# yaramohamadi/Pairwise_Sample_Optimization

Measured on AMD Instinct MI355X. Metric: PSO train-step imgs/sec (paired 1024² SDXL) at 1/2/4/8 MI355X, higher is better.
Workload: dtype bf16; 1 GPU; C2: SDXL-Turbo PSO train step, LoRA r=32 grads, 2 pairs/GPU/micro-step, gas 2, 2-step sampler (T=1); global_batch=4, seq_len=4096, resolution=1024, parallelism=dp1, launch=eager

## Files before the change

include/pso_amd.h:

```cpp
#ifndef PSO_AMD_H
#define PSO_AMD_H

#include <stddef.h>
#include <stdint.h>

#ifdef __cplusplus
extern "C" {
#endif

#define PSO_ABI_VERSION 1

#define PSO_OK 0
#define PSO_ERR_ARG 1
#define PSO_ERR_HIP 2
#define PSO_ERR_UNSUPPORTED 3

#define PSO_F32 0
#define PSO_BF16 1
#define PSO_F16 2
#define PSO_U8 2

#define PSO_MODE_TURBO 0
#define PSO_MODE_DMD 1
#define PSO_MODE_DMD_F16 2
// ... 18 lines not shown
                      const void* eps_ref, int eps_dtype, const float* coef, const float* pref, float beta,
                      float clip_eps, float* lp_out, float* loss_out, void* ws, size_t ws_bytes, void* stream);
int pso_pair_loss_bwd(int mode, int P, int n, const float* x, const float* x_prev, const void* eps_pol,
                      int eps_dtype, const float* coef, const float* pref, float beta, float clip_eps,
                      const float* grad_out, float grad_scale, void* deps_pol, int deps_dtype, const void* ws,
                      size_t ws_bytes, void* stream);

int pso_pair_loss_from_lp(int mode, int P, const float* lp_pol, const float* lp_ref, const float* pref, float beta,
                          float clip_eps, float* loss_out, float* dlp_out, void* stream);

int pso_gemm(int M, int N, const void* a1, long lda1, int K1, const void* b1, long ldb1, const void* a2, long lda2,
             int K2, const void* b2, long ldb2, float alpha, const void* bias, const void* rowbias, long ld_rowbias,
             int rows_per_group, const void* resid, long ldr, void* out, long ldo, int out_dtype, int accumulate,
             int tail_group_n, int tail_rows, void* stream);
size_t pso_gemm_ws_bytes(int M, int N, int K1, int K2);
int pso_gemm_ws(int M, int N, const void* a1, long lda1, int K1, const void* b1, long ldb1, const void* a2, long lda2,
                int K2, const void* b2, long ldb2, float alpha, const void* bias, const void* rowbias, long ld_rowbias,
                int rows_per_group, const void* resid, long ldr, void* out, long ldo, int out_dtype, int accumulate,
                int tail_group_n, int tail_rows, void* ws, size_t ws_bytes, void* stream);

int pso_gemm_batched(int batch, int M, int N, int K, const void* a, long lda, long stride_a, const void* b, long ldb,
                     long stride_b, float alpha, void* out, long ldo, long stride_o, int out_dtype, void* stream);

const char* pso_last_kernel(void);


int pso_gemm_tn(int M, int I, int J, const void* A, long lda, const void* B, long ldb, float alpha, float* out,
                long ldo, void* stream);
size_t pso_gemm_tn_ws_bytes(int M, int I, int J);
int pso_gemm_tn_ws(int M, int I, int J, const void* A, long lda, const void* B, long ldb, float alpha, float* out,
                   long ldo, void* ws, size_t ws_bytes, void* stream);
int pso_gemm_tn_grouped(int M, int I, int J, const void* A, long lda, const void* B, long ldb, float alpha, float* out,
                        long ldo, int group, void* stream);
int pso_gemm_tn_geglu(int M, int F2, int J, const void* A, long lda, const void* B, long ldb, float alpha, float* out,
                      long ldo, void* stream);
typedef struct {
  const void* x; long ldx;
  const void* u; long ldu;
  float* out; long ldo;
  int M, C, group_c;
  float alpha;
} PsoTnRankProblem;
int pso_gemm_tn_rank_batch(int R, int out_jc, int count, const PsoTnRankProblem* probs, void* stream);
size_t pso_gemm_tn_rank_batch_ws_bytes(int R, int out_jc, int count, const PsoTnRankProblem* probs);
int pso_gemm_tn_rank_batch_ws(int R, int out_jc, int count, const PsoTnRankProblem* probs, void* ws, size_t ws_bytes,
                              void* stream);
int pso_gemm_skinny_grouped(int M, int N, int K, const void* A, long lda, const void* W, long ldw, float alpha,
                            void* out, long ldo, int groups, void* stream);

int pso_gemm_geglu(int M, int N, const void* a, long lda, int K, const void* w, long ldw, const void* bias, void* out,
                   long ldo, void* out_pre, long ld_pre, int pre_rows, void* stream);
int pso_gemm_geglu_bwd(int M, int N, const void* a, long lda, int K, const void* w, long ldw, const void* pre,
                       long ld_pre, void* out, long ldo, void* stream);

int pso_quant_rows_fp8(int M, int K, const void* x, long ldx, void* q, long ldq, void* e8m0, void* stream);
int pso_gemm_fp8(int epi, int M, int N, int K, const void* a, long lda, const void* sa, const void* w, long ldw,
                 const void* sw, const void* a2, long lda2, int K2, const void* sa2, const void* w2, long ldw2,
                 const void* sw2, int tail_m, int tail_group_n, float alpha, const void* bias, const void* resid,
                 long ldr, void* out, long ldo, void* out_pre, long ld_pre, int pre_rows, void* stream);

size_t pso_db_loss_ws_bytes(int B, int n);
int pso_db_loss_fwd(int loss_type, int B, int n, const void* eps, const void* eps_ref, int eps_dtype,
                    const float* noisy, const float* x0, const float* sigma, float beta, float neg_defactor,
                    float prior_w, float* losses_out, float* logits_out, float* loss_out, void* ws, size_t ws_bytes,
                    void* stream);
int pso_db_loss_bwd(int loss_type, int B, int n, const void* eps, int eps_dtype, const float* noisy, const float* x0,
                    const float* sigma, float beta, float neg_defactor, float prior_w, const float* grad_out,
                    float grad_scale, void* deps, int deps_dtype, const void* ws, size_t ws_bytes, void* stream);

#define PSO_CONV_NORMAL 1
#define PSO_CONV_UP2 2
#define PSO_CONV_T2 3
int pso_conv2d(int mode, int B, const void* src1, int C1, const void* src2, int C2, int H, int W, int Ho, int Wo,
               int ks, int stride, int pad, const void* weight, int Cout, const void* a2, long lda2, int K2,
               const void* b2, long ldb2, float alpha, const void* bias, const void* rowbias, long ld_rowbias,
               const void* resid, long ldr, void* out, long ldo, int out_dtype, int accumulate, void* stream);
size_t pso_conv2d_ws_bytes(int B, int Ho, int Wo, int Cout, int K1, int K2);
int pso_conv2d_ws(int mode, int B, const void* src1, int C1, const void* src2, int C2, int H, int W, int Ho, int Wo,
                  int ks, int stride, int pad, const void* weight, int Cout, const void* a2, long lda2, int K2,
                  const void* b2, long ldb2, float alpha, const void* bias, const void* rowbias, long ld_rowbias,
                  const void* resid, long ldr, void* out, long ldo, int out_dtype, int accumulate, void* ws,
                  size_t ws_bytes, void* stream);

size_t pso_group_norm_ws_bytes(int B, int HW, int C);
int pso_group_norm_fwd(int B, int HW, int C, int G, float eps, const void* x, const void* gamma, const void* beta,
                       int silu, void* y, float* stats, void* ws, size_t ws_bytes, void* stream);
int pso_group_norm_bwd(int B, int HW, int C, int G, const void* x, const void* dy, const float* stats,
                       const void* gamma, const void* beta, int silu, const void* dadd, void* dx, float* dgamma,
                       float* dbeta, int accumulate_dparams, void* ws, size_t ws_bytes, void* stream);

int pso_layer_norm_fwd(int M, int C, float eps, const void* x, long ldx, const void* gamma, const void* beta, void* y,
                       long ldy, float* stats, void* stream);
int pso_layer_norm_bwd(int M, int C, const void* x, long ldx, const void* dy, long lddy, const float* stats,
                       const void* gamma, const void* dadd, long ldadd, void* dx, long lddx, void* stream);

int pso_attention_fwd(int B, int H, int Sq, int Sk, const void* q, long ldq, long sq_b, const void* k, long ldk,
                      long sk_b, const void* v, long ldv, long sv_b, float scale, void* o, long ldo, long so_b,
                      float* lse, void* stream);
size_t pso_attention_bwd_ws_bytes(int B, int H, int Sq, int Sk);
int pso_attention_bwd(int B, int H, int Sq, int Sk, const void* q, long ldq, long sq_b, const void* k, long ldk,
                      long sk_b, const void* v, long ldv, long sv_b, const void* o, long ldo, long so_b,
                      const float* lse, const void* dO, long lddo, long sdo_b, float scale, void* dq, long lddq,
                      long sdq_b, void* dk, long lddk, long sdk_b, void* dv, long lddv, long sdv_b, void* ws,
                      size_t ws_bytes, void* stream);

int pso_geglu_fwd(long M, int F, const void* in, long ldi, void* out, long ldo, void* stream);
int pso_geglu_bwd(long M, int F, const void* in, long ldi, const void* dout, long lddo, void* din, long lddi,
                  void* stream);
int pso_silu(long n, const void* x, void* y, void* stream);
int pso_timestep_embedding(int n, int dim, const float* t, void* out, long ldo, int out_col, void* stream);
int pso_transpose(int R, int Rp, int C, const void* in, long ldi, void* out, long ldo, void* stream);
int pso_im2col3(int B, int H, int W, int C, const void* in, void* out, int Kp, void* stream);

int pso_colsum_acc(long M, int N, const void* x, long ldx, long rows_per_group, float* out, long ldo, void* stream);
int pso_layer_norm_dparam(int M, int C, const void* x, long ldx, const void* dy, long lddy, const float* stats,
                          float* dgamma, float* dbeta, void* stream);
size_t pso_colsum_acc_ws_bytes(long M, int N, long rows_per_group);
int pso_colsum_acc_ws(long M, int N, const void* x, long ldx, long rows_per_group, float* out, long ldo, void* ws,
                      size_t ws_bytes, void* stream);
size_t pso_layer_norm_dparam_ws_bytes(int M, int C);
int pso_layer_norm_dparam_ws(int M, int C, const void* x, long ldx, const void* dy, long lddy, const float* stats,
                             float* dgamma, float* dbeta, void* ws, size_t ws_bytes, void* stream);
int pso_im2col_conv(int mode, int B, const void* src1, int C1, const void* src2, int C2, int H, int W, int Ho, int Wo,
                    int stride, int pad, void* out, long ldo, void* stream);
int pso_sumpool2(int B, int H, int W, int C, const void* in, const void* dadd, void* out, void* stream);
int pso_axpby(long n, float a, const void* x, float b, const void* z, void* y, void* stream);
int pso_cast_f32_bf16(long n, const float* x, float scale, void* y, void* stream);
int pso_cast_bf16_f32(long n, const void* x, float* y, void* stream);
int pso_conv_weight_t(int Co, int ks, int Ci, int flip, const void* w, void* wt, void* stream);
int pso_transpose_batched(int n, const void* descs, int max_r, int max_c, void* stream);
int pso_lora_pack(int n, const void* descs, long max_items, float scale, void* stream);
int pso_lora_grad_fold(int n, const void* descs, long max_items, void* stream);
int pso_dora_weight_norm(int n, const void* descs, int max_out, int init, void* stream);
int pso_dora_scale_fwd(int M, int N, int rows_policy, const void* z, long ldz, const float* g, const void* bias,
                       const void* resid, long ldr, void* y, long ldy, void* stream);
size_t pso_dora_bwd_ws_bytes(int M, int N);
int pso_dora_bwd(int M, int N, const void* dy, long lddy, const void* z, long ldz, const float* g, const float* n,
                 void* dyg, long lddyg, float* dm, void* ws, size_t ws_bytes, void* stream);
int pso_lora_merge(int n, const void* descs, const void* host_descs, void* stream);
int pso_transpose_multi(int n, const void* descs, int total_tiles, void* stream);
int pso_gather_rows(long n, long row_bytes, const void* src, const int64_t* idx, void* dst, void* stream);
int pso_nchw_to_nhwc(int B, int C, int Cp, long HW, const void* src, int src_dtype, float scale, void* dst,
                     void* stream);
int pso_softmax_rows(int M, int N, void* x, long ld, void* stream);
int pso_nhwc_to_nchw(int B, int C, long HW, const void* src, void* dst, int dst_dtype, void* stream);
int pso_concat_channels(long npix, int C1, const void* x1, int C2, const void* x2, void* out, void* stream);
int pso_split_channels(long npix, int C1, int C2, const void* in, void* y1, void* y2, const void* add2,
                       void* stream);

size_t pso_grad_clip_ws_bytes(long n);
int pso_grad_clip_coef(long n, const float* grad, float grad_scale, float max_norm, float* out_norm_coef, void* ws,
                       size_t ws_bytes, void* stream);
int pso_adamw_step(long n, float* param, const float* grad, float* exp_avg, float* exp_avg_sq, float lr, float beta1,
                   float beta2, float eps, float weight_decay, int step, float grad_scale, const float* clip_coef,
                   void* stream);
size_t pso_adamw8bit_blocks(long n);
void pso_adamw8bit_maps(float* signed_map, float* unsigned_map);
int pso_adamw8bit_step(long n, float* param, const float* grad, uint8_t* exp_avg_q, uint8_t* exp_avg_sq_q,
                       float* absmax_m, float* absmax_v, float lr, float beta1, float beta2, float eps,
                       float weight_decay, int step, float grad_scale, const float* clip_coef, void* stream);
int pso_adamw8bit_step_bf16(long n, float* param, void* param_bf16, const float* grad, uint8_t* exp_avg_q,
                            uint8_t* exp_avg_sq_q, float* absmax_m, float* absmax_v, float lr, float beta1, float beta2,
                            float eps, float weight_decay, int step, float grad_scale, const float* clip_coef,
                            void* stream);
int pso_adamw8bit_step_blocks(long n, int nblk, const long* desc, float* param, void* param_bf16, const float* grad,
                              uint8_t* exp_avg_q, uint8_t* exp_avg_sq_q, float* absmax_m, float* absmax_v,
                              float* exp_avg_32, float* exp_avg_sq_32, float lr, float beta1, float beta2, float eps,
                              float weight_decay, int step, float grad_scale, const float* clip_coef, void* stream);
int pso_adamw8bit_step_blocks_zero_grad(long n, int nblk, const long* desc, float* param, void* param_bf16,
                                        float* grad, uint8_t* exp_avg_q, uint8_t* exp_avg_sq_q, float* absmax_m,
                                        float* absmax_v, float* exp_avg_32, float* exp_avg_sq_32, float lr,
                                        float beta1, float beta2, float eps, float weight_decay, int step,
                                        float grad_scale, const float* clip_coef, void* stream);
int pso_zero_f32(long n, float* x, void* stream);
#define PSO_AMP_WORDS 16
#define PSO_AMP_SCALE 0
#define PSO_AMP_INV_SCALE 1
#define PSO_AMP_FOUND_INF 2
#define PSO_AMP_GROWTH_TRACKER 3
#define PSO_AMP_STEP 4
#define PSO_AMP_SKIPPED 5
#define PSO_AMP_NORM 6
#define PSO_AMP_CLIP_COEF 7
#define PSO_AMP_GRAD_MUL 8
#define PSO_AMP_BC1 9
#define PSO_AMP_BC2_SQRT 10
#define PSO_AMP_C1 11
#define PSO_AMP_C2 12
int pso_amp_unscale_clip(long n, const float* grad, float grad_scale, float max_norm, float beta1, float beta2,
                         void* amp_state, void* ws, size_t ws_bytes, void* stream);
int pso_amp_update(void* amp_state, float growth_factor, float backoff_factor, int growth_interval, void* stream);
int pso_adamw_step_amp(long n, float* param, const float* grad, float* exp_avg, float* exp_avg_sq, float lr,
                       float beta1, float beta2, float eps, float weight_decay, const void* amp_state, void* stream);
int pso_adamw8bit_step_blocks_amp(long n, int nblk, const long* desc, float* param, void* param_bf16,
                                  const float* grad, uint8_t* exp_avg_q, uint8_t* exp_avg_sq_q, float* absmax_m,
                                  float* absmax_v, float* exp_avg_32, float* exp_avg_sq_32, float lr, float beta1,
                                  float beta2, float eps, float weight_decay, const void* amp_state, void* stream);
int pso_adamw8bit_step_blocks_zero_grad_amp(long n, int nblk, const long* desc, float* param, void* param_bf16,
                                            float* grad, uint8_t* exp_avg_q, uint8_t* exp_avg_sq_q, float* absmax_m,
                                            float* absmax_v, float* exp_avg_32, float* exp_avg_sq_32, float lr,
                                            float beta1, float beta2, float eps, float weight_decay,
                                            const void* amp_state, void* stream);
#define PSO_LR_CONSTANT 0
#define PSO_LR_CONSTANT_WITH_WARMUP 1
#define PSO_LR_LINEAR 2
#define PSO_LR_COSINE 3
#define PSO_LR_COSINE_WITH_RESTARTS 4
#define PSO_LR_POLYNOMIAL 5
int pso_lr_schedule(int kind, double base_lr, int warmup, int total, int num_cycles, double power,
                    const void* amp_state, int step, float* lr_out, void* stream);
int pso_adamw_step_amp_lr(long n, float* param, const float* grad, float* exp_avg, float* exp_avg_sq,
                          const float* lr_dev, float beta1, float beta2, float eps, float weight_decay,
                          const void* amp_state, void* stream);
int pso_adamw8bit_step_blocks_amp_lr(long n, int nblk, const long* desc, float* param, void* param_bf16,
                                     const float* grad, uint8_t* exp_avg_q, uint8_t* exp_avg_sq_q, float* absmax_m,
                                     float* absmax_v, float* exp_avg_32, float* exp_avg_sq_32, const float* lr_dev,
                                     float beta1, float beta2, float eps, float weight_decay, const void* amp_state,
                                     void* stream);
int pso_adamw8bit_step_blocks_zero_grad_amp_lr(long n, int nblk, const long* desc, float* param, void* param_bf16,
                                               float* grad, uint8_t* exp_avg_q, uint8_t* exp_avg_sq_q,
                                               float* absmax_m, float* absmax_v, float* exp_avg_32,
                                               float* exp_avg_sq_32, const float* lr_dev, float beta1, float beta2,
                                               float eps, float weight_decay, const void* amp_state, void* stream);
#define PSO_PRODIGY_WORDS 24
#define PSO_PRODIGY_D 0
#define PSO_PRODIGY_D0 2
#define PSO_PRODIGY_D_MAX 4
#define PSO_PRODIGY_D_NUMERATOR 6
#define PSO_PRODIGY_D_DENOM 8
#define PSO_PRODIGY_D_HAT 10
#define PSO_PRODIGY_DLR 12
// ... 43 lines not shown
```

pairwise_sample_optimization_amd/_lib.py:

```python
import ctypes
import os

import torch

_HERE = os.path.dirname(os.path.abspath(__file__))
KNOBS = os.environ.get("PSO_LIB", "") == "knobs"
F16 = os.environ.get("PSO_LIB", "") == "f16"
LIB_PATH = os.environ.get("PSO_LIB_PATH") or os.path.join(
    _HERE, "libpso_amd_knobs.so" if KNOBS else "libpso_amd_f16.so" if F16 else "libpso_amd.so")

PSO_F32 = 0
PSO_BF16 = 1
PSO_F16 = 2
ELEM_DTYPE = torch.float16 if F16 else torch.bfloat16
ELEM_CODE = PSO_F16 if F16 else PSO_BF16
MODE_TURBO = 0
MODE_DMD = 1
MODE_DMD_F16 = 2
MODE_DMD_BF16 = 3
COEF_STRIDE = 8
AMP_WORDS = 16
(AMP_SCALE, AMP_INV_SCALE, AMP_FOUND_INF, AMP_GROWTH_TRACKER, AMP_STEP, AMP_SKIPPED, AMP_NORM, AMP_CLIP_COEF,
 AMP_GRAD_MUL, AMP_BC1, AMP_BC2_SQRT, AMP_C1, AMP_C2) = range(13)
AMP_INT_WORDS = (AMP_FOUND_INF, AMP_GROWTH_TRACKER, AMP_STEP, AMP_SKIPPED)
PRODIGY_WORDS = 24
PRODIGY_F64 = {"d": 0, "d0": 2, "d_max": 4, "d_numerator": 6, "d_denom": 8, "d_hat": 10, "dlr": 12}
PRODIGY_I32 = {"k": 14, "updated": 15, "skipped": 16}
PRODIGY_DECOUPLE, PRODIGY_BIAS_CORRECTION, PRODIGY_SAFEGUARD_WARMUP = 1, 2, 4
LR_KINDS = {"constant": 0, "constant_with_warmup": 1, "linear": 2, "cosine": 3, "cosine_with_restarts": 4,
            "polynomial": 5}

_lib = None


class PsoTnRankProblem(ctypes.Structure):
    _fields_ = [("x", ctypes.c_void_p), ("ldx", ctypes.c_long), ("u", ctypes.c_void_p), ("ldu", ctypes.c_long),
                ("out", ctypes.c_void_p), ("ldo", ctypes.c_long), ("M", ctypes.c_int), ("C", ctypes.c_int),
                ("group_c", ctypes.c_int), ("alpha", ctypes.c_float)]

vp = ctypes.c_void_p
ci = ctypes.c_int
cf = ctypes.c_float
cd = ctypes.c_double
csz = ctypes.c_size_t
ci64 = ctypes.c_int64
cl = ctypes.c_long

SIGNATURES = {
    "pso_last_error": (ctypes.c_char_p, []),
    "pso_abi_version": (ci, []),
    "pso_elem_dtype": (ci, []),
    "pso_step_logprob_ws_bytes": (csz, [ci, ci]),
    "pso_step_logprob": (ci, [ci, ci, ci, vp, vp, ci, vp, vp, ci, vp, vp, vp, vp, csz, vp]),
    "pso_pair_loss_ws_bytes": (csz, [ci, ci]),
    "pso_pair_loss_fwd": (ci, [ci, ci, ci, vp, vp, vp, vp, ci, vp, vp, cf, cf, vp, vp, vp, csz, vp]),
    "pso_pair_loss_bwd": (ci, [ci, ci, ci, vp, vp, vp, ci, vp, vp, cf, cf, vp, cf, vp, ci, vp, csz, vp]),
    "pso_pair_loss_from_lp": (ci, [ci, ci, vp, vp, vp, cf, cf, vp, vp, vp]),
    "pso_db_loss_ws_bytes": (csz, [ci, ci]),
    "pso_db_loss_fwd": (ci, [ci, ci, ci, vp, vp, ci, vp, vp, vp, cf, cf, cf, vp, vp, vp, vp, csz, vp]),
    "pso_db_loss_bwd": (ci, [ci, ci, ci, vp, ci, vp, vp, vp, cf, cf, cf, vp, cf, vp, ci, vp, csz, vp]),
    "pso_gemm": (ci, [ci, ci, vp, cl, ci, vp, cl, vp, cl, ci, vp, cl, cf, vp, vp, cl, ci, vp, cl, vp, cl, ci, ci,
                      ci, ci, vp]),
    "pso_gemm_ws_bytes": (csz, [ci, ci, ci, ci]),
    "pso_gemm_ws": (ci, [ci, ci, vp, cl, ci, vp, cl, vp, cl, ci, vp, cl, cf, vp, vp, cl, ci, vp, cl, vp, cl, ci, ci,
                         ci, ci, vp, csz, vp]),
    "pso_gemm_batched": (ci, [ci, ci, ci, ci, vp, cl, cl, vp, cl, cl, cf, vp, cl, cl, ci, vp]),
    "pso_last_kernel": (ctypes.c_char_p, []),
    "pso_attention_small": (ci, [ci, ci, ci, ci, vp, cl, cl, vp, cl, cl, vp, cl, cl, ci, cf, vp, cl, cl, vp]),
    "pso_activation": (ci, [cl, vp, ci, vp]),
    "pso_embed_tokens": (ci, [ci, ci, ci, vp, vp, vp, vp, vp]),
    "pso_embed_vision": (ci, [ci, ci, ci, vp, vp, vp, vp, vp]),
    "pso_cosine_rows": (ci, [ci, ci, vp, cl, vp, cl, vp, vp]),
    "pso_row_mean": (ci, [ci, cl, vp, vp, vp]),
    "pso_patchify": (ci, [ci, ci, ci, ci, ci, vp, vp, vp]),
    "pso_clip_preprocess_ws_bytes": (csz, [ci, ci, ci, ci]),
    "pso_clip_preprocess": (ci, [ci, ci, ci, vp, ci, ci, ci, ci, vp, vp, vp, vp, csz, vp]),
    "pso_gemm_tn": (ci, [ci, ci, ci, vp, cl, vp, cl, cf, vp, cl, vp]),
    "pso_gemm_tn_grouped": (ci, [ci, ci, ci, vp, cl, vp, cl, cf, vp, cl, ci, vp]),
    "pso_gemm_tn_geglu": (ci, [ci, ci, ci, vp, cl, vp, cl, cf, vp, cl, vp]),
    "pso_gemm_tn_ws_bytes": (csz, [ci, ci, ci]),
    "pso_gemm_tn_ws": (ci, [ci, ci, ci, vp, cl, vp, cl, cf, vp, cl, vp, csz, vp]),
    "pso_gemm_tn_rank_batch": (ci, [ci, ci, ci, vp, vp]),
    "pso_gemm_tn_rank_batch_ws_bytes": (csz, [ci, ci, ci, vp]),
    "pso_gemm_tn_rank_batch_ws": (ci, [ci, ci, ci, vp, vp, csz, vp]),
    "pso_gemm_skinny_grouped": (ci, [ci, ci, ci, vp, cl, vp, cl, cf, vp, cl, ci, vp]),
    "pso_gemm_geglu": (ci, [ci, ci, vp, cl, ci, vp, cl, vp, vp, cl, vp, cl, ci, vp]),
    "pso_gemm_geglu_bwd": (ci, [ci, ci, vp, cl, ci, vp, cl, vp, cl, vp, cl, vp]),
    "pso_quant_rows_fp8": (ci, [ci, ci, vp, cl, vp, cl, vp, vp]),
    "pso_gemm_fp8": (ci, [ci, ci, ci, ci, vp, cl, vp, vp, cl, vp, vp, cl, ci, vp, vp, cl, vp, ci, ci, cf, vp, vp, cl,
                          vp, cl, vp, cl, ci, vp]),
    "pso_conv2d": (ci, [ci, ci, vp, ci, vp, ci, ci, ci, ci, ci, ci, ci, ci, vp, ci, vp, cl, ci, vp, cl, cf, vp, vp,
                        cl, vp, cl, vp, cl, ci, ci, vp]),
    "pso_conv2d_ws_bytes": (csz, [ci, ci, ci, ci, ci, ci]),
    "pso_conv2d_ws": (ci, [ci, ci, vp, ci, vp, ci, ci, ci, ci, ci, ci, ci, ci, vp, ci, vp, cl, ci, vp, cl, cf, vp, vp,
                           cl, vp, cl, vp, cl, ci, ci, vp, csz, vp]),
    "pso_group_norm_ws_bytes": (csz, [ci, ci, ci]),
    "pso_group_norm_fwd": (ci, [ci, ci, ci, ci, cf, vp, vp, vp, ci, vp, vp, vp, csz, vp]),
    "pso_group_norm_bwd": (ci, [ci, ci, ci, ci, vp, vp, vp, vp, vp, ci, vp, vp, vp, vp, ci, vp, csz, vp]),
    "pso_layer_norm_fwd": (ci, [ci, ci, cf, vp, cl, vp, vp, vp, cl, vp, vp]),
    "pso_layer_norm_bwd": (ci, [ci, ci, vp, cl, vp, cl, vp, vp, vp, cl, vp, cl, vp]),
    "pso_attention_fwd": (ci, [ci, ci, ci, ci, vp, cl, cl, vp, cl, cl, vp, cl, cl, cf, vp, cl, cl, vp, vp]),
    "pso_attention_bwd_ws_bytes": (csz, [ci, ci, ci, ci]),
    "pso_attention_bwd": (ci, [ci, ci, ci, ci, vp, cl, cl, vp, cl, cl, vp, cl, cl, vp, cl, cl, vp, vp, cl, cl, cf,
                               vp, cl, cl, vp, cl, cl, vp, cl, cl, vp, csz, vp]),
    "pso_geglu_fwd": (ci, [cl, ci, vp, cl, vp, cl, vp]),
    "pso_geglu_bwd": (ci, [cl, ci, vp, cl, vp, cl, vp, cl, vp]),
    "pso_silu": (ci, [cl, vp, vp, vp]),
    "pso_timestep_embedding": (ci, [ci, ci, vp, vp, cl, ci, vp]),
    "pso_transpose": (ci, [ci, ci, ci, vp, cl, vp, cl, vp]),
    "pso_im2col3": (ci, [ci, ci, ci, ci, vp, vp, ci, vp]),
    "pso_colsum_acc": (ci, [cl, ci, vp, cl, cl, vp, cl, vp]),
    "pso_layer_norm_dparam": (ci, [ci, ci, vp, cl, vp, cl, vp, vp, vp, vp]),
    "pso_colsum_acc_ws_bytes": (csz, [cl, ci, cl]),
    "pso_colsum_acc_ws": (ci, [cl, ci, vp, cl, cl, vp, cl, vp, csz, vp]),
    "pso_layer_norm_dparam_ws_bytes": (csz, [ci, ci]),
    "pso_layer_norm_dparam_ws": (ci, [ci, ci, vp, cl, vp, cl, vp, vp, vp, vp, csz, vp]),
    "pso_im2col_conv": (ci, [ci, ci, vp, ci, vp, ci, ci, ci, ci, ci, ci, ci, vp, cl, vp]),
    "pso_sumpool2": (ci, [ci, ci, ci, ci, vp, vp, vp, vp]),
    "pso_axpby": (ci, [cl, cf, vp, cf, vp, vp, vp]),
    "pso_cast_f32_bf16": (ci, [cl, vp, cf, vp, vp]),
    "pso_cast_bf16_f32": (ci, [cl, vp, vp, vp]),
    "pso_conv_weight_t": (ci, [ci, ci, ci, ci, vp, vp, vp]),
    "pso_concat_channels": (ci, [cl, ci, vp, ci, vp, vp, vp]),
    "pso_nchw_to_nhwc": (ci, [ci, ci, ci, cl, vp, ci, cf, vp, vp]),
    "pso_softmax_rows": (ci, [ci, ci, vp, cl, vp]),
    "pso_grad_clip_ws_bytes": (csz, [cl]),
    "pso_transpose_batched": (ci, [ci, vp, ci, ci, vp]),
    "pso_transpose_multi": (ci, [ci, vp, ci, vp]),
    "pso_lora_pack": (ci, [ci, vp, cl, cf, vp]),
    "pso_lora_grad_fold": (ci, [ci, vp, cl, vp]),
    "pso_dora_weight_norm": (ci, [ci, vp, ci, ci, vp]),
    "pso_dora_scale_fwd": (ci, [ci, ci, ci, vp, cl, vp, vp, vp, cl, vp, cl, vp]),
    "pso_dora_bwd_ws_bytes": (csz, [ci, ci]),
    "pso_dora_bwd": (ci, [ci, ci, vp, cl, vp, cl, vp, vp, vp, cl, vp, vp, csz, vp]),
    "pso_lora_merge": (ci, [ci, vp, vp, vp]),
    "pso_gather_rows": (ci, [cl, cl, vp, vp, vp, vp]),
    "pso_grad_clip_coef": (ci, [cl, vp, cf, cf, vp, vp, csz, vp]),
    "pso_adamw_step": (ci, [cl, vp, vp, vp, vp, cf, cf, cf, cf, cf, ci, cf, vp, vp]),
    "pso_adamw8bit_blocks": (csz, [cl]),
    "pso_adamw8bit_maps": (None, [vp, vp]),
    "pso_adamw8bit_step": (ci, [cl, vp, vp, vp, vp, vp, vp, cf, cf, cf, cf, cf, ci, cf, vp, vp]),
    "pso_adamw8bit_step_bf16": (ci, [cl, vp, vp, vp, vp, vp, vp, vp, cf, cf, cf, cf, cf, ci, cf, vp, vp]),
    "pso_adamw8bit_step_blocks": (ci, [cl, ci, vp, vp, vp, vp, vp, vp, vp, vp, vp, vp, cf, cf, cf, cf, cf, ci, cf,
                                       vp, vp]),
    "pso_adamw8bit_step_blocks_zero_grad": (ci, [cl, ci, vp, vp, vp, vp, vp, vp, vp, vp, vp, vp, cf, cf, cf, cf, cf,
                                                 ci, cf, vp, vp]),
    "pso_amp_unscale_clip": (ci, [cl, vp, cf, cf, cf, cf, vp, vp, csz, vp]),
    "pso_amp_update": (ci, [vp, cf, cf, ci, vp]),
    "pso_adamw_step_amp": (ci, [cl, vp, vp, vp, vp, cf, cf, cf, cf, cf, vp, vp]),
    "pso_adamw8bit_step_blocks_amp": (ci, [cl, ci, vp, vp, vp, vp, vp, vp, vp, vp, vp, vp, cf, cf, cf, cf, cf, vp,
                                           vp]),
    "pso_adamw8bit_step_blocks_zero_grad_amp": (ci, [cl, ci, vp, vp, vp, vp, vp, vp, vp, vp, vp, vp, cf, cf, cf, cf,
                                                     cf, vp, vp]),
    "pso_lr_schedule": (ci, [ci, cd, ci, ci, ci, cd, vp, ci, vp, vp]),
    "pso_adamw_step_amp_lr": (ci, [cl, vp, vp, vp, vp, vp, cf, cf, cf, cf, vp, vp]),
    "pso_adamw8bit_step_blocks_amp_lr": (ci, [cl, ci, vp, vp, vp, vp, vp, vp, vp, vp, vp, vp, vp, cf, cf, cf, cf, vp,
                                              vp]),
    "pso_adamw8bit_step_blocks_zero_grad_amp_lr": (ci, [cl, ci, vp, vp, vp, vp, vp, vp, vp, vp, vp, vp, vp, cf, cf, cf,
                                                        cf, vp, vp]),
    "pso_prodigy_step_lr": (ci, [cl, vp, vp, vp, vp, vp, vp, vp, vp, cf, cf, cf, cf, cf, ci, cf, cf, cf, vp, vp, vp,
                                 csz, vp]),
    "pso_prodigy_ws_bytes": (csz, [cl]),
    "pso_prodigy_step": (ci, [cl, vp, vp, vp, vp, vp, vp, vp, cf, cf, cf, cf, cf, cf, ci, cf, cf, cf, vp, vp, vp, csz,
                              vp]),
    "pso_ema_step": (ci, [cl, vp, vp, cf, vp]),
    "pso_ema_swap": (ci, [cl, vp, vp, vp]),
    "pso_zero_f32": (ci, [cl, vp, vp]),
    "pso_preference": (ci, [ci, ci, vp, vp, ci, vp, vp]),
    "pso_nhwc_to_nchw": (ci, [ci, ci, cl, vp, vp, ci, vp]),
    "pso_split_channels": (ci, [cl, ci, ci, vp, vp, vp, vp, vp]),
}


class PsoGemmPlanQuery(ctypes.Structure):
    _fields_ = ([(n, ci) for n in ("variant", "group", "tn_split", "have_ws", "M", "N", "K1", "K2")] +
                [(n, cl) for n in ("lda1", "ldb1", "lda2", "ldb2")] +
                [(n, ci) for n in ("tail_group_n", "tail_rows", "batch", "out_dtype", "accumulate", "bias_align",
                                   "rowbias_align", "resid_align", "out_align")] +
                [(n, cl) for n in ("ld_rowbias", "ldr", "ldo")] + [("rows_per_group", ci), ("alpha", cf)] +
                [(n, ci) for n in ("conv_mode", "B", "C1", "C2", "H", "W", "Ho", "Wo", "ks", "stride", "pad",
                                   "tn_group")])


class PsoGemmPlanInfo(ctypes.Structure):
    _fields_ = [(n, ci) for n in ("form", "bm", "bn", "wm", "wn", "stages", "pipe", "epi", "conv_mode", "atomic_ks",
                                  "ws_ks", "stage_epi", "vec_ok", "group_m")]


PLAN_GEMM, PLAN_CONV, PLAN_BATCHED, PLAN_GEGLU, PLAN_GEGLU_BWD, PLAN_TN, PLAN_TN_GEGLU = range(7)

KNOB_SIGNATURES = {
    "pso_gemm_set_variant": (None, [ci]),
    "pso_gemm_plan_query": (ci, [ci, ctypes.POINTER(PsoGemmPlanQuery), ctypes.POINTER(PsoGemmPlanInfo)]),
    "pso_gemm8p_skip_epilogue": (None, [ci]),
    "pso_gemm_tn_set_split": (None, [ci]),
    "pso_attention_set_variant": (None, [ci]),
    "pso_attn_pp_trace": (ci, [vp]),
}


class PsoLibError(RuntimeError):
    pass


def _bind(lib):
    for name, (res, args) in SIGNATURES.items():
        fn = getattr(lib, name)
        fn.restype = res
        fn.argtypes = args
    if KNOBS:
        for name, (res, args) in KNOB_SIGNATURES.items():
            fn = getattr(lib, name)
            fn.restype = res
            fn.argtypes = args


def require_knobs(what):
    if not KNOBS:
        raise PsoLibError(f"{what} is a benchmark knob: run with PSO_LIB=knobs (libpso_amd_knobs.so); the product "
                          "library libpso_amd.so has none")


def require_bf16(what):
    if F16:
        raise PsoLibError(f"{what} is not supported by the f16 library (PSO_LIB=f16, libpso_amd_f16.so): unset "
                          "PSO_LIB and run it on the bf16 library")


def lib():
    global _lib
    if _lib is None:
        if not os.path.exists(LIB_PATH):
            raise PsoLibError(f"{LIB_PATH} not built: run `python -c 'import __graft_entry__ as g; g.build()'` "
                              "(no CPU fallback exists)")
        l = ctypes.CDLL(LIB_PATH, mode=ctypes.RTLD_GLOBAL)
        _bind(l)
        if l.pso_elem_dtype() != ELEM_CODE:
            raise PsoLibError(f"{LIB_PATH} has 16-bit element code {l.pso_elem_dtype()}, but PSO_LIB="
                              f"{os.environ.get('PSO_LIB', '')!r} expects {ELEM_CODE} ({ELEM_DTYPE}): PSO_LIB=f16 goes "
                              "with libpso_amd_f16.so, everything else with a bf16 library")
        _lib = l
    return _lib


def check(rc, what=""):
    if rc != 0:
        msg = lib().pso_last_error().decode(errors="replace")
        raise PsoLibError(f"{what} failed (rc={rc}): {msg}")


def stream_ptr(device=None):
    return torch.cuda.current_stream(device).cuda_stream

# ... 22 lines not shown
```

pairwise_sample_optimization_amd/csrc/elementwise.hip:

```cpp
#include "common.h"

__device__ __forceinline__ void unpack8e(uint4 v, float* f) {
  const uint32_t w[4] = {v.x, v.y, v.z, v.w};
#pragma unroll
  for (int i = 0; i < 4; ++i) {
    f[2 * i] = bf2f(w[i] & 0xffff);
    f[2 * i + 1] = bf2f(w[i] >> 16);
  }
}
__device__ __forceinline__ uint4 pack8e(const float* f) {
  return make_uint4(pack2bf(f[0], f[1]), pack2bf(f[2], f[3]), pack2bf(f[4], f[5]), pack2bf(f[6], f[7]));
}

static int grid_for(long n, int per_thread = 1) {
  long g = (n / per_thread + 255) / 256;
  if (g > 8192) g = 8192;
  return (int)(g < 1 ? 1 : g);
}

#define GRID_STRIDE(i, n) for (long i = blockIdx.x * (long)blockDim.x + threadIdx.x; i < (n); i += (long)gridDim.x * blockDim.x)


__global__ void geglu_fwd_kernel(long M, int F, const bf16_t* __restrict__ in, long ldi, bf16_t* __restrict__ out,
                                 long ldo) {
// ... 141 lines not shown
        unpack8e(*reinterpret_cast<const uint4*>(in + (((long)b * 2 * H + 2 * y + dy) * 2 * W + 2 * x + dx) * C + c), a);
#pragma unroll
        for (int j = 0; j < 8; ++j) acc[j] += a[j];
      }
    if (dadd) {
      float a[8];
      unpack8e(*reinterpret_cast<const uint4*>(dadd + pix * C + c), a);
#pragma unroll
      for (int j = 0; j < 8; ++j) acc[j] += a[j];
    }
    *reinterpret_cast<uint4*>(out + pix * C + c) = pack8e(acc);
  }
}

__global__ void axpby_kernel(long n8, float a, const bf16_t* __restrict__ x, float b, const bf16_t* __restrict__ z,
                             bf16_t* __restrict__ y) {
  GRID_STRIDE(v, n8) {
    float p[8], q[8];
    unpack8e(*reinterpret_cast<const uint4*>(x + v * 8), p);
    if (z) unpack8e(*reinterpret_cast<const uint4*>(z + v * 8), q);
#pragma unroll
    for (int j = 0; j < 8; ++j) p[j] = a * p[j] + (z ? b * q[j] : 0.f);
    *reinterpret_cast<uint4*>(y + v * 8) = pack8e(p);
  }
}

__global__ void cast_f32_bf16_kernel(long n, const float* __restrict__ x, float scale, bf16_t* __restrict__ y) {
  long done = 0;
  if (((reinterpret_cast<uintptr_t>(x) | reinterpret_cast<uintptr_t>(y)) & 15) == 0) {
    done = n & ~7L;
    GRID_STRIDE(v, n >> 3) {
      const float4 a = reinterpret_cast<const float4*>(x)[2 * v], b = reinterpret_cast<const float4*>(x)[2 * v + 1];
      reinterpret_cast<uint4*>(y)[v] = make_uint4(pack2bf(a.x * scale, a.y * scale), pack2bf(a.z * scale, a.w * scale),
                                                  pack2bf(b.x * scale, b.y * scale), pack2bf(b.z * scale, b.w * scale));
    }
  }
  GRID_STRIDE(i, n - done) y[done + i] = f2bf(x[done + i] * scale);
}
__global__ void cast_bf16_f32_kernel(long n, const bf16_t* __restrict__ x, float* __restrict__ y) {
  long done = 0;
  if (((reinterpret_cast<uintptr_t>(x) | reinterpret_cast<uintptr_t>(y)) & 15) == 0) {
    done = n & ~7L;
    GRID_STRIDE(v, n >> 3) {
      const uint4 u = reinterpret_cast<const uint4*>(x)[v];
#ifdef PSO_ELEM_F16
      reinterpret_cast<float4*>(y)[2 * v] = make_float4(bf2f(u.x & 0xffff), bf2f(u.x >> 16), bf2f(u.y & 0xffff), bf2f(u.y >> 16));
      reinterpret_cast<float4*>(y)[2 * v + 1] = make_float4(bf2f(u.z & 0xffff), bf2f(u.z >> 16), bf2f(u.w & 0xffff), bf2f(u.w >> 16));
#else
      reinterpret_cast<float4*>(y)[2 * v] = make_float4(__uint_as_float(u.x << 16), __uint_as_float(u.x & 0xffff0000u),
                                                        __uint_as_float(u.y << 16), __uint_as_float(u.y & 0xffff0000u));
      reinterpret_cast<float4*>(y)[2 * v + 1] = make_float4(__uint_as_float(u.z << 16), __uint_as_float(u.z & 0xffff0000u),
                                                            __uint_as_float(u.w << 16), __uint_as_float(u.w & 0xffff0000u));
#endif
    }
  }
  GRID_STRIDE(i, n - done) y[done + i] = bf2f(x[done + i]);
}

__global__ __launch_bounds__(256) void conv_weight_t_kernel(int Co, int ks, int Ci, int flip,
                                                            const bf16_t* __restrict__ w, bf16_t* __restrict__ wt) {
  __shared__ bf16_t tile[64][72];
  const int tap = blockIdx.z, kh = tap / ks, kw = tap - kh * ks;
  const int tap2 = flip ? (ks - 1 - kh) * ks + (ks - 1 - kw) : tap;
  const int ci0 = blockIdx.x * 64, co0 = blockIdx.y * 64, t = threadIdx.x;
  const long ldw = (long)ks * ks * Ci;
  const bool vec = (Ci % 8) == 0 && (reinterpret_cast<uintptr_t>(w) & 15) == 0;
  for (int q = t; q < 64 * 8; q += 256) {
    const int r = q >> 3, c = (q & 7) * 8, co = co0 + r, ci = ci0 + c;
    const bf16_t* src = w + co * ldw + (long)tap * Ci + ci;
    if (vec && co < Co && ci + 8 <= Ci) {
      *reinterpret_cast<uint4*>(&tile[r][c]) = *reinterpret_cast<const uint4*>(src);
    } else {
      for (int e = 0; e < 8; ++e) tile[r][c + e] = (co < Co && ci + e < Ci) ? src[e] : (bf16_t)0;
    }
  }
  __syncthreads();
  const int lx = t & 63, ly = t >> 6;
  for (int i = ly; i < 64; i += 4) {
    const int ci = ci0 + i, co = co0 + lx;
    if (ci < Ci && co < Co) wt[((long)ci * ks * ks + tap2) * Co + co] = tile[lx][i];
  }
}

__global__ void concat_kernel(long npix, int C1, const bf16_t* __restrict__ x1, int C2, const bf16_t* __restrict__ x2,
                              bf16_t* __restrict__ out) {
  const int C8 = (C1 + C2) / 8, c18 = C1 / 8;
  GRID_STRIDE(v, npix * C8) {
    const long p = v / C8;
    const int ch = (int)(v - p * C8);
    const uint4 val = ch < c18 ? *reinterpret_cast<const uint4*>(x1 + p * C1 + ch * 8)
                               : *reinterpret_cast<const uint4*>(x2 + p * C2 + (ch - c18) * 8);
    *reinterpret_cast<uint4*>(out + v * 8) = val;
  }
}

__global__ void split_kernel(long npix, int C1, int C2, const bf16_t* __restrict__ in, bf16_t* __restrict__ y1,
                             bf16_t* __restrict__ y2, const bf16_t* __restrict__ add2) {
  const int C8 = (C1 + C2) / 8, c18 = C1 / 8;
  GRID_STRIDE(v, npix * C8) {
    const long p = v / C8;
    const int ch = (int)(v - p * C8);
    const uint4 val = *reinterpret_cast<const uint4*>(in + v * 8);
    if (ch < c18) {
      *reinterpret_cast<uint4*>(y1 + p * C1 + ch * 8) = val;
    } else {
      bf16_t* o = y2 + p * C2 + (ch - c18) * 8;
      if (add2) {
        float a[8], b[8];
        unpack8e(val, a);
        unpack8e(*reinterpret_cast<const uint4*>(add2 + p * C2 + (ch - c18) * 8), b);
#pragma unroll
        for (int j = 0; j < 8; ++j) a[j] += b[j];
        *reinterpret_cast<uint4*>(o) = pack8e(a);
      } else {
        *reinterpret_cast<uint4*>(o) = val;
      }
    }
  }
}

__global__ void nchw_to_nhwc_kernel(int B, int C, int Cp, long HW, const void* __restrict__ src, int src_f32,
                                    float scale, bf16_t* __restrict__ dst) {
  GRID_STRIDE(i, (long)B * Cp * HW) {
    const int c = (int)(i % Cp);
    const long p = (i / Cp) % HW;
    const int b = (int)(i / (Cp * HW));
    const long s = ((long)b * C + c) * HW + p;
    float v = 0.f;
    if (c < C) v = src_f32 ? reinterpret_cast<const float*>(src)[s] : bf2f(reinterpret_cast<const bf16_t*>(src)[s]);
    dst[i] = f2bf(v * scale);
  }
}
__global__ void nhwc_to_nchw_kernel(int B, int C, long HW, const bf16_t* __restrict__ src, void* __restrict__ dst,
                                    int dst_f32) {
  GRID_STRIDE(i, (long)B * C * HW) {
    const long p = i % HW;
    const int c = (int)((i / HW) % C);
    const int b = (int)(i / (C * HW));
    const bf16_t v = src[((long)b * HW + p) * C + c];
    if (dst_f32) reinterpret_cast<float*>(dst)[i] = bf2f(v);
    else reinterpret_cast<bf16_t*>(dst)[i] = v;
  }
}

struct TransposeDesc {
  const bf16_t* src;
  bf16_t* dst;
  int R, C;
  long ldi, ldo;
};
__global__ void transpose_batched_kernel(const TransposeDesc* __restrict__ d) {
  __shared__ bf16_t tile[64][66];
  const TransposeDesc t = d[blockIdx.z];
  const int r0 = blockIdx.y * 64, c0 = blockIdx.x * 64;
  if (r0 >= t.R || c0 >= t.C) return;
  const int tx = threadIdx.x & 63, ty = threadIdx.x >> 6;
  for (int i = ty; i < 64; i += 4) {
    const int r = r0 + i, c = c0 + tx;
    tile[i][tx] = (r < t.R && c < t.C) ? t.src[(long)r * t.ldi + c] : (bf16_t)0;
  }
  __syncthreads();
  for (int i = ty; i < 64; i += 4) {
    const int c = c0 + i, r = r0 + tx;
    if (c < t.C && r < t.R) t.dst[(long)c * t.ldo + r] = tile[tx][i];
  }
}

template <typename U>
__global__ void gather_rows_kernel(long n, long units, const U* __restrict__ src, const int64_t* __restrict__ idx,
                                   U* __restrict__ dst) {
  GRID_STRIDE(i, n * units) {
    const long r = i / units, c = i - r * units;
    dst[i] = src[idx[r] * units + c];
  }
}

__global__ __launch_bounds__(256) void softmax_rows_kernel(int N, bf16_t* __restrict__ x, long ld) {
  __shared__ float red[4];
  bf16_t* row = x + blockIdx.x * ld;
  float mx = -INFINITY;
  for (int c = threadIdx.x * 8; c < N; c += 256 * 8) {
    float a[8];
    unpack8e(*reinterpret_cast<const uint4*>(row + c), a);
#pragma unroll
    for (int j = 0; j < 8; ++j) mx = fmaxf(mx, a[j]);
  }
  mx = warp_max(mx);
  if ((threadIdx.x & 63) == 0) red[threadIdx.x >> 6] = mx;
  __syncthreads();
  mx = fmaxf(fmaxf(red[0], red[1]), fmaxf(red[2], red[3]));
  __syncthreads();
  float s = 0.f;
  for (int c = threadIdx.x * 8; c < N; c += 256 * 8) {
    float a[8];
    unpack8e(*reinterpret_cast<const uint4*>(row + c), a);
#pragma unroll
    for (int j = 0; j < 8; ++j) s += __expf(a[j] - mx);
  }
  s = warp_sum(s);
  if ((threadIdx.x & 63) == 0) red[threadIdx.x >> 6] = s;
  __syncthreads();
  const float inv = 1.f / (red[0] + red[1] + red[2] + red[3]);
  for (int c = threadIdx.x * 8; c < N; c += 256 * 8) {
    float a[8];
    unpack8e(*reinterpret_cast<const uint4*>(row + c), a);
#pragma unroll
    for (int j = 0; j < 8; ++j) a[j] = __expf(a[j] - mx) * inv;
    *reinterpret_cast<uint4*>(row + c) = pack8e(a);
  }
}

extern "C" {

int pso_softmax_rows(int M, int N, void* x, long ld, void* stream) {
  PSO_ARG_CHECK(N % 8 == 0 && ld % 8 == 0 && x, "pso_softmax_rows: N, ld multiples of 8");
  softmax_rows_kernel<<<M, 256, 0, (hipStream_t)stream>>>(N, (bf16_t*)x, ld);
  return pso_check_launch("pso_softmax_rows");
}

int pso_transpose_batched(int n, const void* descs, int max_r, int max_c, void* stream) {
  PSO_ARG_CHECK(n > 0 && descs, "pso_transpose_batched: bad args");
  dim3 grid(cdiv(max_c, 64), cdiv(max_r, 64), n);
  transpose_batched_kernel<<<grid, 256, 0, (hipStream_t)stream>>>((const TransposeDesc*)descs);
  return pso_check_launch("pso_transpose_batched");
}

int pso_gather_rows(long n, long row_bytes, const void* src, const int64_t* idx, void* dst, void* stream) {
  PSO_ARG_CHECK(row_bytes % 4 == 0 && src && idx && dst, "pso_gather_rows: row_bytes %% 4");
  if (row_bytes % 16 == 0 && ((uintptr_t)src & 15) == 0 && ((uintptr_t)dst & 15) == 0)
    gather_rows_kernel<uint4><<<grid_for(n * (row_bytes / 16)), 256, 0, (hipStream_t)stream>>>(
        n, row_bytes / 16, (const uint4*)src, idx, (uint4*)dst);
  else
    gather_rows_kernel<uint32_t><<<grid_for(n * (row_bytes / 4)), 256, 0, (hipStream_t)stream>>>(
        n, row_bytes / 4, (const uint32_t*)src, idx, (uint32_t*)dst);
  return pso_check_launch("pso_gather_rows");
}

int pso_nchw_to_nhwc(int B, int C, int Cp, long HW, const void* src, int src_dtype, float scale, void* dst,
                     void* stream) {
  PSO_DTYPE_CHECK(src_dtype, "pso_nchw_to_nhwc");
  PSO_ARG_CHECK(src && dst && Cp >= C, "pso_nchw_to_nhwc: bad args");
  nchw_to_nhwc_kernel<<<grid_for((long)B * Cp * HW), 256, 0, (hipStream_t)stream>>>(
      B, C, Cp, HW, src, src_dtype == PSO_F32, scale, (bf16_t*)dst);
  return pso_check_launch("pso_nchw_to_nhwc");
}

int pso_nhwc_to_nchw(int B, int C, long HW, const void* src, void* dst, int dst_dtype, void* stream) {
  PSO_DTYPE_CHECK(dst_dtype, "pso_nhwc_to_nchw");
  PSO_ARG_CHECK(src && dst, "pso_nhwc_to_nchw: bad args");
  nhwc_to_nchw_kernel<<<grid_for((long)B * C * HW), 256, 0, (hipStream_t)stream>>>(B, C, HW, (const bf16_t*)src,
                                                                                  dst, dst_dtype == PSO_F32);
  return pso_check_launch("pso_nhwc_to_nchw");
}

int pso_concat_channels(long npix, int C1, const void* x1, int C2, const void* x2, void* out, void* stream) {
  PSO_ARG_CHECK(C1 % 8 == 0 && C2 % 8 == 0 && x1 && x2 && out, "pso_concat_channels: C %% 8");
  concat_kernel<<<grid_for(npix * (C1 + C2) / 8), 256, 0, (hipStream_t)stream>>>(
      npix, C1, (const bf16_t*)x1, C2, (const bf16_t*)x2, (bf16_t*)out);
  return pso_check_launch("pso_concat_channels");
}

int pso_split_channels(long npix, int C1, int C2, const void* in, void* y1, void* y2, const void* add2,
                       void* stream) {
  PSO_ARG_CHECK(C1 % 8 == 0 && C2 % 8 == 0 && in && y1 && y2, "pso_split_channels: C %% 8");
  split_kernel<<<grid_for(npix * (C1 + C2) / 8), 256, 0, (hipStream_t)stream>>>(
      npix, C1, C2, (const bf16_t*)in, (bf16_t*)y1, (bf16_t*)y2, (const bf16_t*)add2);
  return pso_check_launch("pso_split_channels");
}

int pso_geglu_fwd(long M, int F, const void* in, long ldi, void* out, long ldo, void* stream) {
  PSO_ARG_CHECK(F % 8 == 0 && ldi % 8 == 0 && ldo % 8 == 0 && in && out, "pso_geglu_fwd: bad args");
  geglu_fwd_kernel<<<grid_for(M * (F / 8)), 256, 0, (hipStream_t)stream>>>(M, F, (const bf16_t*)in, ldi,
                                                                          (bf16_t*)out, ldo);
  return pso_check_launch("pso_geglu_fwd");
}

int pso_geglu_bwd(long M, int F, const void* in, long ldi, const void* dout, long lddo, void* din, long lddi,
                  void* stream) {
  PSO_ARG_CHECK(F % 8 == 0 && ldi % 8 == 0 && lddo % 8 == 0 && lddi % 8 == 0 && in && dout && din,
                "pso_geglu_bwd: bad args");
  geglu_bwd_kernel<<<grid_for(M * (F / 8)), 256, 0, (hipStream_t)stream>>>(M, F, (const bf16_t*)in, ldi,
                                                                          (const bf16_t*)dout, lddo, (bf16_t*)din,
                                                                          lddi);
  return pso_check_launch("pso_geglu_bwd");
}

int pso_silu(long n, const void* x, void* y, void* stream) {
  PSO_ARG_CHECK(n % 8 == 0 && x && y, "pso_silu: n must be a multiple of 8");
  silu_kernel<<<grid_for(n / 8), 256, 0, (hipStream_t)stream>>>(n / 8, (const bf16_t*)x, (bf16_t*)y);
  return pso_check_launch("pso_silu");
}

int pso_timestep_embedding(int n, int dim, const float* t, void* out, long ldo, int out_col, void* stream) {
  PSO_ARG_CHECK(dim % 2 == 0 && t && out, "pso_timestep_embedding: bad args");
  timestep_embed_kernel<<<grid_for((long)n * dim / 2), 256, 0, (hipStream_t)stream>>>(n, dim, t, (bf16_t*)out, ldo,
                                                                                      out_col);
  return pso_check_launch("pso_timestep_embedding");
}

int pso_transpose_multi(int n, const void* descs, int total_tiles, void* stream) {
  PSO_ARG_CHECK(n > 0 && descs && total_tiles > 0, "pso_transpose_multi: bad args");
  transpose_multi_kernel<<<total_tiles, 256, 0, (hipStream_t)stream>>>(n, (const TransposeMultiDesc*)descs);
  return pso_check_launch("pso_transpose_multi");
}

int pso_transpose(int R, int Rp, int C, const void* in, long ldi, void* out, long ldo, void* stream) {
  PSO_ARG_CHECK(in && out && Rp >= R, "pso_transpose: bad args");
  dim3 grid(cdiv(C, 64), cdiv(Rp, 64));
  transpose_kernel<<<grid, 256, 0, (hipStream_t)stream>>>(R, Rp, C, (const bf16_t*)in, ldi, (bf16_t*)out, ldo);
  return pso_check_launch("pso_transpose");
}

int pso_im2col3(int B, int H, int W, int C, const void* in, void* out, int Kp, void* stream) {
  PSO_ARG_CHECK(Kp >= 9 * C && in && out, "pso_im2col3: Kp < 9C");
  im2col3_kernel<<<grid_for((long)B * H * W * Kp), 256, 0, (hipStream_t)stream>>>(B, H, W, C, (const bf16_t*)in, 0,
                                                                                  (bf16_t*)out, Kp);
  return pso_check_launch("pso_im2col3");
}

int pso_sumpool2(int B, int H, int W, int C, const void* in, const void* dadd, void* out, void* stream) {
  PSO_ARG_CHECK(C % 8 == 0 && in && out, "pso_sumpool2: C %% 8");
  sumpool2_kernel<<<grid_for((long)B * H * W * C / 8), 256, 0, (hipStream_t)stream>>>(
      B, H, W, C, (const bf16_t*)in, (const bf16_t*)dadd, (bf16_t*)out);
  return pso_check_launch("pso_sumpool2");
}

int pso_axpby(long n, float a, const void* x, float b, const void* z, void* y, void* stream) {
  PSO_ARG_CHECK(n % 8 == 0 && x && y, "pso_axpby: n %% 8");
  axpby_kernel<<<grid_for(n / 8), 256, 0, (hipStream_t)stream>>>(n / 8, a, (const bf16_t*)x, b, (const bf16_t*)z,
                                                                 (bf16_t*)y);
  return pso_check_launch("pso_axpby");
}

int pso_cast_f32_bf16(long n, const float* x, float scale, void* y, void* stream) {
  cast_f32_bf16_kernel<<<grid_for(n, 8), 256, 0, (hipStream_t)stream>>>(n, x, scale, (bf16_t*)y);
  return pso_check_launch("pso_cast_f32_bf16");
}

int pso_cast_bf16_f32(long n, const void* x, float* y, void* stream) {
  cast_bf16_f32_kernel<<<grid_for(n, 8), 256, 0, (hipStream_t)stream>>>(n, (const bf16_t*)x, y);
  return pso_check_launch("pso_cast_bf16_f32");
}
// ... 9 lines not shown
```

pairwise_sample_optimization_amd/csrc/gemm.hip:

```cpp
#include "gemm_args.h"
#include "gemm_plan.h"

#include <cstdlib>

#define GEMM_THREADS 256
#define BK 64

#define EPI_NONE 0
#define EPI_GEGLU 1
#define EPI_GEGLU_BWD 2

__device__ __forceinline__ int swz(int r, int c) { return r * BK + ((c ^ (r & 7)) << 3); }

template <int BM, int BN, int WAVES>
struct Tile {
  static constexpr int A_P = BM / 8, B_P = BN / 8;
  static constexpr int A_CH = (A_P + WAVES - 1) / WAVES;
  static constexpr int B_CH = (B_P + WAVES - 1) / WAVES;
  static constexpr bool A_EVEN = A_P % WAVES == 0, B_EVEN = B_P % WAVES == 0;
};

struct RowCoord {
  int b, oy, ox;
  bool valid;
// ... 718 lines not shown
  GemmFacts f{};
  f.M = g.M; f.N = g.N; f.K1 = g.K1; f.K2 = g.a2 ? g.K2 : 0; f.has_tail = g.a2 != nullptr;
  f.tail_group_n = g.tail_group_n; f.tail_m = g.tail_m; f.batch = g.batch;
  f.out_dtype = g.out_dtype; f.accumulate = g.accumulate;
  f.has_bias = g.bias != nullptr; f.has_rowbias = g.rowbias != nullptr; f.has_resid = g.resid != nullptr;
  f.conv_mode = cv.mode; f.B = hw > 0 ? (int)(g.M / hw) : 0; f.C1 = cv.C1; f.C2 = cv.C2; f.H = cv.H; f.W = cv.W;
  f.Ho = cv.Ho; f.Wo = cv.Wo; f.ks = cv.ks; f.stride = cv.stride; f.pad = cv.pad;
  f.ab16 = al16(g.a1) && al16(g.b1);
  f.ld_ab8 = (g.lda1 % 8) == 0 && (g.ldb1 % 8) == 0;
  f.ld_ab_eq = g.lda1 == g.ldb1;
  f.out16 = al16(g.out); f.out_vec = g.out_dtype == PSO_F32 ? al16(g.out) : al8(g.out);
  f.ldo8 = (g.ldo % 8) == 0; f.ldo4 = (g.ldo % 4) == 0;
  f.resid16 = !g.resid || (al16(g.resid) && (g.ldr % 8) == 0);
  f.resid8 = !g.resid || (al8(g.resid) && (g.ldr % 4) == 0);
  f.bias8 = !g.bias || al8(g.bias);
  f.rowbias8 = !g.rowbias || al8(g.rowbias);
  f.ld_rowbias4 = !g.rowbias || (g.ld_rowbias % 4) == 0;
  f.rowgroup_hw = g.rows_per_group == hw;
  f.fits_a = fits30(g.M, g.lda1); f.fits_b = fits30(g.N, g.ldb1);
  f.fits_tail = fits30(g.tail_m, g.lda2) && fits30(g.N, g.ldb2);
  f.fits_conv = fits30((long)g.M + 2L * (cv.W + 1), cv.C1);
  f.have_ws = g.ws && al16(g.ws); f.ws_bytes = ws_bytes;
  f.small_conv_entry = small_conv_entry;
  return f;
}

#define PSO_TILE(BM, BN, WM, WN, ST, PIPE, EPI) \
  if (p.epi == EPI && p.tile_is(BM, BN, WM, WN, ST, PIPE)) return launch<BM, BN, WM, WN, ST, PIPE, EPI>(g, st, ks)
static int launch_tile(const GemmPlan& p, const GemmArgs& g, hipStream_t st, int ks) {
  PSO_TILE(64, 64, 2, 2, 2, false, EPI_NONE);
  PSO_TILE(64, 128, 2, 2, 2, false, EPI_NONE);
  PSO_TILE(128, 64, 2, 2, 2, false, EPI_NONE);
  PSO_TILE(64, 160, 2, 2, 2, false, EPI_NONE);
  PSO_TILE(128, 128, 2, 4, 2, false, EPI_NONE);
  PSO_TILE(128, 160, 2, 2, 2, false, EPI_NONE);
  PSO_TILE(256, 256, 2, 4, 2, false, EPI_NONE);
  PSO_TILE(256, 256, 2, 4, 2, false, EPI_GEGLU);
  PSO_TILE(128, 160, 2, 2, 2, false, EPI_GEGLU_BWD);
  PSO_TILE(64, 64, 2, 2, 2, false, EPI_GEGLU_BWD);
#ifdef PSO_BENCH_KNOBS
#define PSO_FORCED(V, OK, BM, BN, WM, WN, ST, PIPE) PSO_TILE(BM, BN, WM, WN, ST, PIPE, EPI_NONE);
  PSO_FORCED_TILES(PSO_FORCED)
#undef PSO_FORCED
  PSO_TILE(128, 128, 2, 2, 2, false, EPI_GEGLU);
  PSO_TILE(128, 256, 2, 4, 2, false, EPI_GEGLU);
  PSO_TILE(256, 128, 4, 2, 2, false, EPI_GEGLU);
  PSO_TILE(128, 128, 2, 2, 3, false, EPI_GEGLU);
#endif
  pso_set_error("pso_gemm: tile %d x %d (%d x %d waves, %d stages%s, epilogue %d) is not compiled into this library",
                p.BM, p.BN, p.WM, p.WN, p.STAGES, p.PIPE ? ", pipelined" : "", p.epi);
  return PSO_ERR_UNSUPPORTED;
}
#undef PSO_TILE

static int run_plan(const GemmPlan& p, GemmArgs& g, hipStream_t st) {
  g.stage_epi = p.stage_epi; g.vec_ok = p.vec_ok; g.group_m = p.group_m;
  if (p.ws_ks < 2) g.ws = nullptr;
  switch (p.form) {
    case GF_NONE: return PSO_OK;
    case GF_SKINNY:
      return pso_gemm_skinny_nt(g.M, g.N, g.K1, g.a1, g.lda1, g.b1, g.ldb1, g.alpha, g.out, g.ldo,
                                g.out_dtype == PSO_F32, g.accumulate, 1, st);
    case GF_SMALL_CONV:
      return pso_conv3x3_smallc_run(g.M / (g.conv.H * g.conv.W), g.conv.H, g.conv.W, g.conv.C1, g.N, g.a1, g.b1, g.bias,
                                    g.out, st);
    case GF_8P256: return pso_gemm8p_launch(256, p.epi, false, gemm8_args(g), st);
    case GF_8P160: return pso_gemm8p_launch(160, p.epi, false, gemm8_args(g), st);
    case GF_8P320: return pso_gemm8p_launch(320, p.epi, false, gemm8_args(g), st);
    case GF_8P320_CONV: return pso_gemm8p_launch(320, p.epi, true, gemm8_args(g), st);
    case GF_TILE: break;
    default: pso_set_error("pso_gemm: bad plan form %d", p.form); return PSO_ERR_UNSUPPORTED;
  }
  if (p.ws_ks >= 2) {
    launch_tile(p, g, st, p.ws_ks);
    const long n4 = (long)g.M * (g.N / 4);
    gemm_splitk_reduce_kernel<<<(unsigned)((n4 + 255) / 256), 256, 0, st>>>(g, p.ws_ks);
    return pso_check_launch("pso_gemm_ws");
  }
  return launch_tile(p, g, st, p.atomic_ks);
}

static int run_gemm(GemmArgs& g, hipStream_t st, size_t ws_bytes = 0, bool small_conv_entry = false) {
  GemmFacts f = gemm_facts(g, ws_bytes, small_conv_entry);
  GemmPlan p = gemm_plan(f, g_gemm_knobs);
  if (p.form == GF_SMALL_CONV) {
    if (run_plan(p, g, st) == PSO_OK) return PSO_OK;
    f.small_conv_entry = false;
    p = gemm_plan(f, g_gemm_knobs);
  }
  if (p.form != GF_NONE && g.tail_group_n > 0 && (g.tail_group_n % 64) != 0) {
    pso_set_error("pso_gemm: tail_group_n must be a multiple of 64");
    return PSO_ERR_ARG;
  }
  return run_plan(p, g, st);
}

typedef __attribute__((address_space(3))) s16x4 lds_s16x4_g;
typedef __attribute__((address_space(3))) void tnr_lds_void_g;
__device__ __forceinline__ int swz_tr64(int r, int c) { return r * 64 + ((c ^ (((r >> 1) & 3) << 1)) << 3); }

__device__ __forceinline__ s16x4 tr_read64(const bf16_t* img, int r0, int col0, int lane) {
  const int li = lane & 15;
  const int q = li >> 2, p = li & 3;
  const int col = col0 + 4 * p;
  return __builtin_amdgcn_ds_read_tr16_b64_v4i16((lds_s16x4_g*)(img + swz_tr64(r0 + q, col >> 3) + (col & 7)));
}

__global__ __launch_bounds__(256, 2) void gemm_tn_kernel(int M, int I, int J, const bf16_t* __restrict__ A, long lda,
                                                         const bf16_t* __restrict__ B, long ldb, float alpha,
                                                         float* __restrict__ out, long ldo,
                                                         float* __restrict__ part) {
  __shared__ __attribute__((aligned(16))) bf16_t sA[2][64 * 64];
  __shared__ __attribute__((aligned(16))) bf16_t sB[2][64 * 64];
  const int tid = threadIdx.x, lane = tid & 63, wave = tid >> 6;
  const int wi = wave >> 1, wj = wave & 1;
  const int nbj = (J + 63) / 64;
  const int bi = blockIdx.x / nbj, bj = blockIdx.x - bi * nbj;
  const int i0 = bi * 64, j0 = bj * 64;
  const int nkt = (M + 63) / 64;
  const int per = (nkt + gridDim.y - 1) / gridDim.y;
  const int t_beg = blockIdx.y * per, t_end = min(nkt, t_beg + per);
  uint4 ra[2], rb[2];
  auto load = [&](int t) {
#pragma unroll
    for (int h = 0; h < 2; ++h) {
      const int q = tid + 256 * h;
      const int row = q >> 3, ch = q & 7;
      const int m = t * 64 + row;
      const int ci = i0 + ch * 8, cj = j0 + ch * 8;
      ra[h] = (m < M && ci < I) ? *reinterpret_cast<const uint4*>(A + (long)m * lda + ci) : make_uint4(0, 0, 0, 0);
      rb[h] = (m < M && cj < J) ? *reinterpret_cast<const uint4*>(B + (long)m * ldb + cj) : make_uint4(0, 0, 0, 0);
    }
  };
  auto store = [&](int buf) {
#pragma unroll
    for (int h = 0; h < 2; ++h) {
      const int q = tid + 256 * h;
      const int row = q >> 3, ch = q & 7;
      *reinterpret_cast<uint4*>(sA[buf] + swz_tr64(row, ch)) = ra[h];
      *reinterpret_cast<uint4*>(sB[buf] + swz_tr64(row, ch)) = rb[h];
    }
  };
  f32x4 acc[2][2];
#pragma unroll
  for (int a = 0; a < 2; ++a)
#pragma unroll
    for (int b = 0; b < 2; ++b) acc[a][b] = f32x4{0.f, 0.f, 0.f, 0.f};
  const int g = lane >> 4, c = lane & 15;
  if (t_beg < t_end) {
    load(t_beg);
    store(0);
  }
  __syncthreads();
  for (int t = t_beg; t < t_end; ++t) {
    const int cur = (t - t_beg) & 1;
    if (t + 1 < t_end) load(t + 1);
#pragma unroll
    for (int ks = 0; ks < 2; ++ks) {
      bf16x8 af[2], bfr[2];
#pragma unroll
      for (int a = 0; a < 2; ++a) {
        const int col = wi * 32 + a * 16;
        typedef __attribute__((ext_vector_type(8))) short s16x8;
        const s16x4 x0 = tr_read64(sA[cur], ks * 32 + 8 * g, col, lane);
        const s16x4 x1 = tr_read64(sA[cur], ks * 32 + 8 * g + 4, col, lane);
        s16x8 v = {x0[0], x0[1], x0[2], x0[3], x1[0], x1[1], x1[2], x1[3]};
// ... 353 lines not shown
}

static int conv_entry_args(const char* who, GemmArgs& g, int mode, int B, const void* src1, int C1, const void* src2,
                           int C2, int H, int W, int Ho, int Wo, int ks, int stride, int pad, const void* weight,
                           int Cout, const void* a2, long lda2, int K2, const void* b2, long ldb2, float alpha,
                           const void* bias, const void* rowbias, long ld_rowbias, const void* resid, long ldr,
                           void* out, long ldo, int out_dtype, int accumulate) {
  PSO_ARG_CHECK(mode == PSO_CONV_NORMAL || mode == PSO_CONV_UP2 || mode == PSO_CONV_T2, "%s: bad mode", who);
  PSO_ARG_CHECK(src1 && weight && out, "%s: null operand", who);
  PSO_ARG_CHECK((C1 % 64) == 0 && (C2 % 64) == 0 && (C2 == 0 || src2),
                "%s: channel sources must be multiples of 64 (C1=%d C2=%d); use im2col for small C", who, C1, C2);
  PSO_ARG_CHECK(al16(src1) && (!src2 || al16(src2)) && al16(weight), "%s: alignment", who);
  PSO_ARG_CHECK(ks == 1 || ks == 3, "%s: ks must be 1 or 3", who);
  PSO_ARG_CHECK(mode != PSO_CONV_UP2 || (Ho == 2 * H && Wo == 2 * W && stride == 1), "%s: UP2 geometry", who);
  PSO_ARG_CHECK(!a2 || ((K2 % 8) == 0 && b2 && al16(a2) && al16(b2)), "%s: bad second operand", who);
  PSO_DTYPE_CHECK(out_dtype, who);
  PSO_ARG_CHECK(!accumulate || out_dtype == PSO_F32, "%s: accumulate needs f32 output", who);
  const int Ct = C1 + C2;
  g.a1 = (const bf16_t*)src1; g.lda1 = 0; g.K1 = ks * ks * Ct;
  g.b1 = (const bf16_t*)weight; g.ldb1 = g.K1;
  g.a2 = (const bf16_t*)a2; g.lda2 = lda2; g.K2 = a2 ? K2 : 0;
  g.b2 = (const bf16_t*)b2; g.ldb2 = ldb2;
  g.M = B * Ho * Wo; g.N = Cout;
  g.tail_m = g.M;
  g.conv.mode = mode; g.conv.src2 = (const bf16_t*)src2; g.conv.C1 = C1; g.conv.C2 = C2;
  g.conv.H = H; g.conv.W = W; g.conv.Ho = Ho; g.conv.Wo = Wo; g.conv.ks = ks; g.conv.stride = stride; g.conv.pad = pad;
  g.alpha = alpha;
  g.bias = (const bf16_t*)bias;
  g.rowbias = (const bf16_t*)rowbias; g.ld_rowbias = ld_rowbias; g.rows_per_group = Ho * Wo;
  g.resid = (const bf16_t*)resid; g.ldr = ldr;
  g.out = out; g.ldo = ldo; g.out_dtype = out_dtype; g.accumulate = accumulate;
  return PSO_OK;
}

static GemmArgs batched_args(int batch, int M, int N, int K, const void* a, long lda, long stride_a, const void* b,
                             long ldb, long stride_b, float alpha, void* out, long ldo, long stride_o, int out_dtype) {
  GemmArgs g{};
  g.a1 = (const bf16_t*)a; g.lda1 = lda; g.K1 = K;
  g.b1 = (const bf16_t*)b; g.ldb1 = ldb;
  g.M = M; g.N = N; g.tail_m = M;
  g.alpha = alpha; g.rows_per_group = 1;
  g.out = out; g.ldo = ldo; g.out_dtype = out_dtype;
  g.bat_a = stride_a; g.bat_b = stride_b; g.bat_o = stride_o; g.batch = batch;
  return g;
}

extern "C" {

int pso_gemm_tn_ws(int M, int I, int J, const void* A, long lda, const void* B, long ldb, float alpha, float* out,
                   long ldo, void* ws, size_t ws_bytes, void* stream) {
  PSO_ARG_CHECK(M >= 0 && I > 0 && J > 0 && A && B && out, "pso_gemm_tn_ws: bad args");
  PSO_ARG_CHECK(((uintptr_t)A & 15) == 0 && ((uintptr_t)B & 15) == 0 && (lda % 8) == 0 && (ldb % 8) == 0 &&
                    (I % 8) == 0 && (J % 8) == 0,
                "pso_gemm_tn_ws: operands need 16-B aligned rows and I, J multiples of 8");
  if (M == 0) return PSO_OK;
  const hipStream_t st = (hipStream_t)stream;
  const TnPlan p = tn_plan(M, I, J, lda, ldb, 0, ws && al16(ws), g_gemm_knobs);
  const size_t need = tn_plan_ws_bytes(p, M, I, J);
  if (!need || ws_bytes < need) return pso_gemm_tn_grouped(M, I, J, A, lda, B, ldb, alpha, out, ldo, 0, stream);
  if (p.kind == TNP_RANK) {
    PsoTnRankProblem q{};
    q.x = p.swap ? B : A; q.ldx = p.swap ? ldb : lda;
    q.u = p.swap ? A : B; q.ldu = p.swap ? lda : ldb;
    q.out = out; q.ldo = ldo; q.M = M; q.C = p.swap ? J : I; q.group_c = 0; q.alpha = alpha;
    return pso_gemm_tn_rank_batch_ws(p.rank, p.swap ? 1 : 0, 1, &q, ws, ws_bytes, stream);
  }
  tn_launch_tiles(p, M, I, J, A, lda, B, ldb, alpha, out, ldo, (float*)ws, st);
  const long n4 = (long)I * J / 4;
  tn_reduce_slices_kernel<<<(unsigned)((n4 + 255) / 256), 256, 0, st>>>(I, J, p.ks, (const float*)ws, out, ldo);
  return pso_check_launch("pso_gemm_tn_ws");
}

int pso_gemm(int M, int N, const void* a1, long lda1, int K1, const void* b1, long ldb1, const void* a2, long lda2,
             int K2, const void* b2, long ldb2, float alpha, const void* bias, const void* rowbias, long ld_rowbias,
             int rows_per_group, const void* resid, long ldr, void* out, long ldo, int out_dtype, int accumulate,
             int tail_group_n, int tail_rows, void* stream) {
  GemmArgs g{};
  const int rc = gemm_entry_args("pso_gemm", g, M, N, a1, lda1, K1, b1, ldb1, a2, lda2, K2, b2, ldb2, alpha, bias,
                                 rowbias, ld_rowbias, rows_per_group, resid, ldr, out, ldo, out_dtype, accumulate,
                                 tail_group_n, tail_rows);
  return rc != PSO_OK ? rc : run_gemm(g, (hipStream_t)stream);
}

size_t pso_gemm_ws_bytes(int M, int N, int K1, int K2) {
  const SplitPlan sp = gemm_split_plan(M, N, K1, K2, K2 > 0, g_gemm_knobs);
  return sp.ks >= 2 ? (size_t)sp.ks * M * N * sizeof(float) : 0;
}

int pso_gemm_ws(int M, int N, const void* a1, long lda1, int K1, const void* b1, long ldb1, const void* a2, long lda2,
                int K2, const void* b2, long ldb2, float alpha, const void* bias, const void* rowbias, long ld_rowbias,
                int rows_per_group, const void* resid, long ldr, void* out, long ldo, int out_dtype, int accumulate,
                int tail_group_n, int tail_rows, void* ws, size_t ws_bytes, void* stream) {
  GemmArgs g{};
  const int rc = gemm_entry_args("pso_gemm_ws", g, M, N, a1, lda1, K1, b1, ldb1, a2, lda2, K2, b2, ldb2, alpha, bias,
                                 rowbias, ld_rowbias, rows_per_group, resid, ldr, out, ldo, out_dtype, accumulate,
                                 tail_group_n, tail_rows);
  g.ws = (float*)ws;
  return rc != PSO_OK ? rc : run_gemm(g, (hipStream_t)stream, ws_bytes);
}

int pso_gemm_batched(int batch, int M, int N, int K, const void* a, long lda, long stride_a, const void* b, long ldb,
                     long stride_b, float alpha, void* out, long ldo, long stride_o, int out_dtype, void* stream) {
  PSO_ARG_CHECK(batch >= 1 && M >= 0 && N >= 0 && K >= 0 && (K % 8) == 0, "pso_gemm_batched: bad shape (K %% 8 == 0)");
  PSO_ARG_CHECK(a && b && out, "pso_gemm_batched: null operand");
  PSO_ARG_CHECK(al16(a) && al16(b) && (lda % 8) == 0 && (ldb % 8) == 0 && (stride_a % 8) == 0 && (stride_b % 8) == 0,
                "pso_gemm_batched: A/B need 16-B aligned rows and batch strides");
  PSO_DTYPE_CHECK(out_dtype, "pso_gemm_batched");
  PSO_ARG_CHECK((long)M * lda < 0x7fffffffL && (long)N * ldb < 0x7fffffffL,
                "pso_gemm_batched: one operand spans more than 2^31 elements");
  GemmArgs g = batched_args(batch, M, N, K, a, lda, stride_a, b, ldb, stride_b, alpha, out, ldo, stride_o, out_dtype);
  return run_gemm(g, (hipStream_t)stream);
}

int pso_conv2d(int mode, int B, const void* src1, int C1, const void* src2, int C2, int H, int W, int Ho, int Wo,
               int ks, int stride, int pad, const void* weight, int Cout, const void* a2, long lda2, int K2,
               const void* b2, long ldb2, float alpha, const void* bias, const void* rowbias, long ld_rowbias,
               const void* resid, long ldr, void* out, long ldo, int out_dtype, int accumulate, void* stream) {
  GemmArgs g{};
  const int rc = conv_entry_args("pso_conv2d", g, mode, B, src1, C1, src2, C2, H, W, Ho, Wo, ks, stride, pad, weight,
                                 Cout, a2, lda2, K2, b2, ldb2, alpha, bias, rowbias, ld_rowbias, resid, ldr, out, ldo,
                                 out_dtype, accumulate);
  return rc != PSO_OK ? rc : run_gemm(g, (hipStream_t)stream, 0, alpha == 1.f && ldo == Cout);
}

size_t pso_conv2d_ws_bytes(int B, int Ho, int Wo, int Cout, int K1, int K2) {
  const long M = (long)B * Ho * Wo;
  if (M <= 0 || M > 0x7fffffffL) return 0;
  return pso_gemm_ws_bytes((int)M, Cout, K1, K2);
}

int pso_conv2d_ws(int mode, int B, const void* src1, int C1, const void* src2, int C2, int H, int W, int Ho, int Wo,
                  int ks, int stride, int pad, const void* weight, int Cout, const void* a2, long lda2, int K2,
                  const void* b2, long ldb2, float alpha, const void* bias, const void* rowbias, long ld_rowbias,
                  const void* resid, long ldr, void* out, long ldo, int out_dtype, int accumulate, void* ws,
                  size_t ws_bytes, void* stream) {
  GemmArgs g{};
  const int rc = conv_entry_args("pso_conv2d_ws", g, mode, B, src1, C1, src2, C2, H, W, Ho, Wo, ks, stride, pad, weight,
                                 Cout, a2, lda2, K2, b2, ldb2, alpha, bias, rowbias, ld_rowbias, resid, ldr, out, ldo,
                                 out_dtype, accumulate);
  g.ws = (float*)ws;
  return rc != PSO_OK ? rc : run_gemm(g, (hipStream_t)stream, ws_bytes);
}

int pso_gemm_geglu(int M, int N, const void* a, long lda, int K, const void* w, long ldw, const void* bias, void* out,
                   long ldo, void* out_pre, long ld_pre, int pre_rows, void* stream) {
  PSO_ARG_CHECK(M > 0 && N > 0 && (N % 256) == 0 && K > 0 && (K % 8) == 0 && a && w && bias && out,
                "pso_gemm_geglu: need N %% 256 == 0, K %% 8 == 0, bias");
  PSO_ARG_CHECK(al16(a) && al16(w) && (lda % 8) == 0 && (ldw % 8) == 0 && al16(out) && (ldo % 8) == 0 && al8(bias) &&
                    (!out_pre || (al16(out_pre) && (ld_pre % 8) == 0)),
                "pso_gemm_geglu: alignment (16-B rows)");
  PSO_ARG_CHECK((long)M * lda < 0x7fffffffL && (long)N * ldw < 0x7fffffffL, "pso_gemm_geglu: operand too large");
  GemmArgs g{};
  g.a1 = (const bf16_t*)a; g.lda1 = lda; g.K1 = K;
  g.b1 = (const bf16_t*)w; g.ldb1 = ldw;
  g.M = M; g.N = N; g.alpha = 1.f;
  g.bias = (const bf16_t*)bias;
  g.out = out; g.ldo = ldo; g.out_dtype = PSO_ELEM;
  g.out2 = out_pre; g.ldo2 = ld_pre;
  g.tail_m = (pre_rows > 0 && pre_rows < M) ? pre_rows : M;
  g.rows_per_group = 1;
  return run_plan(geglu_plan(M, N, K, lda == ldw, fits30(M, lda) && fits30(N, ldw), g_gemm_knobs), g,
                  (hipStream_t)stream);
}

int pso_gemm_geglu_bwd(int M, int N, const void* a, long lda, int K, const void* w, long ldw, const void* pre,
                       long ld_pre, void* out, long ldo, void* stream) {
// ... 141 lines not shown
```

pairwise_sample_optimization_amd/csrc/gemm_args.h:

```cpp
#ifndef PSO_GEMM_ARGS_H
#define PSO_GEMM_ARGS_H

#include "common.h"

struct ConvGeom {
  int mode;
  const bf16_t* src2;
  int C1, C2;
  int H, W;
  int Ho, Wo;
  int ks, stride, pad;
};

struct GemmArgs {
  const bf16_t* a1; long lda1; int K1;
  const bf16_t* b1; long ldb1;
  const bf16_t* a2; long lda2; int K2;
  const bf16_t* b2; long ldb2;
  int tail_group_n;
  int tail_m;
  int M, N;
  ConvGeom conv;
  float alpha;
  const bf16_t* bias;
  const bf16_t* rowbias; long ld_rowbias; int rows_per_group;
  const bf16_t* resid; long ldr;
  void* out; long ldo; int out_dtype; int accumulate;
  int vec_ok;
  int stage_epi;
  int group_m;
  void* out2; long ldo2;
  const bf16_t* aux; long ldaux;
  long bat_a, bat_b, bat_o;
  int batch;
  float* ws;
};

struct Gemm8Args {
  const bf16_t* a; long lda;
  const bf16_t* w; long ldw;
  int M, N, K;
  const bf16_t* a2; long lda2; int K2;
  const bf16_t* w2; long ldw2;
  int tail_m, tail_group_n;
  float alpha;
  const bf16_t* bias;
  const bf16_t* resid; long ldr;
  void* out; long ldo;
  void* out2; long ldo2; int pre_rows;
  const bf16_t* aux; long ldaux;
  int group_m;
  int skip_epi;
  const uint8_t* sa; const uint8_t* sw; const uint8_t* sa2; const uint8_t* sw2;
  int cv_H, cv_W, cv_lh, cv_lw, cv_ct, cv_recip;
  const bf16_t* rowbias; long ld_rowbias;
};

inline Gemm8Args gemm8_args(const GemmArgs& g) {
  Gemm8Args r{};
  r.a = g.a1; r.lda = g.conv.mode ? g.conv.C1 : g.lda1; r.w = g.b1; r.ldw = g.ldb1;
  r.M = g.M; r.N = g.N; r.K = g.K1;
  r.a2 = g.a2; r.lda2 = g.lda2; r.K2 = g.a2 ? g.K2 : 0; r.w2 = g.b2; r.ldw2 = g.ldb2;
  r.tail_m = g.tail_m; r.tail_group_n = g.a2 ? g.tail_group_n : 0;
  r.alpha = g.alpha; r.bias = g.bias; r.resid = g.resid; r.ldr = g.ldr;
  r.out = g.out; r.ldo = g.ldo; r.out2 = g.out2; r.ldo2 = g.ldo2; r.pre_rows = g.tail_m;
  r.aux = g.aux; r.ldaux = g.ldaux;
  r.group_m = g.group_m;
  r.cv_H = g.conv.H; r.cv_W = g.conv.W;
  r.rowbias = g.rowbias; r.ld_rowbias = g.ld_rowbias;
  return r;
}

int pso_gemm8p_launch(int bn, int epi, bool conv, Gemm8Args g, hipStream_t st);

#endif
```

pairwise_sample_optimization_amd/csrc/norm.hip:

```cpp
#include "common.h"

#define GN_ROWS 64
#define GN_ROWS_BIG 512
static int gn_rows_fwd(int HW) { return (HW + GN_ROWS - 1) / GN_ROWS > 256 ? GN_ROWS_BIG : GN_ROWS; }

__device__ __forceinline__ void unpack8(uint4 v, float* f) {
  const uint32_t w[4] = {v.x, v.y, v.z, v.w};
#pragma unroll
  for (int i = 0; i < 4; ++i) {
    f[2 * i] = bf2f(w[i] & 0xffff);
    f[2 * i + 1] = bf2f(w[i] >> 16);
  }
}
__device__ __forceinline__ uint4 pack8(const float* f) {
  return make_uint4(pack2bf(f[0], f[1]), pack2bf(f[2], f[3]), pack2bf(f[4], f[5]), pack2bf(f[6], f[7]));
}
__device__ __forceinline__ float sigmoidf_(float x) { return 1.0f / (1.0f + __expf(-x)); }

template <bool BWD, bool SILU>
__global__ void gn_partial_kernel(int HW, int rows, int C, int G, const bf16_t* __restrict__ x, const bf16_t* __restrict__ dy,
                                  const float* __restrict__ stats, const bf16_t* __restrict__ gamma,
                                  const bf16_t* __restrict__ beta, float* __restrict__ ws, float* __restrict__ ws_ch) {
  extern __shared__ float red[];
  const int TPR = C / 8;
  const int RS = blockDim.x / TPR;
  const int slot = threadIdx.x / TPR, cc = threadIdx.x - slot * TPR;
  const int b = blockIdx.y, chunk = blockIdx.x, nchunks = gridDim.x;
  const int r0 = chunk * rows, r1 = min(HW, r0 + rows);
  const int Cg = C / G;
  float s1[8], s2[8];
#pragma unroll
  for (int j = 0; j < 8; ++j) s1[j] = s2[j] = 0.f;
  float mean[8], rstd[8], gm[8], bt[8];
  if (BWD && slot < RS) {
#pragma unroll
    for (int j = 0; j < 8; ++j) {
      const int c = cc * 8 + j, g = c / Cg;
      mean[j] = stats[(b * G + g) * 2];
      rstd[j] = stats[(b * G + g) * 2 + 1];
      gm[j] = gamma ? bf2f(gamma[c]) : 1.f;
      bt[j] = beta ? bf2f(beta[c]) : 0.f;
    }
  }
  if (slot < RS) {
    for (int r = r0 + slot; r < r1; r += RS) {
      const size_t off = ((size_t)b * HW + r) * C + cc * 8;
      float xv[8];
      unpack8(*reinterpret_cast<const uint4*>(x + off), xv);
      if (!BWD) {
#pragma unroll
        for (int j = 0; j < 8; ++j) {
          s1[j] += xv[j];
          s2[j] += xv[j] * xv[j];
        }
      } else {
        float dv[8];
        unpack8(*reinterpret_cast<const uint4*>(dy + off), dv);
#pragma unroll
        for (int j = 0; j < 8; ++j) {
          const float xh = (xv[j] - mean[j]) * rstd[j];
          float dz = dv[j];
          if (SILU) {
            const float z = xh * gm[j] + bt[j];
            const float sg = sigmoidf_(z);
            dz *= sg * (1.f + z * (1.f - sg));
          }
          s1[j] += dz;
          s2[j] += dz * xh;
        }
      }
    }
  }
  if (slot < RS) {
#pragma unroll
    for (int j = 0; j < 8; ++j) {
      red[(slot * C + cc * 8 + j) * 2] = s1[j];
      red[(slot * C + cc * 8 + j) * 2 + 1] = s2[j];
    }
  }
  __syncthreads();
  for (int c = threadIdx.x; c < C; c += blockDim.x) {
    float a = 0.f, q = 0.f;
    for (int s = 0; s < RS; ++s) {
      a += red[(s * C + c) * 2];
      q += red[(s * C + c) * 2 + 1];
    }
    if (ws_ch) {
      float* o = ws_ch + (((size_t)b * nchunks + chunk) * C + c) * 2;
      o[0] = a;
      o[1] = q;
    }
    if (BWD && gamma) {
      const float gmc = bf2f(gamma[c]);
      a *= gmc;
      q *= gmc;
    }
    red[c * 2] = a;
    red[c * 2 + 1] = q;
  }
  __syncthreads();
  for (int g = threadIdx.x; g < G; g += blockDim.x) {
    float a = 0.f, q = 0.f;
    for (int c = g * Cg; c < (g + 1) * Cg; ++c) {
      a += red[c * 2];
      q += red[c * 2 + 1];
    }
    float* o = ws + (((size_t)b * nchunks + chunk) * G + g) * 2;
    o[0] = a;
    o[1] = q;
  }
}

template <bool BWD>
__global__ void gn_finalize_kernel(int B, int HW, int C, int G, int nchunks, float eps, const float* __restrict__ ws,
                                   float* __restrict__ out) {
  const int id = blockIdx.x * (blockDim.x / 64) + (threadIdx.x >> 6);
  const int lane = threadIdx.x & 63;
  if (id >= B * G) return;
  const int b = id / G, g = id - b * G;
  const int Cg = C / G;
  double a = 0.0, q = 0.0;
  for (int k = lane; k < nchunks; k += 64) {
    const float* p = ws + (((size_t)b * nchunks + k) * G + g) * 2;
    a += p[0];
    q += p[1];
  }
  a = warp_sum_d(a);
  q = warp_sum_d(q);
  if (lane != 0) return;
  const double n = (double)HW * Cg;
  if (!BWD) {
// ... 10 lines not shown

__global__ void gn_dparam_kernel(int B, int C, int nchunks, const float* __restrict__ ws, float* __restrict__ dgamma,
                                 float* __restrict__ dbeta, int accumulate) {
  const int c = blockIdx.x * blockDim.x + threadIdx.x;
  if (c >= C) return;
  double a = 0.0, q = 0.0;
  for (int b = 0; b < B; ++b)
    for (int k = 0; k < nchunks; ++k) {
      const float* p = ws + (((size_t)b * nchunks + k) * C + c) * 2;
      a += p[0];
      q += p[1];
    }
  if (dbeta) dbeta[c] = (accumulate ? dbeta[c] : 0.f) + (float)a;
  if (dgamma) dgamma[c] = (accumulate ? dgamma[c] : 0.f) + (float)q;
}

__global__ __launch_bounds__(256) void gn_dparam_split_kernel(int BK, int C, int S, const float* __restrict__ ws,
                                                              double* __restrict__ part2) {
  __shared__ double red[4][64][2];
  const int t = threadIdx.x, tx = t & 63, ty = t >> 6;
  const int c = blockIdx.x * 64 + tx, sp = blockIdx.y;
  double a = 0.0, q = 0.0;
  if (c < C)
    for (int e = sp + S * ty; e < BK; e += 4 * S) {
      const float2 v = *reinterpret_cast<const float2*>(ws + ((size_t)e * C + c) * 2);
      a += v.x;
      q += v.y;
    }
  red[ty][tx][0] = a;
  red[ty][tx][1] = q;
  __syncthreads();
  if (ty == 0 && c < C) {
    part2[((size_t)sp * C + c) * 2] = red[0][tx][0] + red[1][tx][0] + red[2][tx][0] + red[3][tx][0];
    part2[((size_t)sp * C + c) * 2 + 1] = red[0][tx][1] + red[1][tx][1] + red[2][tx][1] + red[3][tx][1];
  }
}

__global__ void gn_dparam_final_kernel(int C, int S, const double* __restrict__ part2, float* __restrict__ dgamma,
                                       float* __restrict__ dbeta, int accumulate) {
  const int c = blockIdx.x * blockDim.x + threadIdx.x;
  if (c >= C) return;
  double a = 0.0, q = 0.0;
  for (int sp = 0; sp < S; ++sp) {
    a += part2[((size_t)sp * C + c) * 2];
    q += part2[((size_t)sp * C + c) * 2 + 1];
  }
  if (dbeta) dbeta[c] = (accumulate ? dbeta[c] : 0.f) + (float)a;
  if (dgamma) dgamma[c] = (accumulate ? dgamma[c] : 0.f) + (float)q;
}

template <bool SILU>
__global__ void gn_apply_fwd_kernel(int HW, int rows, int C, int G, const bf16_t* __restrict__ x, const float* __restrict__ stats,
                                    const bf16_t* __restrict__ gamma, const bf16_t* __restrict__ beta,
                                    bf16_t* __restrict__ y) {
  const int TPR = C / 8;
  const int RS = blockDim.x / TPR;
  const int slot = threadIdx.x / TPR, cc = threadIdx.x - slot * TPR;
  if (slot >= RS) return;
  const int b = blockIdx.y;
  const int r0 = blockIdx.x * rows, r1 = min(HW, r0 + rows);
  const int Cg = C / G;
  float sc[8], sh[8];
#pragma unroll
  for (int j = 0; j < 8; ++j) {
    const int c = cc * 8 + j, g = c / Cg;
    const float mean = stats[(b * G + g) * 2], rstd = stats[(b * G + g) * 2 + 1];
    const float gm = gamma ? bf2f(gamma[c]) : 1.f, bt = beta ? bf2f(beta[c]) : 0.f;
    sc[j] = rstd * gm;
    sh[j] = bt - mean * rstd * gm;
  }
  for (int r = r0 + slot; r < r1; r += RS) {
    const size_t off = ((size_t)b * HW + r) * C + cc * 8;
    float xv[8], o[8];
    unpack8(*reinterpret_cast<const uint4*>(x + off), xv);
#pragma unroll
    for (int j = 0; j < 8; ++j) {
      const float z = fmaf(xv[j], sc[j], sh[j]);
      o[j] = SILU ? z * sigmoidf_(z) : z;
    }
    *reinterpret_cast<uint4*>(y + off) = pack8(o);
  }
}

template <bool SILU>
__global__ void gn_apply_bwd_kernel(int HW, int C, int G, const bf16_t* __restrict__ x, const bf16_t* __restrict__ dy,
                                    const float* __restrict__ stats, const float* __restrict__ coef,
                                    const bf16_t* __restrict__ gamma, const bf16_t* __restrict__ beta,
                                    const bf16_t* __restrict__ dadd, bf16_t* __restrict__ dx) {
  const int TPR = C / 8;
  const int RS = blockDim.x / TPR;
  const int slot = threadIdx.x / TPR, cc = threadIdx.x - slot * TPR;
  if (slot >= RS) return;
  const int b = blockIdx.y;
  const int r0 = blockIdx.x * GN_ROWS, r1 = min(HW, r0 + GN_ROWS);
  const int Cg = C / G;
  float xs[8], xo[8], zs[8], zo[8], P[8], Q[8], R[8];
#pragma unroll
  for (int j = 0; j < 8; ++j) {
    const int c = cc * 8 + j, g = c / Cg;
    const float mean = stats[(b * G + g) * 2], rstd = stats[(b * G + g) * 2 + 1];
    const float ca = coef[(b * G + g) * 2], cb = coef[(b * G + g) * 2 + 1];
    const float gm = gamma ? bf2f(gamma[c]) : 1.f, bt = beta ? bf2f(beta[c]) : 0.f;
    xs[j] = rstd;
    xo[j] = -mean * rstd;
    zs[j] = rstd * gm;
    zo[j] = bt - mean * rstd * gm;
    P[j] = rstd * gm;
    Q[j] = -rstd * ca;
    R[j] = -rstd * cb;
  }
  for (int r = r0 + slot; r < r1; r += RS) {
    const size_t off = ((size_t)b * HW + r) * C + cc * 8;
    float xv[8], dv[8], o[8], av[8];
    unpack8(*reinterpret_cast<const uint4*>(x + off), xv);
    unpack8(*reinterpret_cast<const uint4*>(dy + off), dv);
    if (dadd) unpack8(*reinterpret_cast<const uint4*>(dadd + off), av);
#pragma unroll
    for (int j = 0; j < 8; ++j) {
      const float xh = fmaf(xv[j], xs[j], xo[j]);
      float dz = dv[j];
      if (SILU) {
        const float z = fmaf(xv[j], zs[j], zo[j]);
        const float sg = sigmoidf_(z);
        dz *= sg * (1.f + z * (1.f - sg));
      }
      o[j] = fmaf(P[j], dz, fmaf(R[j], xh, Q[j])) + (dadd ? av[j] : 0.f);
    }
    *reinterpret_cast<uint4*>(dx + off) = pack8(o);
  }
}

static int gn_block(int C) {
  const int TPR = C / 8;
  int rs = 1;
  while (TPR * rs * 2 <= 512) rs *= 2;
  return TPR * rs;
}


template <int MAXV>
__global__ __launch_bounds__(256) void ln_fwd_kernel(int M, int C, float eps, const bf16_t* __restrict__ x, long ldx,
                                                     const bf16_t* __restrict__ gamma, const bf16_t* __restrict__ beta,
                                                     bf16_t* __restrict__ y, long ldy, float* __restrict__ stats) {
  const int row = blockIdx.x * 4 + (threadIdx.x >> 6);
  const int lane = threadIdx.x & 63;
  if (row >= M) return;
  const int C8 = C / 8;
  float v[MAXV][8];
  float s = 0.f;
#pragma unroll
  for (int i = 0; i < MAXV; ++i) {
    const int ch = lane + 64 * i;
    if (ch < C8) {
      unpack8(*reinterpret_cast<const uint4*>(x + row * ldx + ch * 8), v[i]);
#pragma unroll
      for (int j = 0; j < 8; ++j) s += v[i][j];
    }
  }
  const float mean = warp_sum(s) / C;
  float q = 0.f;
#pragma unroll
  for (int i = 0; i < MAXV; ++i) {
    const int ch = lane + 64 * i;
    if (ch < C8) {
#pragma unroll
      for (int j = 0; j < 8; ++j) {
        const float d = v[i][j] - mean;
        q += d * d;
      }
    }
  }
  const float rstd = rsqrtf(warp_sum(q) / C + eps);
#pragma unroll
  for (int i = 0; i < MAXV; ++i) {
    const int ch = lane + 64 * i;
    if (ch < C8) {
      const uint4 gv = *reinterpret_cast<const uint4*>(gamma + ch * 8);
      const uint4 bv = *reinterpret_cast<const uint4*>(beta + ch * 8);
      float gf[8], bf[8], o[8];
      unpack8(gv, gf);
      unpack8(bv, bf);
#pragma unroll
      for (int j = 0; j < 8; ++j) o[j] = (v[i][j] - mean) * rstd * gf[j] + bf[j];
      *reinterpret_cast<uint4*>(y + row * ldy + ch * 8) = pack8(o);
    }
  }
  if (stats && lane == 0) {
    stats[row * 2] = mean;
    stats[row * 2 + 1] = rstd;
  }
}

template <int MAXV>
__global__ __launch_bounds__(256) void ln_bwd_kernel(int M, int C, const bf16_t* __restrict__ x, long ldx,
                                                     const bf16_t* __restrict__ dy, long lddy,
                                                     const float* __restrict__ stats, const bf16_t* __restrict__ gamma,
                                                     const bf16_t* __restrict__ dadd, long ldadd,
                                                     bf16_t* __restrict__ dx, long lddx) {
  const int row = blockIdx.x * 4 + (threadIdx.x >> 6);
  const int lane = threadIdx.x & 63;
  if (row >= M) return;
  const int C8 = C / 8;
  const float mean = stats[row * 2], rstd = stats[row * 2 + 1];
  float xh[MAXV][8], g[MAXV][8];
  float s1 = 0.f, s2 = 0.f;
#pragma unroll
  for (int i = 0; i < MAXV; ++i) {
    const int ch = lane + 64 * i;
    if (ch < C8) {
      float xv[8], dv[8], gf[8];
      unpack8(*reinterpret_cast<const uint4*>(x + row * ldx + ch * 8), xv);
// ... 19 lines not shown
      for (int j = 0; j < 8; ++j) o[j] = rstd * (g[i][j] - a - xh[i][j] * b) + (dadd ? av[j] : 0.f);
      *reinterpret_cast<uint4*>(dx + row * lddx + ch * 8) = pack8(o);
    }
  }
}

static bool ln_aligned16(const void* p, long ld) { return (((uintptr_t)p) & 15) == 0 && (ld % 8) == 0; }

extern "C" {

size_t pso_group_norm_ws_bytes(int B, int HW, int C) {
  return (size_t)B * cdiv(HW, GN_ROWS) * C * 2 * sizeof(float) * 2 + (size_t)B * C * 2 * sizeof(float);
}

int pso_group_norm_fwd(int B, int HW, int C, int G, float eps, const void* x, const void* gamma, const void* beta,
                       int silu, void* y, float* stats, void* ws, size_t ws_bytes, void* stream) {
  PSO_ARG_CHECK(B > 0 && HW > 0 && C > 0 && G > 0 && C % G == 0 && C % 8 == 0 && C <= 4096,
                "pso_group_norm_fwd: bad shape B=%d HW=%d C=%d G=%d", B, HW, C, G);
  PSO_ARG_CHECK(x && y && stats && ws, "pso_group_norm_fwd: null pointer");
  PSO_ARG_CHECK(ws_bytes >= pso_group_norm_ws_bytes(B, HW, C), "pso_group_norm_fwd: workspace too small");
  hipStream_t st = (hipStream_t)stream;
  const int rows = gn_rows_fwd(HW);
  const int nchunks = cdiv(HW, rows);
  const int threads = gn_block(C);
  const size_t shm = (size_t)(threads / (C / 8)) * C * 2 * sizeof(float);
  gn_partial_kernel<false, false><<<dim3(nchunks, B), threads, shm, st>>>(HW, rows, C, G, (const bf16_t*)x, nullptr,
                                                                          nullptr, nullptr, nullptr, (float*)ws,
                                                                          nullptr);
  gn_finalize_kernel<false><<<cdiv(B * G, 4), 256, 0, st>>>(B, HW, C, G, nchunks, eps, (const float*)ws, stats);
  if (silu)
    gn_apply_fwd_kernel<true><<<dim3(nchunks, B), threads, 0, st>>>(HW, rows, C, G, (const bf16_t*)x, stats,
                                                                    (const bf16_t*)gamma, (const bf16_t*)beta,
                                                                    (bf16_t*)y);
  else
    gn_apply_fwd_kernel<false><<<dim3(nchunks, B), threads, 0, st>>>(HW, rows, C, G, (const bf16_t*)x, stats,
                                                                     (const bf16_t*)gamma, (const bf16_t*)beta,
                                                                     (bf16_t*)y);
  return pso_check_launch("pso_group_norm_fwd");
}

int pso_group_norm_bwd(int B, int HW, int C, int G, const void* x, const void* dy, const float* stats,
                       const void* gamma, const void* beta, int silu, const void* dadd, void* dx, float* dgamma,
                       float* dbeta, int accumulate_dparams, void* ws, size_t ws_bytes, void* stream) {
  PSO_ARG_CHECK(B > 0 && HW > 0 && C > 0 && G > 0 && C % G == 0 && C % 8 == 0 && C <= 4096,
                "pso_group_norm_bwd: bad shape");
  PSO_ARG_CHECK(x && dy && stats && dx && ws, "pso_group_norm_bwd: null pointer");
  PSO_ARG_CHECK(ws_bytes >= pso_group_norm_ws_bytes(B, HW, C), "pso_group_norm_bwd: workspace too small");
  hipStream_t st = (hipStream_t)stream;
  const int nchunks = cdiv(HW, GN_ROWS);
  const int threads = gn_block(C);
  const size_t shm = (size_t)(threads / (C / 8)) * C * 2 * sizeof(float);
  const size_t half = (size_t)B * nchunks * C * 2;
  float* part = (float*)ws;
  float* part_ch = (dgamma || dbeta) ? part + half : nullptr;
  float* coef = part + 2 * half;
  const bf16_t *xp = (const bf16_t*)x, *dyp = (const bf16_t*)dy, *gp = (const bf16_t*)gamma,
               *bp = (const bf16_t*)beta;
  if (silu)
    gn_partial_kernel<true, true><<<dim3(nchunks, B), threads, shm, st>>>(HW, GN_ROWS, C, G, xp, dyp, stats, gp, bp,
                                                                          part, part_ch);
  else
    gn_partial_kernel<true, false><<<dim3(nchunks, B), threads, shm, st>>>(HW, GN_ROWS, C, G, xp, dyp, stats, gp, bp,
                                                                           part, part_ch);
  gn_finalize_kernel<true><<<cdiv(B * G, 4), 256, 0, st>>>(B, HW, C, G, nchunks, 0.f, part, coef);
  if (dgamma || dbeta) {
    const int BK = B * nchunks, S = BK >= 64 ? 32 : BK / 2;
    if (S >= 2) {
      gn_dparam_split_kernel<<<dim3(cdiv(C, 64), S), 256, 0, st>>>(BK, C, S, part_ch, (double*)part);
      gn_dparam_final_kernel<<<cdiv(C, 128), 128, 0, st>>>(C, S, (const double*)part, dgamma, dbeta,
                                                           accumulate_dparams);
    } else {
      gn_dparam_kernel<<<cdiv(C, 128), 128, 0, st>>>(B, C, nchunks, part_ch, dgamma, dbeta, accumulate_dparams);
    }
  }
  if (silu)
    gn_apply_bwd_kernel<true><<<dim3(nchunks, B), threads, 0, st>>>(HW, C, G, xp, dyp, stats, coef, gp, bp,
                                                                    (const bf16_t*)dadd, (bf16_t*)dx);
  else
    gn_apply_bwd_kernel<false><<<dim3(nchunks, B), threads, 0, st>>>(HW, C, G, xp, dyp, stats, coef, gp, bp,
                                                                     (const bf16_t*)dadd, (bf16_t*)dx);
  return pso_check_launch("pso_group_norm_bwd");
}

int pso_layer_norm_fwd(int M, int C, float eps, const void* x, long ldx, const void* gamma, const void* beta, void* y,
                       long ldy, float* stats, void* stream) {
  PSO_ARG_CHECK(M >= 0 && C > 0 && C % 8 == 0 && C <= 64 * 8 * 4, "pso_layer_norm_fwd: C=%d unsupported", C);
  PSO_ARG_CHECK(x && y && gamma && beta, "pso_layer_norm_fwd: null pointer");
  PSO_ARG_CHECK(ln_aligned16(x, ldx) && ln_aligned16(y, ldy) && ln_aligned16(gamma, 0) && ln_aligned16(beta, 0),
                "pso_layer_norm_fwd: x, y, gamma, beta need 16-B aligned rows (pointers, and ld % 8 == 0)");
  if (M == 0) return PSO_OK;
  hipStream_t st = (hipStream_t)stream;
  const int C8 = C / 8;
  const int grid = cdiv(M, 4);
  if (C8 <= 64)
    ln_fwd_kernel<1><<<grid, 256, 0, st>>>(M, C, eps, (const bf16_t*)x, ldx, (const bf16_t*)gamma,
                                          (const bf16_t*)beta, (bf16_t*)y, ldy, stats);
  else if (C8 <= 128)
    ln_fwd_kernel<2><<<grid, 256, 0, st>>>(M, C, eps, (const bf16_t*)x, ldx, (const bf16_t*)gamma,
                                          (const bf16_t*)beta, (bf16_t*)y, ldy, stats);
  else
    ln_fwd_kernel<4><<<grid, 256, 0, st>>>(M, C, eps, (const bf16_t*)x, ldx, (const bf16_t*)gamma,
                                          (const bf16_t*)beta, (bf16_t*)y, ldy, stats);
  return pso_check_launch("pso_layer_norm_fwd");
}

int pso_layer_norm_bwd(int M, int C, const void* x, long ldx, const void* dy, long lddy, const float* stats,
                       const void* gamma, const void* dadd, long ldadd, void* dx, long lddx, void* stream) {
  PSO_ARG_CHECK(M >= 0 && C > 0 && C % 8 == 0 && C <= 64 * 8 * 4, "pso_layer_norm_bwd: C=%d unsupported", C);
  PSO_ARG_CHECK(x && dy && stats && gamma && dx, "pso_layer_norm_bwd: null pointer");
  PSO_ARG_CHECK(ln_aligned16(x, ldx) && ln_aligned16(dy, lddy) && ln_aligned16(gamma, 0) && ln_aligned16(dx, lddx) &&
                    (!dadd || ln_aligned16(dadd, ldadd)),
                "pso_layer_norm_bwd: x, dy, gamma, dadd, dx need 16-B aligned rows (pointers, and ld % 8 == 0)");
  if (M == 0) return PSO_OK;
  hipStream_t st = (hipStream_t)stream;
  const int C8 = C / 8;
  const int grid = cdiv(M, 4);
  if (C8 <= 64)
    ln_bwd_kernel<1><<<grid, 256, 0, st>>>(M, C, (const bf16_t*)x, ldx, (const bf16_t*)dy, lddy, stats,
                                          (const bf16_t*)gamma, (const bf16_t*)dadd, ldadd, (bf16_t*)dx, lddx);
  else if (C8 <= 128)
    ln_bwd_kernel<2><<<grid, 256, 0, st>>>(M, C, (const bf16_t*)x, ldx, (const bf16_t*)dy, lddy, stats,
                                          (const bf16_t*)gamma, (const bf16_t*)dadd, ldadd, (bf16_t*)dx, lddx);
  else
    ln_bwd_kernel<4><<<grid, 256, 0, st>>>(M, C, (const bf16_t*)x, ldx, (const bf16_t*)dy, lddy, stats,
                                          (const bf16_t*)gamma, (const bf16_t*)dadd, ldadd, (bf16_t*)dx, lddx);
  return pso_check_launch("pso_layer_norm_bwd");
}

}
```

pairwise_sample_optimization_amd/kernels.py:

```python
import ctypes
import math
import os

import torch

from . import _lib
from ._lib import check, lib, ptr, require_cuda, stream_ptr, dtype_code, PSO_BF16, PSO_F32

CONV_NORMAL, CONV_UP2, CONV_T2 = 1, 2, 3
ELEM = _lib.ELEM_DTYPE

PROFILE = None


def _prof_begin():
    if PROFILE is None:
        return None
    e0 = torch.cuda.Event(enable_timing=True)
    e0.record()
    return e0


def _prof_end(e0, flops, nbytes=0.0, tag=None):
    if e0 is not None:
# ... 256 lines not shown
    return None


class TnRankQueue:

    deterministic = os.environ.get("PSO_TN_DETERMINISTIC", "1") != "0"

    def __init__(self):
        self.pending = {}

    def add(self, a, b, out, alpha=1.0, group=0):
        M, I = a.shape
        J = b.shape[1]
        r = J * group // I if group else J
        assert b.shape[0] == M and out.shape == (I, r) and out.dtype == torch.float32
        form = _tn_rank_form(a, b, group)
        if form is None:
            return gemm_tn(a, b, out, alpha, group)
        key, x, u, R, gc = form
        require_cuda(x, u, out)
        prob = _lib.PsoTnRankProblem(ptr(x), _row_stride(x), ptr(u), _row_stride(u), ptr(out), _row_stride(out),
                                     M, x.shape[1], gc, float(alpha))
        self.pending.setdefault(key, []).append((prob, (x, u, out), 2.0 * M * I * r, 2.0 * M * (I + J) + 8.0 * I * r))
        return out

    def flush(self):
        for (R, ojc), items in self.pending.items():
            arr = (_lib.PsoTnRankProblem * len(items))(*[it[0] for it in items])
            e0 = _prof_begin()
            if TnRankQueue.deterministic:
                wsb = lib().pso_gemm_tn_rank_batch_ws_bytes(R, ojc, len(items), arr)
                ws = torch.empty(max(int(wsb), 16), device=items[0][1][2].device, dtype=torch.uint8)
                check(lib().pso_gemm_tn_rank_batch_ws(R, ojc, len(items), arr, ptr(ws), ws.numel(), stream_ptr()),
                      "pso_gemm_tn_rank_batch_ws")
            else:
                check(lib().pso_gemm_tn_rank_batch(R, ojc, len(items), arr, stream_ptr()), "pso_gemm_tn_rank_batch")
            _prof_end(e0, sum(it[2] for it in items), sum(it[3] for it in items), ("gemm_tn_batch", R, ojc, len(items)))
        self.pending = {}


def conv2d(x, weight, *, x2=None, mode=CONV_NORMAL, stride=1, pad=None, out_hw=None, bias=None, rowbias=None,
           resid=None, a2=None, w2=None, alpha=1.0, out=None, out_dtype=ELEM, accumulate=False):
    require_cuda(x, weight)
    B, H, W, C1 = x.shape
    C2 = x2.shape[3] if x2 is not None else 0
    Cout, ks, ks2, Ct = weight.shape
    assert ks == ks2 and Ct == C1 + C2 and x.is_contiguous() and weight.is_contiguous()
    if pad is None:
        pad = ks // 2
    if out_hw is None:
        if mode == CONV_UP2:
            out_hw = (2 * H, 2 * W)
        elif mode == CONV_T2:
            out_hw = (2 * H, 2 * W)
        else:
            out_hw = ((H + 2 * pad - ks) // stride + 1, (W + 2 * pad - ks) // stride + 1)
    Ho, Wo = out_hw
    if out is None:
        out = torch.empty((B, Ho, Wo, Cout), device=x.device, dtype=out_dtype)
    K2 = a2.shape[1] if a2 is not None else 0
    o2 = out.view(B * Ho * Wo, -1) if out.is_contiguous() else None
    ldo = Cout if o2 is None else o2.stride(0)
    key = ("conv", B, Ho, Wo, Cout, ks * ks * Ct, K2)
    wsb = _GEMM_WS.get(key)
    if wsb is None:
        wsb = _GEMM_WS[key] = int(lib().pso_conv2d_ws_bytes(B, Ho, Wo, Cout, ks * ks * Ct, K2))
    args = (mode, B, ptr(x), C1, ptr(x2), C2, H, W, Ho, Wo, ks, stride, pad, ptr(weight), Cout,
            ptr(a2), _row_stride(a2) if a2 is not None else 0, K2,
            ptr(w2), _row_stride(w2) if w2 is not None else 0, float(alpha), ptr(bias),
            ptr(rowbias), rowbias.stride(0) if rowbias is not None else 0,
            ptr(resid), Cout if resid is not None else 0, ptr(out), ldo, dtype_code(out), int(accumulate))
    e0 = _prof_begin()
    if wsb:
        ws = torch.empty(wsb, device=x.device, dtype=torch.uint8)
        check(lib().pso_conv2d_ws(*args, ptr(ws), wsb, stream_ptr()), "pso_conv2d_ws")
    else:
        check(lib().pso_conv2d(*args, stream_ptr()), "pso_conv2d")
    _prof_end(e0, 2.0 * B * Ho * Wo * Cout * (ks * ks * (C1 + C2) + K2),
              2.0 * (B * H * W * (C1 + C2) + Cout * ks * ks * (C1 + C2) + B * Ho * Wo * K2 + Cout * K2)
              + out.element_size() * B * Ho * Wo * Cout, ("conv", mode, B, H, W, C1, C2, Cout, ks, stride, K2))
    return out


def step_logprob(mode, sample, eps, coef, prev=None, noise=None, noise_shared=False):
    require_cuda(sample, eps, coef, prev, noise)
    B = sample.shape[0]
    n = sample[0].numel()
    sample = sample.contiguous()
    eps = eps.contiguous()
    lp = torch.empty(B, device=sample.device, dtype=torch.float32)
    prev_out = None if prev is not None else torch.empty_like(sample, dtype=torch.float32)
    ws_bytes = lib().pso_step_logprob_ws_bytes(B, n)
    ws = torch.empty(ws_bytes, device=sample.device, dtype=torch.uint8)
    check(lib().pso_step_logprob(mode, B, n, ptr(sample), ptr(eps), dtype_code(eps),
                                 ptr(prev.contiguous()) if prev is not None else None,
                                 ptr(noise.contiguous()) if noise is not None else None, int(noise_shared),
                                 ptr(coef.contiguous()), ptr(prev_out), ptr(lp), ptr(ws), ws_bytes, stream_ptr()),
          "pso_step_logprob")
    return (prev if prev is not None else prev_out), lp


def pair_loss_ws(P, n, device):
    return torch.empty(lib().pso_pair_loss_ws_bytes(P, n), device=device, dtype=torch.uint8)


def _check_pair_operands(x, x_prev, eps_pol, coef, pref, eps_ref=None):
    require_cuda(x, x_prev, eps_pol, eps_ref, coef, pref)
    if x.dtype != torch.float32 or x_prev.dtype != torch.float32:
        raise _lib.PsoLibError("pair loss: x / x_prev must be float32")
    if x.shape != x_prev.shape or x.shape != eps_pol.shape or (eps_ref is not None and eps_ref.shape != x.shape):
        raise _lib.PsoLibError(f"pair loss: shape mismatch x {tuple(x.shape)} x_prev {tuple(x_prev.shape)} "
                               f"eps_pol {tuple(eps_pol.shape)}" +
                               (f" eps_ref {tuple(eps_ref.shape)}" if eps_ref is not None else ""))
    if eps_ref is not None and eps_ref.dtype != eps_pol.dtype:
        raise _lib.PsoLibError(f"pair loss: eps_pol {eps_pol.dtype} and eps_ref {eps_ref.dtype} differ")
    dtype_code(eps_pol)
    if x.shape[0] % 2:
        raise _lib.PsoLibError("pair loss: batch must be 2P images (pair p, member k at row 2p + k)")
    P = x.shape[0] // 2
    if coef.dtype != torch.float32 or tuple(coef.shape) != (2 * P, _lib.COEF_STRIDE):
        raise _lib.PsoLibError(f"pair loss: coef must be float32 [{2 * P}, {_lib.COEF_STRIDE}]")
    if pref.dtype != torch.float32 or tuple(pref.shape) != (P, 2):
        raise _lib.PsoLibError(f"pair loss: pref must be float32 [{P}, 2]")
    for t in (x, x_prev, eps_pol, eps_ref, coef, pref):
        if t is not None and not t.is_contiguous():
            raise _lib.PsoLibError("pair loss: operands must be contiguous")


def pair_loss_fwd(mode, x, x_prev, eps_pol, eps_ref, coef, pref, beta, clip_eps, ws):
    _check_pair_operands(x, x_prev, eps_pol, coef, pref, eps_ref)
    P = x.shape[0] // 2
    n = x[0].numel()
    lp = torch.empty((2 * P, 2), device=x.device, dtype=torch.float32)
    loss = torch.empty((), device=x.device, dtype=torch.float32)
    check(lib().pso_pair_loss_fwd(mode, P, n, ptr(x), ptr(x_prev), ptr(eps_pol), ptr(eps_ref), dtype_code(eps_pol),
                                  ptr(coef), ptr(pref), float(beta), float(clip_eps), ptr(lp), ptr(loss), ptr(ws),
                                  ws.numel(), stream_ptr()), "pso_pair_loss_fwd")
    return loss, lp


def pair_loss_bwd(mode, x, x_prev, eps_pol, coef, pref, beta, clip_eps, ws, grad_out=None, grad_scale=1.0,
                  out_dtype=ELEM):
    _check_pair_operands(x, x_prev, eps_pol, coef, pref)
    P = x.shape[0] // 2
    n = x[0].numel()
    deps = torch.empty(eps_pol.shape, device=x.device, dtype=out_dtype)
    check(lib().pso_pair_loss_bwd(mode, P, n, ptr(x), ptr(x_prev), ptr(eps_pol), dtype_code(eps_pol), ptr(coef),
                                  ptr(pref), float(beta), float(clip_eps), ptr(grad_out), float(grad_scale),
                                  ptr(deps), dtype_code(deps), ptr(ws), ws.numel(), stream_ptr()),
          "pso_pair_loss_bwd")
    return deps


def pair_loss_from_lp(mode, lp_pol, lp_ref, pref, beta, clip_eps):
    require_cuda(lp_pol, lp_ref, pref)
    P = lp_pol.shape[0]
    for t in (lp_pol, lp_ref, pref):
        assert t.dtype == torch.float32 and tuple(t.shape) == (P, 2)
    loss = torch.empty((), device=lp_pol.device, dtype=torch.float32)
    dlp = torch.empty((P, 2), device=lp_pol.device, dtype=torch.float32)
    check(lib().pso_pair_loss_from_lp(mode, P, ptr(lp_pol.contiguous()), ptr(lp_ref.contiguous()),
                                      ptr(pref.contiguous()), float(beta), float(clip_eps), ptr(loss), ptr(dlp),
                                      stream_ptr()), "pso_pair_loss_from_lp")
    return loss, dlp


DB_SIGMOID, DB_HINGE = 0, 1


def db_loss_ws(B, n, device):
    return torch.empty(lib().pso_db_loss_ws_bytes(B, n), device=device, dtype=torch.uint8)


def db_loss_fwd(loss_type, eps, noisy, x0, sigma, beta, neg_defactor, prior_w, ws, eps_ref=None):
    B2 = eps.shape[0]
    n = eps[0].numel()
    B = B2 // 2
    losses = torch.empty((2 * B2 if eps_ref is not None else B2,), device=eps.device, dtype=torch.float32)
    logits = torch.empty((B,), device=eps.device, dtype=torch.float32)
    loss = torch.empty((), device=eps.device, dtype=torch.float32)
    check(lib().pso_db_loss_fwd(loss_type, B, n, ptr(eps), ptr(eps_ref), dtype_code(eps), ptr(noisy), ptr(x0),
                                ptr(sigma), float(beta), float(neg_defactor), float(prior_w), ptr(losses), ptr(logits),
                                ptr(loss), ptr(ws), ws.numel(), stream_ptr()), "pso_db_loss_fwd")
    return loss, losses, logits


def db_loss_bwd(loss_type, eps, noisy, x0, sigma, beta, neg_defactor, prior_w, ws, grad_out=None, grad_scale=1.0,
                out_dtype=ELEM):
    B = eps.shape[0] // 2
    n = eps[0].numel()
    deps = torch.empty(eps.shape, device=eps.device, dtype=out_dtype)
    check(lib().pso_db_loss_bwd(loss_type, B, n, ptr(eps), dtype_code(eps), ptr(noisy), ptr(x0), ptr(sigma),
                                float(beta), float(neg_defactor), float(prior_w), ptr(grad_out), float(grad_scale),
                                ptr(deps), dtype_code(deps), ptr(ws), ws.numel(), stream_ptr()), "pso_db_loss_bwd")
    return deps


def _norm_out(out, like, rows_contiguous):
    if out is None:
        if rows_contiguous:
            return torch.empty_like(like)
        return torch.empty(like.shape, device=like.device, dtype=like.dtype)
    require_cuda(out)
    assert out.shape == like.shape and out.dtype == like.dtype, (out.shape, out.dtype, like.shape, like.dtype)
    assert not rows_contiguous or out.is_contiguous(), "GroupNorm writes contiguous NHWC rows"
    return out


def group_norm_fwd(x, gamma, beta, groups, eps, silu, out=None):
    B, C = x.shape[0], x.shape[-1]
    HW = x.numel() // (B * C)
    y = _norm_out(out, x, True)
    stats = torch.empty((B, groups, 2), device=x.device, dtype=torch.float32)
    wsb = lib().pso_group_norm_ws_bytes(B, HW, C)
    ws = torch.empty(wsb, device=x.device, dtype=torch.uint8)
    check(lib().pso_group_norm_fwd(B, HW, C, groups, float(eps), ptr(x), ptr(gamma), ptr(beta), int(silu), ptr(y),
                                   ptr(stats), ptr(ws), wsb, stream_ptr()), "pso_group_norm_fwd")
    return y, stats


def group_norm_bwd(x, dy, stats, gamma, beta, silu, dadd=None, dgamma=None, dbeta=None, accumulate=False, out=None):
    B, C = x.shape[0], x.shape[-1]
    G = stats.shape[1]
    HW = x.numel() // (B * C)
    dx = _norm_out(out, x, True)
    wsb = lib().pso_group_norm_ws_bytes(B, HW, C)
    ws = torch.empty(wsb, device=x.device, dtype=torch.uint8)
    check(lib().pso_group_norm_bwd(B, HW, C, G, ptr(x), ptr(dy.contiguous()), ptr(stats), ptr(gamma), ptr(beta),
                                   int(silu), ptr(dadd), ptr(dx), ptr(dgamma), ptr(dbeta), int(accumulate), ptr(ws),
                                   wsb, stream_ptr()), "pso_group_norm_bwd")
    return dx


def layer_norm_fwd(x, gamma, beta, eps, out=None):
    M, C = x.shape
    y = _norm_out(out, x, False)
    stats = torch.empty((M, 2), device=x.device, dtype=torch.float32)
    check(lib().pso_layer_norm_fwd(M, C, float(eps), ptr(x), _row_stride(x), ptr(gamma), ptr(beta), ptr(y),
                                   _row_stride(y), ptr(stats), stream_ptr()), "pso_layer_norm_fwd")
    return y, stats


def layer_norm_bwd(x, dy, stats, gamma, dadd=None, out=None):
    M, C = x.shape
    dx = _norm_out(out, x, False)
    check(lib().pso_layer_norm_bwd(M, C, ptr(x), _row_stride(x), ptr(dy), _row_stride(dy), ptr(stats), ptr(gamma),
                                   ptr(dadd), _row_stride(dadd) if dadd is not None else 0, ptr(dx), _row_stride(dx),
                                   stream_ptr()), "pso_layer_norm_bwd")
    return dx


def _bsd(t):
    assert t.dim() == 3 and t.stride(2) == 1
    return t.stride(1), t.stride(0)


def attention_fwd(q, k, v, heads, scale=None, out=None):
    B, Sq, C = q.shape
    Sk = k.shape[1]
    assert C == heads * 64
    if scale is None:
        scale = 64 ** -0.5
    if out is None:
        out = torch.empty((B, Sq, C), device=q.device, dtype=q.dtype)
    lse = torch.empty((B, heads, Sq), device=q.device, dtype=torch.float32)
    (ldq, sqb), (ldk, skb), (ldv, svb), (ldo, sob) = _bsd(q), _bsd(k), _bsd(v), _bsd(out)
    check(lib().pso_attention_fwd(B, heads, Sq, Sk, ptr(q), ldq, sqb, ptr(k), ldk, skb, ptr(v), ldv, svb,
                                  float(scale), ptr(out), ldo, sob, ptr(lse), stream_ptr()), "pso_attention_fwd")
    return out, lse


def attention_bwd(q, k, v, o, lse, do, heads, scale=None, dq=None, dk=None, dv=None):
    B, Sq, C = q.shape
    Sk = k.shape[1]
    if scale is None:
        scale = 64 ** -0.5
    dq = torch.empty_like(q, memory_format=torch.contiguous_format) if dq is None else dq
    dk = torch.empty((B, Sk, C), device=q.device, dtype=q.dtype) if dk is None else dk
    dv = torch.empty((B, Sk, C), device=q.device, dtype=q.dtype) if dv is None else dv
    if Sk <= 256:
        assert dk.stride(0) == Sk * dk.stride(1) and dv.stride(0) == Sk * dv.stride(1)
    wsb = lib().pso_attention_bwd_ws_bytes(B, heads, Sq, Sk)
    ws = torch.empty(wsb, device=q.device, dtype=torch.uint8)
    do = do.contiguous()
    a = [_bsd(t) for t in (q, k, v, o, do, dq, dk, dv)]
    check(lib().pso_attention_bwd(B, heads, Sq, Sk, ptr(q), *a[0], ptr(k), *a[1], ptr(v), *a[2], ptr(o), *a[3],
                                  ptr(lse), ptr(do), *a[4], float(scale), ptr(dq), *a[5], ptr(dk), *a[6], ptr(dv),
                                  *a[7], ptr(ws), wsb, stream_ptr()), "pso_attention_bwd")
    return dq, dk, dv


def geglu_fwd(h):
    M, F2 = h.shape
    F = F2 // 2
    out = torch.empty((M, F), device=h.device, dtype=h.dtype)
    check(lib().pso_geglu_fwd(M, F, ptr(h), _row_stride(h), ptr(out), F, stream_ptr()), "pso_geglu_fwd")
    return out


def geglu_bwd(h, dout):
    M, F2 = h.shape
    F = F2 // 2
    din = torch.empty((M, F2), device=h.device, dtype=h.dtype)
    check(lib().pso_geglu_bwd(M, F, ptr(h), _row_stride(h), ptr(dout), _row_stride(dout), ptr(din), F2,
                              stream_ptr()), "pso_geglu_bwd")
    return din


def silu(x):
    y = torch.empty_like(x)
    check(lib().pso_silu(x.numel(), ptr(x.contiguous()), ptr(y), stream_ptr()), "pso_silu")
    return y


def timestep_embedding(t, dim, out=None, out_col=0):
    t = t.reshape(-1).float().contiguous()
# ... 79 lines not shown

_FULLGRAD_ATOMIC = os.environ.get("PSO_FULLGRAD_ATOMIC", "0") == "1"
_STREAM_WS = {}


def _stream_ws(nbytes, device):
    key = (device.index, torch.cuda.current_stream(device).cuda_stream)
    ws = _STREAM_WS.get(key)
    if ws is None or ws.numel() < nbytes:
        ws = _STREAM_WS[key] = torch.empty(max(int(nbytes * 1.25), 1 << 16), device=device, dtype=torch.uint8)
    return ws


def colsum_acc(x, out, rows_per_group=None):
    M, N = x.shape
    rpg = M if rows_per_group is None else rows_per_group
    if _FULLGRAD_ATOMIC:
        check(lib().pso_colsum_acc(M, N, ptr(x), _row_stride(x), rpg, ptr(out),
                                   out.stride(0) if out.dim() > 1 else N, stream_ptr()), "pso_colsum_acc")
        return out
    wsb = int(lib().pso_colsum_acc_ws_bytes(M, N, rpg))
    ws = _stream_ws(wsb, x.device)
    check(lib().pso_colsum_acc_ws(M, N, ptr(x), _row_stride(x), rpg, ptr(out), out.stride(0) if out.dim() > 1 else N,
                                  ptr(ws), ws.numel(), stream_ptr()), "pso_colsum_acc_ws")
    return out


def layer_norm_dparam(x, dy, stats, dgamma, dbeta):
    M, C = x.shape
    if _FULLGRAD_ATOMIC:
        check(lib().pso_layer_norm_dparam(M, C, ptr(x), _row_stride(x), ptr(dy), _row_stride(dy), ptr(stats),
                                          ptr(dgamma), ptr(dbeta), stream_ptr()), "pso_layer_norm_dparam")
        return
    wsb = int(lib().pso_layer_norm_dparam_ws_bytes(M, C))
    ws = _stream_ws(wsb, x.device)
    check(lib().pso_layer_norm_dparam_ws(M, C, ptr(x), _row_stride(x), ptr(dy), _row_stride(dy), ptr(stats),
                                         ptr(dgamma), ptr(dbeta), ptr(ws), ws.numel(), stream_ptr()),
          "pso_layer_norm_dparam_ws")


def im2col_conv(x, x2=None, mode=CONV_NORMAL, stride=1, pad=1, out_hw=None):
    B, H, W, C1 = x.shape
    C2 = x2.shape[3] if x2 is not None else 0
    if out_hw is None:
        out_hw = (2 * H, 2 * W) if mode == CONV_UP2 else ((H + 2 * pad - 3) // stride + 1, (W + 2 * pad - 3) // stride + 1)
    Ho, Wo = out_hw
    out = torch.empty((B * Ho * Wo, 9 * (C1 + C2)), device=x.device, dtype=ELEM)
    check(lib().pso_im2col_conv(mode, B, ptr(x.contiguous()), C1, ptr(x2.contiguous()) if x2 is not None else None, C2,
                                H, W, Ho, Wo, stride, pad, ptr(out), out.stride(0), stream_ptr()), "pso_im2col_conv")
    return out


def add(x, z):
    return axpby(1.0, x, 1.0, z)


def cast_f32_bf16(x, scale=1.0, out=None):
    out = torch.empty(x.shape, device=x.device, dtype=ELEM) if out is None else out
    check(lib().pso_cast_f32_bf16(x.numel(), ptr(x.contiguous()), float(scale), ptr(out), stream_ptr()),
          "pso_cast_f32_bf16")
    return out


def cast_bf16_f32(x, out=None):
    out = torch.empty(x.shape, device=x.device, dtype=torch.float32) if out is None else out
    check(lib().pso_cast_bf16_f32(x.numel(), ptr(x.contiguous()), ptr(out), stream_ptr()), "pso_cast_bf16_f32")
    return out


def conv_weight_t(w, flip):
    Co, ks, _, Ci = w.shape
    out = torch.empty((Ci, ks, ks, Co), device=w.device, dtype=w.dtype)
    check(lib().pso_conv_weight_t(Co, ks, Ci, int(flip), ptr(w.contiguous()), ptr(out), stream_ptr()),
          "pso_conv_weight_t")
    return out


def concat_channels(x1, x2):
    C1, C2 = x1.shape[-1], x2.shape[-1]
    out = torch.empty(x1.shape[:-1] + (C1 + C2,), device=x1.device, dtype=x1.dtype)
    npix = x1.numel() // C1
    check(lib().pso_concat_channels(npix, C1, ptr(x1.contiguous()), C2, ptr(x2.contiguous()), ptr(out),
                                    stream_ptr()), "pso_concat_channels")
    return out


def split_channels(x, C1, add2=None):
    C = x.shape[-1]
    C2 = C - C1
    y1 = torch.empty(x.shape[:-1] + (C1,), device=x.device, dtype=x.dtype)
    y2 = torch.empty(x.shape[:-1] + (C2,), device=x.device, dtype=x.dtype)
    npix = x.numel() // C
    check(lib().pso_split_channels(npix, C1, C2, ptr(x.contiguous()), ptr(y1), ptr(y2),
                                   ptr(add2.contiguous()) if add2 is not None else None, stream_ptr()),
          "pso_split_channels")
    return y1, y2


def nchw_to_nhwc(x, pad_to=None, scale=1.0):
    B, C, H, W = x.shape
    Cp = pad_to or C
    out = torch.empty((B, H, W, Cp), device=x.device, dtype=ELEM)
    check(lib().pso_nchw_to_nhwc(B, C, Cp, H * W, ptr(x.contiguous()), dtype_code(x), float(scale), ptr(out),
                                 stream_ptr()), "pso_nchw_to_nhwc")
    return out


def softmax_rows(x):
    M, N = x.shape
    check(lib().pso_softmax_rows(M, N, ptr(x), _row_stride(x), stream_ptr()), "pso_softmax_rows")
    return x


def nhwc_to_nchw(x, dtype=torch.float32):
    B, H, W, C = x.shape
    out = torch.empty((B, C, H, W), device=x.device, dtype=dtype)
    check(lib().pso_nhwc_to_nchw(B, C, H * W, ptr(x.contiguous()), ptr(out), dtype_code(out), stream_ptr()),
          "pso_nhwc_to_nchw")
    return out


def grad_clip_coef(grad, max_norm, grad_scale=1.0, out=None):
    n = grad.numel()
    out = torch.empty(2, device=grad.device, dtype=torch.float32) if out is None else out
    wsb = lib().pso_grad_clip_ws_bytes(n)
    ws = torch.empty(wsb, device=grad.device, dtype=torch.uint8)
    check(lib().pso_grad_clip_coef(n, ptr(grad), float(grad_scale), float(max_norm), ptr(out), ptr(ws), wsb,
                                   stream_ptr()), "pso_grad_clip_coef")
    return out


def adamw_step(param, grad, exp_avg, exp_avg_sq, lr, betas, eps, weight_decay, step, grad_scale=1.0, clip=None):
    check(lib().pso_adamw_step(param.numel(), ptr(param), ptr(grad), ptr(exp_avg), ptr(exp_avg_sq), float(lr),
                               float(betas[0]), float(betas[1]), float(eps), float(weight_decay), int(step),
                               float(grad_scale), ptr(clip), stream_ptr()), "pso_adamw_step")


class Adam8State:

    BLOCK = 2048
    MIN_8BIT_SIZE = 4096

    def __init__(self, n, device, segments=None):
        self.n = n
        self.qm = torch.zeros(n, dtype=torch.uint8, device=device)
        self.qv = torch.zeros(n, dtype=torch.uint8, device=device)
        self.desc = None
        self.m32 = self.v32 = None
        if segments is None:
            nb = lib().pso_adamw8bit_blocks(n)
            self.block_start = None
        else:
            rows, n32 = [], 0
            for off, k in sorted(segments):
                assert 0 <= off and off + k <= n, (off, k, n)
                if k < self.MIN_8BIT_SIZE:
                    for b0 in range(0, k, self.BLOCK):
                        rows.append((off + b0, min(self.BLOCK, k - b0), n32 + b0, 0))
                    n32 += -(-k // 8) * 8
                else:
                    for b0 in range(0, k, self.BLOCK):
                        rows.append((off + b0, min(self.BLOCK, k - b0), -1, 0))
            for (o1, l1, _, _), (o2, _, _, _) in zip(rows, rows[1:]):
                assert o1 + l1 <= o2, "parameter segments overlap"
            nb = len(rows)
            self.desc = torch.tensor(rows, dtype=torch.int64).to(device)
# ... 541 lines not shown
```

pairwise_sample_optimization_amd/unet.py:

```python
import math
import os
from dataclasses import dataclass, field, replace
from types import SimpleNamespace

import torch
import torch.nn as nn

from . import _lib
from . import kernels as K

ELEM = _lib.ELEM_DTYPE
TN_BATCH = os.environ.get("PSO_TN_BATCH", "1") != "0"


@dataclass
class UNetConfig:
    in_channels: int = 4
    out_channels: int = 4
    block_out_channels: tuple = (320, 640, 1280)
    layers_per_block: int = 2
    transformer_layers_per_block: tuple = (1, 2, 10)
    down_has_attn: tuple = (False, True, True)
    head_dim: int = 64
    cross_attention_dim: int = 2048
# ... 907 lines not shown

    def __init__(self, C, depth, cross_dim, groups):
        super().__init__()
        self.C, self.groups = C, groups
        self.norm = Norm(C)
        self.proj_in = Linear(C, C)
        self.transformer_blocks = nn.ModuleList([BasicTransformerBlock(C, cross_dim) for _ in range(depth)])
        self.proj_out = Linear(C, C)

    def prepare(self):
        self.proj_in.prepare()
        self.proj_out.prepare()
        for b in self.transformer_blocks:
            b.prepare()

    def fwd(self, x, rt, path):
        B, H, W, C = x.shape
        xn, st = K.group_norm_fwd(x, self.norm.weight, self.norm.bias, self.groups, 1e-6, False)
        h = K.gemm(xn.view(-1, C), self.proj_in.weight, bias=self.proj_in.bias)
        if rt.save:
            rt.saved.append({"x": rt.pol(x), "st": rt.pol(st), "xn": xn.view(-1, C) if rt.fg is not None else None})
        for i, blk in enumerate(self.transformer_blocks):
            h = blk.fwd(h, rt, f"{path}.transformer_blocks.{i}")
        if rt.save and rt.fg is not None:
            rt.saved.append({"hout": h})
        return K.gemm(h, self.proj_out.weight, bias=self.proj_out.bias, resid=x.view(-1, C)).view(B, H, W, C)

    def bwd(self, dy, rt, path, need_dx=True):
        B, H, W, C = dy.shape
        d2 = dy.view(-1, C)
        fg = rt.fg
        if fg is not None:
            _lin_dw(fg, self.proj_out, d2, rt.saved.pop()["hout"], rt)
        dh = K.gemm(d2, self.proj_out.wt)
        for i in reversed(range(len(self.transformer_blocks))):
            dh = self.transformer_blocks[i].bwd(dh, rt.saved.pop(), rt, f"{path}.transformer_blocks.{i}",
                                                need_dx=need_dx or i > 0)
        sv = rt.saved.pop()
        if not need_dx:
            return None
        dn = K.gemm(dh, self.proj_in.wt).view(B, H, W, C)
        if fg is not None:
            _lin_dw(fg, self.proj_in, dh, sv["xn"], rt)
            return K.group_norm_bwd(sv["x"], dn, sv["st"], self.norm.weight, self.norm.bias, False, dadd=dy,
                                    dgamma=fg.g(self.norm.weight), dbeta=fg.g(self.norm.bias), accumulate=True)
        return K.group_norm_bwd(sv["x"], dn, sv["st"], self.norm.weight, self.norm.bias, False, dadd=dy)


class ResnetBlock2D(nn.Module):
    def __init__(self, cin, cout, groups, eps, temb_dim):
        super().__init__()
        self.cin, self.cout, self.groups, self.eps = cin, cout, groups, eps
        self.norm1 = Norm(cin)
        self.conv1 = Conv2d(cin, cout, 3)
        self.time_emb_proj = Linear(temb_dim, cout) if temb_dim else None
        self.norm2 = Norm(cout)
        self.conv2 = Conv2d(cout, cout, 3)
        self.conv_shortcut = Conv2d(cin, cout, 1) if cin != cout else None

    def prepare(self):
        self.conv1.prepare()
        self.conv2.prepare()
        if self.conv_shortcut is not None:
            self.conv_shortcut.prepare()

    def fwd(self, x, rt, temb=None):
        h1, st1 = K.group_norm_fwd(x, self.norm1.weight, self.norm1.bias, self.groups, self.eps, True)
        c1 = K.conv2d(h1, self.conv1.w_nhwc, bias=self.conv1.bias, rowbias=temb)
        h2, st2 = K.group_norm_fwd(c1, self.norm2.weight, self.norm2.bias, self.groups, self.eps, True)
        if self.conv_shortcut is not None:
            B, H, W, _ = x.shape
            sc = K.gemm(x.view(-1, self.cin), self.conv_shortcut.w_mat, bias=self.conv_shortcut.bias)
            sc = sc.view(B, H, W, self.cout)
        else:
            sc = x
        out = K.conv2d(h2, self.conv2.w_nhwc, bias=self.conv2.bias, resid=sc)
        if rt.save:
            sv = {"x": rt.pol(x), "st1": rt.pol(st1), "c1": rt.pol(c1), "st2": rt.pol(st2)}
            if rt.fg is not None:
                sv.update(h1=h1, h2=h2)
            rt.saved.append(sv)
        return out

    def bwd(self, dout, rt):
        sv = rt.saved.pop()
        fg = rt.fg
        B, H, W, _ = dout.shape
        dh2 = K.conv2d(dout, self.conv2.w_dx)
        if fg is not None:
            _conv_dw(fg, self.conv2, dout.view(-1, self.cout), sv["h2"], rt, K.im2col_conv)
            dc1 = K.group_norm_bwd(sv["c1"], dh2, sv["st2"], self.norm2.weight, self.norm2.bias, True,
                                   dgamma=fg.g(self.norm2.weight), dbeta=fg.g(self.norm2.bias), accumulate=True)
            dc2 = dc1.view(-1, self.cout)
            _conv_dw(fg, self.conv1, dc2, sv["h1"], rt, K.im2col_conv)
            K.colsum_acc(dc2, rt.dtemb[:, self._temb_off:self._temb_off + self.cout], rows_per_group=H * W)
        else:
            dc1 = K.group_norm_bwd(sv["c1"], dh2, sv["st2"], self.norm2.weight, self.norm2.bias, True)
        dh1 = K.conv2d(dc1, self.conv1.w_dx)
        if self.conv_shortcut is not None:
            dsc = K.gemm(dout.view(-1, self.cout), self.conv_shortcut.wt).view(B, H, W, self.cin)
            if fg is not None:
                d2, x2 = dout.view(-1, self.cout), sv["x"].view(-1, self.cin)
                sc = self.conv_shortcut

                def sc_dw():
                    K.gemm_tn(d2, x2, fg.g(sc.weight).view(self.cout, self.cin))
                    K.colsum_acc(d2, fg.g(sc.bias).view(1, -1))
                rt.side.launch(sc_dw, d2, x2)
        else:
            dsc = dout
        if fg is not None:
            return K.group_norm_bwd(sv["x"], dh1, sv["st1"], self.norm1.weight, self.norm1.bias, True, dadd=dsc,
                                    dgamma=fg.g(self.norm1.weight), dbeta=fg.g(self.norm1.bias), accumulate=True)
        return K.group_norm_bwd(sv["x"], dh1, sv["st1"], self.norm1.weight, self.norm1.bias, True, dadd=dsc)


class Downsample2D(nn.Module):
    def __init__(self, C):
        super().__init__()
        self.conv = Conv2d(C, C, 3, stride=2)

    def prepare(self):
        self.conv.prepare()

    def fwd(self, x, rt):
        if rt.save:
            rt.saved.append({"hw": x.shape[1:3], "x": x if rt.fg is not None else None})
        return K.conv2d(x, self.conv.w_nhwc, stride=2, bias=self.conv.bias)

    def bwd(self, dy, rt):
        sv = rt.saved.pop()
        if rt.fg is not None:
            _conv_dw(rt.fg, self.conv, dy.reshape(-1, self.conv.cout), sv["x"], rt,
                     lambda x: K.im2col_conv(x, stride=2))
        return K.conv2d(dy, self.conv.w_dx, mode=K.CONV_T2, out_hw=tuple(sv["hw"]))


class Upsample2D(nn.Module):
    def __init__(self, C):
        super().__init__()
        self.conv = Conv2d(C, C, 3)

    def prepare(self):
        self.conv.prepare()

    def fwd(self, x, rt):
        if rt.save and rt.fg is not None:
            rt.saved.append({"x": x})
        return K.conv2d(x, self.conv.w_nhwc, mode=K.CONV_UP2, bias=self.conv.bias)

    def bwd(self, dy, rt):
        if rt.fg is not None:
            _conv_dw(rt.fg, self.conv, dy.reshape(-1, self.conv.cout), rt.saved.pop()["x"], rt,
                     lambda x: K.im2col_conv(x, mode=K.CONV_UP2))
        du = K.conv2d(dy, self.conv.w_dx)
        return K.sumpool2(du)


class _Block(nn.Module):

    def __init__(self):
        super().__init__()


class TimestepEmbedding(nn.Module):
    def __init__(self, fin, dim):
        super().__init__()
        self.linear_1 = Linear(fin, dim)
        self.linear_2 = Linear(dim, dim)


class _Output(SimpleNamespace):
    pass


class UNet2DConditionModel(nn.Module):
    def __init__(self, config: UNetConfig = None):
        super().__init__()
        cfg = config or UNetConfig.sdxl()
        self.cfg = cfg
        self.config = SimpleNamespace(in_channels=cfg.in_channels, out_channels=cfg.out_channels,
                                      sample_size=cfg.sample_size, block_out_channels=cfg.block_out_channels,
                                      cross_attention_dim=cfg.cross_attention_dim,
                                      addition_time_embed_dim=cfg.addition_time_embed_dim,
                                      projection_class_embeddings_input_dim=cfg.projection_class_embeddings_input_dim)
        ch = cfg.block_out_channels
        G, eps, tdim = cfg.norm_num_groups, cfg.norm_eps, cfg.time_embed_dim
        self.conv_in = Conv2d(cfg.in_channels, ch[0], 3)
        self.time_embedding = TimestepEmbedding(cfg.time_proj_dim, tdim)
        self.add_embedding = TimestepEmbedding(cfg.projection_class_embeddings_input_dim, tdim)
        nlev = len(ch)
        self.down_blocks = nn.ModuleList()
        cin = ch[0]
        for i in range(nlev):
            blk = _Block()
            blk.resnets = nn.ModuleList()
            if cfg.down_has_attn[i]:
                blk.attentions = nn.ModuleList()
            for j in range(cfg.layers_per_block):
                blk.resnets.append(ResnetBlock2D(cin if j == 0 else ch[i], ch[i], G, eps, tdim))
                if cfg.down_has_attn[i]:
                    blk.attentions.append(Transformer2DModel(ch[i], cfg.transformer_layers_per_block[i],
                                                             cfg.cross_attention_dim, G))
            if i < nlev - 1:
                blk.downsamplers = nn.ModuleList([Downsample2D(ch[i])])
            cin = ch[i]
            self.down_blocks.append(blk)
        mid = _Block()
        mid.resnets = nn.ModuleList([ResnetBlock2D(ch[-1], ch[-1], G, eps, tdim),
                                     ResnetBlock2D(ch[-1], ch[-1], G, eps, tdim)])
        mid.attentions = nn.ModuleList([Transformer2DModel(ch[-1], cfg.transformer_layers_per_block[-1],
                                                           cfg.cross_attention_dim, G)])
        self.mid_block = mid
        self.up_blocks = nn.ModuleList()
        rch = list(reversed(ch))
        rattn = list(reversed(cfg.down_has_attn))
        rdepth = list(reversed(cfg.transformer_layers_per_block))
        prev = ch[-1]
        for i in range(nlev):
            out_c = rch[i]
            in_c = rch[min(i + 1, nlev - 1)]
            blk = _Block()
            blk.resnets = nn.ModuleList()
            if rattn[i]:
                blk.attentions = nn.ModuleList()
            n = cfg.layers_per_block + 1
            for j in range(n):
                skip_c = in_c if j == n - 1 else out_c
                res_in = prev if j == 0 else out_c
                blk.resnets.append(ResnetBlock2D(res_in + skip_c, out_c, G, eps, tdim))
                if rattn[i]:
                    blk.attentions.append(Transformer2DModel(out_c, rdepth[i], cfg.cross_attention_dim, G))
            if i < nlev - 1:
                blk.upsamplers = nn.ModuleList([Upsample2D(out_c)])
            prev = out_c
            self.up_blocks.append(blk)
        self.conv_norm_out = Norm(ch[0])
        self.conv_out = Conv2d(ch[0], cfg.out_channels, 3)
        self.lora = None
        self.full = None
        self.fp8 = False
        self._fp8_cache = {}
        self.lora_fused = False
        self._merged = None
        self._adapters_enabled = True
        self._prepared = False
        self.gradient_checkpointing = False

    def _remap_key(self, k):
        return k.replace(".ff.net.0.proj.", ".ff.proj.").replace(".ff.net.2.", ".ff.out.")

    def _unmap_key(self, k):
        return k.replace(".ff.proj.", ".ff.net.0.proj.").replace(".ff.out.", ".ff.net.2.")

    def state_dict(self, *a, **kw):
        sd = super().state_dict(*a, **kw)
        return {self._unmap_key(k): v for k, v in sd.items()}

    def load_state_dict(self, sd, strict=True):
        sd = {self._remap_key(k): v for k, v in sd.items()}
        res = super().load_state_dict({k: v.to(ELEM) for k, v in sd.items()}, strict=strict)
        self._prepared = False
        return res

    @classmethod
    def from_config(cls, config=None, **kw):
        from . import diffusers_io
        if config is None:
            config = UNetConfig.sdxl()
        elif isinstance(config, dict):
            config = diffusers_io.unet_config_from_diffusers(dict(config, **kw))
        elif not isinstance(config, UNetConfig):
            raise TypeError(f"from_config takes a UNetConfig or a diffusers config dict, not {type(config).__name__}")
        return cls(config)

    @classmethod
    def load_config(cls, path, subfolder=None, **kw):
        from . import diffusers_io
        return diffusers_io.load_config(path, subfolder)

    @classmethod
    def from_pretrained(cls, path, subfolder=None, torch_dtype=None, variant=None, revision=None, **kw):
        from . import diffusers_io
        model = cls.from_config(diffusers_io.load_config(path, subfolder))
        model.load_state_dict(diffusers_io.load_weights(path, subfolder, variant))
        return model

    def save_pretrained(self, path):
        from . import diffusers_io
        diffusers_io.save_pretrained(self, path, diffusers_io.unet_config_to_diffusers(self.cfg))

    def init_weights(self, seed=0):
        g = torch.Generator(device=self.conv_in.weight.device).manual_seed(seed)
        for m in self.modules():
            if isinstance(m, (Linear, Conv2d, Norm)):
                m.reset(g)
        self._prepared = False
        return self

    def enable_gradient_checkpointing(self):
        self.gradient_checkpointing = True

    def _attn_modules(self):
        for name, m in self.named_modules():
            if isinstance(m, BasicTransformerBlock):
                yield name, m

    def add_adapter(self, lora_config, allow_dora=False):
        r, alpha = check_lora_config(lora_config, allow_dora=allow_dora)
        dora = getattr(lora_config, "use_dora", False) is True
        if dora and self.fp8:
            raise ValueError("use_dora with the fp8 forward is not implemented: the e4m3 K-tail has no column scale")
        blocks = [(name, blk.dim, blk.attn2.kv_dim) for name, blk in self._attn_modules()]
        dev = self.conv_in.weight.device
        self.lora = LoraState(blocks, r, alpha, dev, dora=dora)
        self.lora_fused, self._merged = False, None
        if dev.type == "cuda":
            self.lora.bind_base(self._adapted_weights())
            self.lora.init_gaussian(seed=getattr(lora_config, "seed", 0))
            if dora:
                self.lora.init_magnitudes()
        self._adapters_enabled = True
        return self.lora

    def _adapted_weights(self):
        out = {}
        for name, blk in self._attn_modules():
            for a in ("attn1", "attn2"):
                m = getattr(blk, a)
                for mod, lin in (("to_q", m.to_q), ("to_k", m.to_k), ("to_v", m.to_v), ("to_out.0", m.to_out[0])):
# ... 203 lines not shown

    def kv_text(self, rt, C):
        hit = rt.kv_cache.get(C)
        if hit is not None:
            return hit
        grp = self._kv_groups[C]
        enc = rt.enc
        if rt.lora_on:
            A, sB = self.lora.kv_stacks[C][:2]
            u = K.gemm(rt.pol(enc), A)
            kv = _gemm_fwd(enc, grp.W, a2=u, w2=sB, tail_group_n=C, tail_rows=enc.shape[0] // 2 if rt.paired else 0)
            if rt.dora:
                rows = rt.pol(enc).shape[0]
                rt.kv_z[C] = kv[:rows]
                kv = K.dora_scale_fwd(kv, self.lora.kv_g[C], rows_policy=rows)
        else:
            u, kv = None, K.gemm(enc, rt.merged.kv[C] if rt.merged is not None else grp.W)
        rt.kv_cache[C] = (kv, u)
        return kv, u

    def _runtime(self, B, enc, save, lora_on):
        fg = self.full if save else None
        side = K.SideStream(enabled=True) if (fg is not None and _FULL_SIDE) else K.SideStream()
        rt = SimpleNamespace(B=B, enc=enc, save=save, saved=[], lora_on=lora_on, paired=False, side=side, fg=fg)
        rt.pol = lambda t: t[:t.shape[0] // 2] if rt.paired else t
        rt.kv_cache = {}
        rt.kv_text = lambda C: self.kv_text(rt, C)
        rt.lora = self.lora
        rt.r = self.lora.r_pad if lora_on else 0
        rt.fp8 = self._fp8_weight if self.fp8 else None
        rt.dora = lora_on and self.lora.dora
        rt.kv_z = {}
        rt.merged = None
        if rt.dora and self.fp8:
            raise ValueError("use_dora adapters with the fp8 forward are not implemented")
        return rt

    def _embed(self, timestep, time_ids, text_embeds, B, dev):
        cfg = self.cfg
        t = torch.as_tensor(timestep, device=dev).float().reshape(-1)
        if t.numel() == 1:
            t = t.expand(B).contiguous()
        te = K.timestep_embedding(t, cfg.time_proj_dim)
        l1, l2 = self.time_embedding.linear_1, self.time_embedding.linear_2
        t1 = K.gemm(te, l1.weight, bias=l1.bias)
        s1 = K.silu(t1)
        emb = K.gemm(s1, l2.weight, bias=l2.bias)
        tid = K.timestep_embedding(time_ids.reshape(-1), cfg.addition_time_embed_dim).view(B, -1)
        add_in = K.concat_channels(text_embeds.to(ELEM).contiguous(), tid)
        a1, a2 = self.add_embedding.linear_1, self.add_embedding.linear_2
        u1 = K.gemm(add_in, a1.weight, bias=a1.bias)
        s2 = K.silu(u1)
        emb = K.gemm(s2, a2.weight, bias=a2.bias, resid=emb)
        se = K.silu(emb)
        self._emb_saved = dict(te=te, t1=t1, s1=s1, add_in=add_in, u1=u1, s2=s2, emb=emb, se=se)
        return K.gemm(se, self._temb_w, bias=self._temb_b)

    def forward_nhwc(self, x, timestep, enc, text_embeds, time_ids, save=False, paired_ref=False):
        if not self._prepared:
            self.prepare()
        B = x.shape[0]
        lora_on = self.lora is not None and self._adapters_enabled
        encf = enc.to(ELEM).reshape(B * enc.shape[1], enc.shape[2]).contiguous()
        fused = lora_on and self.lora_fused and not save and not paired_ref
        rt = self._runtime(B, encf, save, lora_on and not fused)
        if fused:
            rt.merged = self._merged
        temb_all = self._embed(timestep, time_ids, text_embeds, B, x.device)
        tb = lambda m: temb_all[:, m._temb_off:m._temb_off + m.cout]
        _, H, W, _ = x.shape
        cols = K.im2col3(x, self.conv_in.kp)
        h = K.gemm(cols, self.conv_in.w_col, bias=self.conv_in.bias).view(B, H, W, -1)
        skips = [h]
        i0, j0 = self._first_attn
        full = rt.fg is not None
        if full and paired_ref:
            raise ValueError("full-UNet training: the reference is a separate frozen UNet, not the adapter-free pass")
        if full:
            rt.emb = self._emb_saved
            rt.cols_in = cols
            i0, j0 = -1, -1
        else:
            rt.save = False
        for i, blk in enumerate(self.down_blocks):
            for j, res in enumerate(blk.resnets):
                if (i, j) == (i0, j0):
                    rt.save = save
                    if paired_ref:
                        dup = lambda t: torch.cat([t, t], 0)
                        h = dup(h)
                        skips = [dup(s_) for s_ in skips]
                        temb_all = dup(temb_all)
                        rt.enc = dup(rt.enc)
                        rt.B = 2 * B
                        rt.paired = True
                h = res.fwd(h, rt, tb(res))
                if hasattr(blk, "attentions"):
                    h = blk.attentions[j].fwd(h, rt, f"down_blocks.{i}.attentions.{j}")
                skips.append(h)
            if hasattr(blk, "downsamplers"):
                h = blk.downsamplers[0].fwd(h, rt)
                skips.append(h)
        m = self.mid_block
        h = m.resnets[0].fwd(h, rt, tb(m.resnets[0]))
        h = m.attentions[0].fwd(h, rt, "mid_block.attentions.0")
        h = m.resnets[1].fwd(h, rt, tb(m.resnets[1]))
        for i, blk in enumerate(self.up_blocks):
            for j, res in enumerate(blk.resnets):
                s = skips.pop()
                hc = K.concat_channels(h, s)
                if rt.save:
                    rt.saved.append({"c1": h.shape[-1]})
                h = res.fwd(hc, rt, tb(res))
                if hasattr(blk, "attentions"):
                    h = blk.attentions[j].fwd(h, rt, f"up_blocks.{i}.attentions.{j}")
            if hasattr(blk, "upsamplers"):
                h = blk.upsamplers[0].fwd(h, rt)
        hn, st = K.group_norm_fwd(h, self.conv_norm_out.weight, self.conv_norm_out.bias, self.cfg.norm_num_groups,
                                  self.cfg.norm_eps, True)
        out = K.conv2d(hn, self.conv_out.w_nhwc, bias=self.conv_out.bias)
        if save:
            rt.saved.append({"h": rt.pol(h), "st": rt.pol(st), "hn": hn if full else None})
        rt.B = B
        rt.enc = rt.pol(rt.enc)
        rt.paired = False
        return out, rt

    def backward_nhwc(self, dout, rt):
        B = dout.shape[0]
        sv = rt.saved.pop()
        fg = rt.fg
        _, H, W, _ = dout.shape
        cols = K.im2col3(dout.contiguous(), self.conv_out.kp_dx)
        dhn = K.gemm(cols, self.conv_out.w_dx_col).view(B, H, W, -1)
        if fg is not None:
            rt.dtemb = torch.zeros((B, self._temb_n), device=dout.device, dtype=torch.float32)
            co = self.conv_out.cout
            dy8 = torch.zeros((B * H * W, 8), device=dout.device, dtype=ELEM)
            dy8[:, :co] = dout.reshape(-1, co)
            _conv_dw(fg, self.conv_out, dy8, sv["hn"], rt, K.im2col_conv)
            dh = K.group_norm_bwd(sv["h"], dhn, sv["st"], self.conv_norm_out.weight, self.conv_norm_out.bias, True,
                                  dgamma=fg.g(self.conv_norm_out.weight), dbeta=fg.g(self.conv_norm_out.bias),
                                  accumulate=True)
        else:
            dh = K.group_norm_bwd(sv["h"], dhn, sv["st"], self.conv_norm_out.weight, self.conv_norm_out.bias, True)
        unit_done = getattr(rt, "unit_done", None) or (lambda unit: None)
        dwq = K.TnRankQueue() if TN_BATCH else None
        rt.dw = dwq.add if dwq is not None else K.gemm_tn

        lora = self.lora if rt.lora_on and self.lora.grad_pad is not None else None

        def done(unit):
            if dwq is not None:
                dwq.flush()
            if lora is not None and lora.fold_range(unit):
                rt.side.launch(lambda: lora.fold_grads(unit))
            unit_done(unit)

        done("conv_out")
        skip_grads = []
        for i in reversed(range(len(self.up_blocks))):
            blk = self.up_blocks[i]
            if hasattr(blk, "upsamplers"):
                dh = blk.upsamplers[0].bwd(dh, rt)
                done(f"up_blocks.{i}.upsamplers.0")
            for j in reversed(range(len(blk.resnets))):
                if hasattr(blk, "attentions"):
                    dh = blk.attentions[j].bwd(dh, rt, f"up_blocks.{i}.attentions.{j}")
                    done(f"up_blocks.{i}.attentions.{j}")
                dhc = blk.resnets[j].bwd(dh, rt)
                done(f"up_blocks.{i}.resnets.{j}")
                c1 = rt.saved.pop()["c1"]
                dh, ds = K.split_channels(dhc, c1)
                skip_grads.append(ds)
        m = self.mid_block
        dh = m.resnets[1].bwd(dh, rt)
        done("mid_block.resnets.1")
        dh = m.attentions[0].bwd(dh, rt, "mid_block.attentions.0")
        done("mid_block.attentions.0")
        dh = m.resnets[0].bwd(dh, rt)
        done("mid_block.resnets.0")
        i0, j0 = self._first_attn if fg is None else (0, -1)
        for i in reversed(range(i0, len(self.down_blocks))):
            blk = self.down_blocks[i]
            if hasattr(blk, "downsamplers"):
                dh = K.add(dh, skip_grads.pop())
                dh = blk.downsamplers[0].bwd(dh, rt)
                done(f"down_blocks.{i}.downsamplers.0")
            for j in reversed(range(len(blk.resnets))):
                dh = K.add(dh, skip_grads.pop())
                if (i, j) == (i0, j0):
                    blk.attentions[j].bwd(dh, rt, f"down_blocks.{i}.attentions.{j}", need_dx=False)
                    done(f"down_blocks.{i}.attentions.{j}")
                    break
                if hasattr(blk, "attentions"):
                    dh = blk.attentions[j].bwd(dh, rt, f"down_blocks.{i}.attentions.{j}")
                    done(f"down_blocks.{i}.attentions.{j}")
                dh = blk.resnets[j].bwd(dh, rt)
                done(f"down_blocks.{i}.resnets.{j}")
        if fg is not None:
            dh = K.add(dh, skip_grads.pop())
            self._conv_in_dw(fg, dh, rt)
            self._embed_bwd(fg, rt)
            done("embed")
        rt.saved.clear()
        if dwq is not None:
            dwq.flush()
        rt.side.join()
        return None

    def _conv_in_dw(self, fg, dh, rt):
        ci = self.conv_in
        tmp = torch.zeros((ci.cout, ci.kp), device=dh.device, dtype=torch.float32)
        d2 = dh.reshape(-1, ci.cout)
        K.gemm_tn(d2, rt.cols_in, tmp)
        fg.g(ci.weight).add_(tmp[:, :9 * ci.cin].view(ci.cout, 3, 3, ci.cin).permute(0, 3, 1, 2))
        K.colsum_acc(d2, fg.g(ci.bias).view(1, -1))

    def _embed_bwd(self, fg, rt):
        e = rt.emb
        dt = K.cast_f32_bf16(rt.dtemb)
        res = [m for m in self.modules() if isinstance(m, ResnetBlock2D)]
        gw = _stacked([fg.g(m.time_emb_proj.weight) for m in res])
        gb = _stacked([fg.g(m.time_emb_proj.bias) for m in res])
        if gw.data_ptr() == fg.g(res[0].time_emb_proj.weight).data_ptr() and \
                gb.data_ptr() == fg.g(res[0].time_emb_proj.bias).data_ptr():
            K.gemm_tn(dt, e["se"], gw)
            gb.add_(rt.dtemb.sum(0))
        else:
            tmp = torch.zeros((self._temb_n, e["se"].shape[1]), device=dt.device, dtype=torch.float32)
            K.gemm_tn(dt, e["se"], tmp)
            for m in res:
                fg.g(m.time_emb_proj.weight).add_(tmp[m._temb_off:m._temb_off + m.cout])
                fg.g(m.time_emb_proj.bias).add_(rt.dtemb[:, m._temb_off:m._temb_off + m.cout].sum(0))

        def silu_bwd(dy, x):
            xf = x.float()
            sg = torch.sigmoid(xf)
            return (dy.float() * sg * (1 + xf * (1 - sg))).to(ELEM)

        demb = silu_bwd(K.gemm(dt, self._temb_wt), e["emb"])
        a1, a2 = self.add_embedding.linear_1, self.add_embedding.linear_2
        _lin_dw(fg, a2, demb, e["s2"])
        du1 = silu_bwd(K.gemm(demb, a2.wt), e["u1"])
        _lin_dw(fg, a1, du1, e["add_in"])
        l1, l2 = self.time_embedding.linear_1, self.time_embedding.linear_2
        _lin_dw(fg, l2, demb, e["s1"])
        dt1 = silu_bwd(K.gemm(demb, l2.wt), e["t1"])
        _lin_dw(fg, l1, dt1, e["te"])

    @property
    def _first_attn(self):
        for i, blk in enumerate(self.down_blocks):
            if hasattr(blk, "attentions"):
                return i, 0
        raise ValueError("UNet without attention blocks has no adapter to train")

# ... 43 lines not shown
```

Measured before the change: 38.80 imgs/s.

## Skip duplicating prefix skip activations and prune dead skip-gradient columns in UNet backward

In the paired-reference path, skip tensors from blocks before the gradient entry point are no longer duplicated. Instead a wrap-around concat kernel reads them modulo batch. In backward, up-block resnets fed by such dead skips compute only the live input-channel columns of the conv1 and shortcut dgrad. They use new column-subset GEMM/conv entry points that reuse the full product's tile plan. A fused group-norm backward reads the two concat halves directly and writes split outputs, removing the concat-grad and split_channels round trip. This adds layout/plan constraints with fallbacks, and adds complexity to the saved-state bookkeeping.

```diff
diff --git a/include/pso_amd.h b/include/pso_amd.h
--- a/include/pso_amd.h
+++ b/include/pso_amd.h
@@ -124,12 +124,21 @@
                   const void* resid, long ldr, void* out, long ldo, int out_dtype, int accumulate, void* ws,
                   size_t ws_bytes, void* stream);
 
+int pso_gemm_cols(int M, int N, int plan_n, const void* a, long lda, int K, const void* w, long ldw, void* out, long ldo,
+                  void* stream);
+int pso_conv2d_cols(int B, const void* src, int C, int H, int W, const void* weight, int Cout, int plan_cout, void* out,
+                    long ldo, void* stream);
+
 size_t pso_group_norm_ws_bytes(int B, int HW, int C);
 int pso_group_norm_fwd(int B, int HW, int C, int G, float eps, const void* x, const void* gamma, const void* beta,
                        int silu, void* y, float* stats, void* ws, size_t ws_bytes, void* stream);
 int pso_group_norm_bwd(int B, int HW, int C, int G, const void* x, const void* dy, const float* stats,
                        const void* gamma, const void* beta, int silu, const void* dadd, void* dx, float* dgamma,
                        float* dbeta, int accumulate_dparams, void* ws, size_t ws_bytes, void* stream);
+int pso_group_norm_bwd_skip(int B, int HW, int C1, int C2, int G, const void* x1, long ldx1, const void* x2, long ldx2,
+                            int B2, const void* dy, int cdy, const float* stats, const void* gamma, const void* beta,
+                            int silu, const void* dadd, int cadd, void* d1, void* d2, void* ws, size_t ws_bytes,
+                            void* stream);
 
 int pso_layer_norm_fwd(int M, int C, float eps, const void* x, long ldx, const void* gamma, const void* beta, void* y,
                        long ldy, float* stats, void* stream);
@@ -189,6 +198,8 @@
 int pso_concat_channels(long npix, int C1, const void* x1, int C2, const void* x2, void* out, void* stream);
 int pso_split_channels(long npix, int C1, int C2, const void* in, void* y1, void* y2, const void* add2,
                        void* stream);
+int pso_concat_channels_wrap(long npix, int C1, const void* x1, int C2, const void* x2, long npix2, void* out,
+                             void* stream);
 
 size_t pso_grad_clip_ws_bytes(long n);
 int pso_grad_clip_coef(long n, const float* grad, float grad_scale, float max_norm, float* out_norm_coef, void* ws,
diff --git a/pairwise_sample_optimization_amd/_lib.py b/pairwise_sample_optimization_amd/_lib.py
--- a/pairwise_sample_optimization_amd/_lib.py
+++ b/pairwise_sample_optimization_amd/_lib.py
@@ -64,6 +64,8 @@
     "pso_gemm_ws_bytes": (csz, [ci, ci, ci, ci]),
     "pso_gemm_ws": (ci, [ci, ci, vp, cl, ci, vp, cl, vp, cl, ci, vp, cl, cf, vp, vp, cl, ci, vp, cl, vp, cl, ci, ci,
                          ci, ci, vp, csz, vp]),
+    "pso_gemm_cols": (ci, [ci, ci, ci, vp, cl, ci, vp, cl, vp, cl, vp]),
+    "pso_conv2d_cols": (ci, [ci, vp, ci, ci, ci, vp, ci, ci, vp, cl, vp]),
     "pso_gemm_batched": (ci, [ci, ci, ci, ci, vp, cl, cl, vp, cl, cl, cf, vp, cl, cl, ci, vp]),
     "pso_last_kernel": (ctypes.c_char_p, []),
     "pso_attention_small": (ci, [ci, ci, ci, ci, vp, cl, cl, vp, cl, cl, vp, cl, cl, ci, cf, vp, cl, cl, vp]),
@@ -97,6 +99,8 @@
     "pso_group_norm_ws_bytes": (csz, [ci, ci, ci]),
     "pso_group_norm_fwd": (ci, [ci, ci, ci, ci, cf, vp, vp, vp, ci, vp, vp, vp, csz, vp]),
     "pso_group_norm_bwd": (ci, [ci, ci, ci, ci, vp, vp, vp, vp, vp, ci, vp, vp, vp, vp, ci, vp, csz, vp]),
+    "pso_group_norm_bwd_skip": (ci, [ci, ci, ci, ci, ci, vp, cl, vp, cl, ci, vp, ci, vp, vp, vp, ci, vp, ci, vp, vp, vp,
+                                     csz, vp]),
     "pso_layer_norm_fwd": (ci, [ci, ci, cf, vp, cl, vp, vp, vp, cl, vp, vp]),
     "pso_layer_norm_bwd": (ci, [ci, ci, vp, cl, vp, cl, vp, vp, vp, cl, vp, cl, vp]),
     "pso_attention_fwd": (ci, [ci, ci, ci, ci, vp, cl, cl, vp, cl, cl, vp, cl, cl, cf, vp, cl, cl, vp, vp]),
@@ -169,6 +173,7 @@
     "pso_preference": (ci, [ci, ci, vp, vp, ci, vp, vp]),
     "pso_nhwc_to_nchw": (ci, [ci, ci, cl, vp, vp, ci, vp]),
     "pso_split_channels": (ci, [cl, ci, ci, vp, vp, vp, vp, vp]),
+    "pso_concat_channels_wrap": (ci, [cl, ci, vp, ci, vp, cl, vp, vp]),
 }
 
 
diff --git a/pairwise_sample_optimization_amd/csrc/elementwise.hip b/pairwise_sample_optimization_amd/csrc/elementwise.hip
--- a/pairwise_sample_optimization_amd/csrc/elementwise.hip
+++ b/pairwise_sample_optimization_amd/csrc/elementwise.hip
@@ -247,14 +247,15 @@
   }
 }
 
+template <bool WRAP>
 __global__ void concat_kernel(long npix, int C1, const bf16_t* __restrict__ x1, int C2, const bf16_t* __restrict__ x2,
-                              bf16_t* __restrict__ out) {
+                              bf16_t* __restrict__ out, long npix2) {
   const int C8 = (C1 + C2) / 8, c18 = C1 / 8;
   GRID_STRIDE(v, npix * C8) {
     const long p = v / C8;
     const int ch = (int)(v - p * C8);
     const uint4 val = ch < c18 ? *reinterpret_cast<const uint4*>(x1 + p * C1 + ch * 8)
-                               : *reinterpret_cast<const uint4*>(x2 + p * C2 + (ch - c18) * 8);
+                               : *reinterpret_cast<const uint4*>(x2 + (WRAP ? p % npix2 : p) * C2 + (ch - c18) * 8);
     *reinterpret_cast<uint4*>(out + v * 8) = val;
   }
 }
@@ -420,9 +421,19 @@
 
 int pso_concat_channels(long npix, int C1, const void* x1, int C2, const void* x2, void* out, void* stream) {
   PSO_ARG_CHECK(C1 % 8 == 0 && C2 % 8 == 0 && x1 && x2 && out, "pso_concat_channels: C %% 8");
-  concat_kernel<<<grid_for(npix * (C1 + C2) / 8), 256, 0, (hipStream_t)stream>>>(
-      npix, C1, (const bf16_t*)x1, C2, (const bf16_t*)x2, (bf16_t*)out);
+  concat_kernel<false><<<grid_for(npix * (C1 + C2) / 8), 256, 0, (hipStream_t)stream>>>(
+      npix, C1, (const bf16_t*)x1, C2, (const bf16_t*)x2, (bf16_t*)out, npix);
   return pso_check_launch("pso_concat_channels");
+}
+
+int pso_concat_channels_wrap(long npix, int C1, const void* x1, int C2, const void* x2, long npix2, void* out,
+                             void* stream) {
+  PSO_ARG_CHECK(C1 % 8 == 0 && C2 % 8 == 0 && x1 && x2 && out, "pso_concat_channels_wrap: C %% 8");
+  PSO_ARG_CHECK(npix2 > 0 && npix % npix2 == 0, "pso_concat_channels_wrap: npix=%ld is no multiple of npix2=%ld", npix,
+                npix2);
+  concat_kernel<true><<<grid_for(npix * (C1 + C2) / 8), 256, 0, (hipStream_t)stream>>>(
+      npix, C1, (const bf16_t*)x1, C2, (const bf16_t*)x2, (bf16_t*)out, npix2);
+  return pso_check_launch("pso_concat_channels_wrap");
 }
 
 int pso_split_channels(long npix, int C1, int C2, const void* in, void* y1, void* y2, const void* add2,
diff --git a/pairwise_sample_optimization_amd/csrc/gemm.hip b/pairwise_sample_optimization_amd/csrc/gemm.hip
--- a/pairwise_sample_optimization_amd/csrc/gemm.hip
+++ b/pairwise_sample_optimization_amd/csrc/gemm.hip
@@ -824,6 +824,19 @@
 
 static int run_gemm(GemmArgs& g, hipStream_t st, size_t ws_bytes = 0, bool small_conv_entry = false) {
   GemmFacts f = gemm_facts(g, ws_bytes, small_conv_entry);
+  if (g.plan_N > g.N) {
+    f.N = g.plan_N;
+    const GemmPlan p = gemm_plan(f, g_gemm_knobs);
+    const bool tiled = p.form == GF_TILE || p.form == GF_8P256 || p.form == GF_8P160 || p.form == GF_8P320 ||
+                       p.form == GF_8P320_CONV;
+    if (!tiled || p.ws_ks >= 2 || p.atomic_ks != 1 || p.BN <= 0 || (g.N % p.BN) != 0 ||
+        gemm_split_plan(g.M, g.plan_N, g.K1, g.K2, g.a2 != nullptr, g_gemm_knobs).ks >= 2) {
+      pso_set_error("pso_gemm_cols / pso_conv2d_cols: the first N columns are not whole tiles of the plain tiled form "
+                    "the whole product takes");
+      return PSO_ERR_ARG;
+    }
+    return run_plan(p, g, st);
+  }
   GemmPlan p = gemm_plan(f, g_gemm_knobs);
   if (p.form == GF_SMALL_CONV) {
     if (run_plan(p, g, st) == PSO_OK) return PSO_OK;
@@ -1343,6 +1356,28 @@
   return rc != PSO_OK ? rc : run_gemm(g, (hipStream_t)stream);
 }
 
+int pso_gemm_cols(int M, int N, int plan_n, const void* a, long lda, int K, const void* w, long ldw, void* out, long ldo,
+                  void* stream) {
+  PSO_ARG_CHECK(N > 0 && plan_n >= N, "pso_gemm_cols: need 0 < N <= plan_n (N=%d plan_n=%d)", N, plan_n);
+  GemmArgs g{};
+  const int rc = gemm_entry_args("pso_gemm_cols", g, M, N, a, lda, K, w, ldw, nullptr, 0, 0, nullptr, 0, 1.f, nullptr,
+                                 nullptr, 0, 1, nullptr, 0, out, ldo, PSO_ELEM, 0, 0, 0);
+  g.plan_N = plan_n;
+  return rc != PSO_OK ? rc : run_gemm(g, (hipStream_t)stream);
+}
+
+int pso_conv2d_cols(int B, const void* src, int C, int H, int W, const void* weight, int Cout, int plan_cout, void* out,
+                    long ldo, void* stream) {
+  PSO_ARG_CHECK(Cout > 0 && plan_cout >= Cout, "pso_conv2d_cols: need 0 < Cout <= plan_cout (Cout=%d plan_cout=%d)",
+                Cout, plan_cout);
+  GemmArgs g{};
+  const int rc = conv_entry_args("pso_conv2d_cols", g, PSO_CONV_NORMAL, B, src, C, nullptr, 0, H, W, H, W, 3, 1, 1,
+                                 weight, Cout, nullptr, 0, 0, nullptr, 0, 1.f, nullptr, nullptr, 0, nullptr, 0, out, ldo,
+                                 PSO_ELEM, 0);
+  g.plan_N = plan_cout;
+  return rc != PSO_OK ? rc : run_gemm(g, (hipStream_t)stream);
+}
+
 size_t pso_gemm_ws_bytes(int M, int N, int K1, int K2) {
   const SplitPlan sp = gemm_split_plan(M, N, K1, K2, K2 > 0, g_gemm_knobs);
   return sp.ks >= 2 ? (size_t)sp.ks * M * N * sizeof(float) : 0;
diff --git a/pairwise_sample_optimization_amd/csrc/gemm_args.h b/pairwise_sample_optimization_amd/csrc/gemm_args.h
--- a/pairwise_sample_optimization_amd/csrc/gemm_args.h
+++ b/pairwise_sample_optimization_amd/csrc/gemm_args.h
@@ -34,6 +34,7 @@
   long bat_a, bat_b, bat_o;
   int batch;
   float* ws;
+  int plan_N;
 };
 
 struct Gemm8Args {
diff --git a/pairwise_sample_optimization_amd/csrc/norm.hip b/pairwise_sample_optimization_amd/csrc/norm.hip
--- a/pairwise_sample_optimization_amd/csrc/norm.hip
+++ b/pairwise_sample_optimization_amd/csrc/norm.hip
@@ -17,10 +17,26 @@
 }
 __device__ __forceinline__ float sigmoidf_(float x) { return 1.0f / (1.0f + __expf(-x)); }
 
-template <bool BWD, bool SILU>
+struct GnSkip {
+  const bf16_t* x2;
+  long ldx1, ldx2;
+  int B2, C1;
+  int cdy, cadd;
+  int csum;
+  bf16_t* d2;
+};
+template <bool SKIP>
+__device__ __forceinline__ const bf16_t* gn_src(const bf16_t* x, const GnSkip& sk, int b, int HW, int r, int C, int c0) {
+  if (!SKIP) return x + ((size_t)b * HW + r) * C + c0;
+  return c0 < sk.C1 ? x + ((size_t)b * HW + r) * sk.ldx1 + c0
+                    : sk.x2 + ((size_t)(b % sk.B2) * HW + r) * sk.ldx2 + (c0 - sk.C1);
+}
+
+template <bool BWD, bool SILU, bool SKIP = false>
 __global__ void gn_partial_kernel(int HW, int rows, int C, int G, const bf16_t* __restrict__ x, const bf16_t* __restrict__ dy,
                                   const float* __restrict__ stats, const bf16_t* __restrict__ gamma,
-                                  const bf16_t* __restrict__ beta, float* __restrict__ ws, float* __restrict__ ws_ch) {
+                                  const bf16_t* __restrict__ beta, float* __restrict__ ws, float* __restrict__ ws_ch,
+                                  GnSkip sk = GnSkip{}) {
   extern __shared__ float red[];
   const int TPR = C / 8;
   const int RS = blockDim.x / TPR;
@@ -42,11 +58,11 @@
       bt[j] = beta ? bf2f(beta[c]) : 0.f;
     }
   }
-  if (slot < RS) {
+  if (slot < RS && (!SKIP || cc * 8 < sk.csum)) {
     for (int r = r0 + slot; r < r1; r += RS) {
-      const size_t off = ((size_t)b * HW + r) * C + cc * 8;
+      const size_t off = ((size_t)b * HW + r) * (SKIP ? sk.cdy : C) + cc * 8;
       float xv[8];
-      unpack8(*reinterpret_cast<const uint4*>(x + off), xv);
+      unpack8(*reinterpret_cast<const uint4*>(gn_src<SKIP>(x, sk, b, HW, r, C, cc * 8)), xv);
       if (!BWD) {
 #pragma unroll
         for (int j = 0; j < 8; ++j) {
@@ -223,15 +239,16 @@
   }
 }
 
-template <bool SILU>
+template <bool SILU, bool SKIP = false>
 __global__ void gn_apply_bwd_kernel(int HW, int C, int G, const bf16_t* __restrict__ x, const bf16_t* __restrict__ dy,
                                     const float* __restrict__ stats, const float* __restrict__ coef,
                                     const bf16_t* __restrict__ gamma, const bf16_t* __restrict__ beta,
-                                    const bf16_t* __restrict__ dadd, bf16_t* __restrict__ dx) {
+                                    const bf16_t* __restrict__ dadd, bf16_t* __restrict__ dx, GnSkip sk = GnSkip{}) {
   const int TPR = C / 8;
   const int RS = blockDim.x / TPR;
   const int slot = threadIdx.x / TPR, cc = threadIdx.x - slot * TPR;
   if (slot >= RS) return;
+  if (SKIP && cc * 8 >= sk.C1 && !sk.d2) return;
   const int b = blockIdx.y;
   const int r0 = blockIdx.x * GN_ROWS, r1 = min(HW, r0 + GN_ROWS);
   const int Cg = C / G;
@@ -251,11 +268,12 @@
     R[j] = -rstd * cb;
   }
   for (int r = r0 + slot; r < r1; r += RS) {
-    const size_t off = ((size_t)b * HW + r) * C + cc * 8;
+    const size_t pix = (size_t)b * HW + r;
+    const size_t off = pix * C + cc * 8;
     float xv[8], dv[8], o[8], av[8];
-    unpack8(*reinterpret_cast<const uint4*>(x + off), xv);
-    unpack8(*reinterpret_cast<const uint4*>(dy + off), dv);
-    if (dadd) unpack8(*reinterpret_cast<const uint4*>(dadd + off), av);
+    unpack8(*reinterpret_cast<const uint4*>(gn_src<SKIP>(x, sk, b, HW, r, C, cc * 8)), xv);
+    unpack8(*reinterpret_cast<const uint4*>(SKIP ? dy + pix * sk.cdy + cc * 8 : dy + off), dv);
+    if (dadd) unpack8(*reinterpret_cast<const uint4*>(SKIP ? dadd + pix * sk.cadd + cc * 8 : dadd + off), av);
 #pragma unroll
     for (int j = 0; j < 8; ++j) {
       const float xh = fmaf(xv[j], xs[j], xo[j]);
@@ -267,7 +285,9 @@
       }
       o[j] = fmaf(P[j], dz, fmaf(R[j], xh, Q[j])) + (dadd ? av[j] : 0.f);
     }
-    *reinterpret_cast<uint4*>(dx + off) = pack8(o);
+    bf16_t* dst = !SKIP ? dx + off
+                        : (cc * 8 < sk.C1 ? dx + pix * sk.C1 + cc * 8 : sk.d2 + pix * (C - sk.C1) + (cc * 8 - sk.C1));
+    *reinterpret_cast<uint4*>(dst) = pack8(o);
   }
 }
 
@@ -453,6 +473,52 @@
   return pso_check_launch("pso_group_norm_bwd");
 }
 
+int pso_group_norm_bwd_skip(int B, int HW, int C1, int C2, int G, const void* x1, long ldx1, const void* x2, long ldx2,
+                            int B2, const void* dy, int cdy, const float* stats, const void* gamma, const void* beta,
+                            int silu, const void* dadd, int cadd, void* d1, void* d2, void* ws, size_t ws_bytes,
+                            void* stream) {
+  const int C = C1 + C2;
+  PSO_ARG_CHECK(B > 0 && HW > 0 && C1 > 0 && C2 > 0 && G > 0 && C % G == 0 && C1 % 8 == 0 && C2 % 8 == 0 && C <= 4096 &&
+                    B2 > 0 && B2 <= B,
+                "pso_group_norm_bwd_skip: bad shape B=%d B2=%d HW=%d C1=%d C2=%d G=%d", B, B2, HW, C1, C2, G);
+  PSO_ARG_CHECK(x1 && x2 && dy && stats && d1 && ws, "pso_group_norm_bwd_skip: null pointer");
+  PSO_ARG_CHECK(ldx1 >= C1 && ldx2 >= C2 && ldx1 % 8 == 0 && ldx2 % 8 == 0 && ((uintptr_t)x1 & 15) == 0 &&
+                    ((uintptr_t)x2 & 15) == 0,
+                "pso_group_norm_bwd_skip: x1 / x2 need 16-B aligned rows of at least C1 / C2 channels");
+  PSO_ARG_CHECK(cdy == C || (cdy == C1 && !d2 && C1 % (C / G) == 0),
+                "pso_group_norm_bwd_skip: dy has C1 + C2 columns, or C1 with d2 null and C1 on a group boundary (cdy=%d)",
+                cdy);
+  PSO_ARG_CHECK(!dadd || cadd == C || (cadd == C1 && !d2),
+                "pso_group_norm_bwd_skip: dadd has C1 + C2 columns, or C1 with d2 null (cadd=%d)", cadd);
+  PSO_ARG_CHECK(ws_bytes >= pso_group_norm_ws_bytes(B, HW, C), "pso_group_norm_bwd_skip: workspace too small");
+  hipStream_t st = (hipStream_t)stream;
+  const int nchunks = cdiv(HW, GN_ROWS);
+  const int threads = gn_block(C);
+  const size_t shm = (size_t)(threads / (C / 8)) * C * 2 * sizeof(float);
+  const size_t half = (size_t)B * nchunks * C * 2;
+  float* part = (float*)ws;
+  float* coef = part + 2 * half;
+  const bf16_t *xp = (const bf16_t*)x1, *dyp = (const bf16_t*)dy, *gp = (const bf16_t*)gamma,
+               *bp = (const bf16_t*)beta;
+  const int Cg = C / G;
+  const int csum = d2 ? C : min(cdy, (cdiv(C1, Cg) * Cg + 7) / 8 * 8);
+  const GnSkip sk{(const bf16_t*)x2, ldx1, ldx2, B2, C1, cdy, dadd ? cadd : C, csum, (bf16_t*)d2};
+  if (silu)
+    gn_partial_kernel<true, true, true><<<dim3(nchunks, B), threads, shm, st>>>(HW, GN_ROWS, C, G, xp, dyp, stats, gp,
+                                                                                bp, part, nullptr, sk);
+  else
+    gn_partial_kernel<true, false, true><<<dim3(nchunks, B), threads, shm, st>>>(HW, GN_ROWS, C, G, xp, dyp, stats, gp,
+                                                                                 bp, part, nullptr, sk);
+  gn_finalize_kernel<true><<<cdiv(B * G, 4), 256, 0, st>>>(B, HW, C, G, nchunks, 0.f, part, coef);
+  if (silu)
+    gn_apply_bwd_kernel<true, true><<<dim3(nchunks, B), threads, 0, st>>>(HW, C, G, xp, dyp, stats, coef, gp, bp,
+                                                                          (const bf16_t*)dadd, (bf16_t*)d1, sk);
+  else
+    gn_apply_bwd_kernel<false, true><<<dim3(nchunks, B), threads, 0, st>>>(HW, C, G, xp, dyp, stats, coef, gp, bp,
+                                                                           (const bf16_t*)dadd, (bf16_t*)d1, sk);
+  return pso_check_launch("pso_group_norm_bwd_skip");
+}
+
 int pso_layer_norm_fwd(int M, int C, float eps, const void* x, long ldx, const void* gamma, const void* beta, void* y,
                        long ldy, float* stats, void* stream) {
   PSO_ARG_CHECK(M >= 0 && C > 0 && C % 8 == 0 && C <= 64 * 8 * 4, "pso_layer_norm_fwd: C=%d unsupported", C);
diff --git a/pairwise_sample_optimization_amd/kernels.py b/pairwise_sample_optimization_amd/kernels.py
--- a/pairwise_sample_optimization_amd/kernels.py
+++ b/pairwise_sample_optimization_amd/kernels.py
@@ -362,6 +362,39 @@
     return out
 
 
+_ERR_ARG = 1
+
+
+def gemm_cols(a, w, n):
+    require_cuda(a, w)
+    M, K1 = a.shape
+    N = w.shape[0]
+    if n < N:
+        out = torch.empty((M, n), device=a.device, dtype=ELEM)
+        rc = lib().pso_gemm_cols(M, n, N, ptr(a), _row_stride(a), K1, ptr(w), _row_stride(w), ptr(out), n,
+                                 stream_ptr())
+        if rc == 0:
+            return out
+        if rc != _ERR_ARG:
+            check(rc, "pso_gemm_cols")
+    return gemm(a, w)
+
+
+def conv2d_cols(x, weight, n):
+    require_cuda(x, weight)
+    B, H, W, C = x.shape
+    Cout = weight.shape[0]
+    assert weight.shape[1:] == (3, 3, C) and x.is_contiguous() and weight.is_contiguous()
+    if n < Cout:
+        out = torch.empty((B, H, W, n), device=x.device, dtype=ELEM)
+        rc = lib().pso_conv2d_cols(B, ptr(x), C, H, W, ptr(weight), n, Cout, ptr(out), n, stream_ptr())
+        if rc == 0:
+            return out
+        if rc != _ERR_ARG:
+            check(rc, "pso_conv2d_cols")
+    return conv2d(x, weight)
+
+
 def step_logprob(mode, sample, eps, coef, prev=None, noise=None, noise_shared=False):
     require_cuda(sample, eps, coef, prev, noise)
     B = sample.shape[0]
@@ -512,6 +545,34 @@
     return dx
 
 
+def _skip_part(t):
+    C, ld = t.shape[-1], t.stride(-2)
+    if t.stride(-1) == 1 and ld >= C and all(t.stride(i) == t.stride(i + 1) * t.shape[i + 1] for i in range(t.dim() - 2)):
+        return t, ld
+    return t.contiguous(), C
+
+
+def group_norm_bwd_skip(x1, x2, dy, stats, gamma, beta, silu, dadd=None, want_d2=True):
+    B, B2, C1, C2 = x1.shape[0], x2.shape[0], x1.shape[-1], x2.shape[-1]
+    C, G = C1 + C2, stats.shape[1]
+    HW = math.prod(x1.shape[1:-1])
+    x1, ld1 = _skip_part(x1)
+    x2, ld2 = _skip_part(x2)
+    dy = dy.contiguous()
+    cdy, cadd = dy.shape[-1], C
+    d1 = torch.empty(tuple(x1.shape[:-1]) + (C1,), device=x1.device, dtype=x1.dtype)
+    d2 = torch.empty((B,) + tuple(x2.shape[1:-1]) + (C2,), device=x1.device, dtype=x1.dtype) if want_d2 else None
+    if dadd is not None:
+        dadd = dadd.contiguous()
+        cadd = dadd.shape[-1]
+    wsb = lib().pso_group_norm_ws_bytes(B, HW, C)
+    ws = torch.empty(wsb, device=x1.device, dtype=torch.uint8)
+    check(lib().pso_group_norm_bwd_skip(B, HW, C1, C2, G, ptr(x1), ld1, ptr(x2), ld2, B2, ptr(dy), cdy, ptr(stats),
+                                        ptr(gamma), ptr(beta), int(silu), ptr(dadd), cadd, ptr(d1), ptr(d2), ptr(ws),
+                                        wsb, stream_ptr()), "pso_group_norm_bwd_skip")
+    return d1, d2
+
+
 def layer_norm_fwd(x, gamma, beta, eps, out=None):
     M, C = x.shape
     y = _norm_out(out, x, False)
@@ -757,6 +818,15 @@
     npix = x1.numel() // C1
     check(lib().pso_concat_channels(npix, C1, ptr(x1.contiguous()), C2, ptr(x2.contiguous()), ptr(out),
                                     stream_ptr()), "pso_concat_channels")
+    return out
+
+
+def concat_channels_wrap(x1, x2):
+    C1, C2 = x1.shape[-1], x2.shape[-1]
+    assert x1.shape[1:-1] == x2.shape[1:-1] and x1.shape[0] % x2.shape[0] == 0, (x1.shape, x2.shape)
+    out = torch.empty(x1.shape[:-1] + (C1 + C2,), device=x1.device, dtype=x1.dtype)
+    check(lib().pso_concat_channels_wrap(x1.numel() // C1, C1, ptr(x1.contiguous()), C2, ptr(x2.contiguous()),
+                                         x2.numel() // C2, ptr(out), stream_ptr()), "pso_concat_channels_wrap")
     return out
 
 
diff --git a/pairwise_sample_optimization_amd/unet.py b/pairwise_sample_optimization_amd/unet.py
--- a/pairwise_sample_optimization_amd/unet.py
+++ b/pairwise_sample_optimization_amd/unet.py
@@ -1013,6 +1013,21 @@
             rt.saved.append(sv)
         return out
 
+    def bwd_skip(self, dout, rt, c1, dead):
+        sv = rt.saved.pop()
+        B, H, W, _ = dout.shape
+        sc = self.conv_shortcut
+        assert rt.fg is None and sc is not None
+        dh2 = K.conv2d(dout, self.conv2.w_dx)
+        dc1 = K.group_norm_bwd(sv["c1"], dh2, sv["st2"], self.norm2.weight, self.norm2.bias, True)
+        n1 = c1 if dead and c1 % (self.cin // self.groups) == 0 else self.cin
+        na = c1 if dead else self.cin
+        dh1 = K.conv2d_cols(dc1, self.conv1.w_dx, n1)
+        dsc = K.gemm_cols(dout.view(-1, self.cout), sc.wt, na).view(B, H, W, -1)
+        x = sv["x"]
+        return K.group_norm_bwd_skip(x[..., :c1], x[..., c1:], dh1, sv["st1"], self.norm1.weight, self.norm1.bias,
+                                     True, dadd=dsc, want_d2=not dead)
+
     def bwd(self, dout, rt):
         sv = rt.saved.pop()
         fg = rt.fg
@@ -1177,6 +1192,7 @@
         self._adapters_enabled = True
         self._prepared = False
         self.gradient_checkpointing = False
+        self.materialize_skips = False
 
     def _remap_key(self, k):
         return k.replace(".ff.net.0.proj.", ".ff.proj.").replace(".ff.net.2.", ".ff.out.")
@@ -1546,19 +1562,27 @@
             i0, j0 = -1, -1
         else:
             rt.save = False
+        lean = not full and not self.materialize_skips
+        n_prefix = 0
         for i, blk in enumerate(self.down_blocks):
             for j, res in enumerate(blk.resnets):
-                if (i, j) == (i0, j0):
+                enter = (i, j) == (i0, j0)
+                if enter and lean:
+                    n_prefix = len(skips)
+                    h = res.fwd(h, rt, tb(res))
+                if enter:
                     rt.save = save
                     if paired_ref:
                         dup = lambda t: torch.cat([t, t], 0)
                         h = dup(h)
-                        skips = [dup(s_) for s_ in skips]
+                        if not lean:
+                            skips = [dup(s_) for s_ in skips]
                         temb_all = dup(temb_all)
                         rt.enc = dup(rt.enc)
                         rt.B = 2 * B
                         rt.paired = True
-                h = res.fwd(h, rt, tb(res))
+                if not (enter and lean):
+                    h = res.fwd(h, rt, tb(res))
                 if hasattr(blk, "attentions"):
                     h = blk.attentions[j].fwd(h, rt, f"down_blocks.{i}.attentions.{j}")
                 skips.append(h)
@@ -1572,9 +1596,9 @@
         for i, blk in enumerate(self.up_blocks):
             for j, res in enumerate(blk.resnets):
                 s = skips.pop()
-                hc = K.concat_channels(h, s)
+                hc = K.concat_channels(h, s) if s.shape[0] == h.shape[0] else K.concat_channels_wrap(h, s)
                 if rt.save:
-                    rt.saved.append({"c1": h.shape[-1]})
+                    rt.saved.append({"c1": h.shape[-1], "lean": lean, "dead": lean and len(skips) < n_prefix})
                 h = res.fwd(hc, rt, tb(res))
                 if hasattr(blk, "attentions"):
                     h = blk.attentions[j].fwd(h, rt, f"up_blocks.{i}.attentions.{j}")
@@ -1632,11 +1656,15 @@
                 if hasattr(blk, "attentions"):
                     dh = blk.attentions[j].bwd(dh, rt, f"up_blocks.{i}.attentions.{j}")
                     done(f"up_blocks.{i}.attentions.{j}")
-                dhc = blk.resnets[j].bwd(dh, rt)
+                sk = rt.saved[-2]
+                if sk["lean"]:
+                    dh, ds = blk.resnets[j].bwd_skip(dh, rt, sk["c1"], sk["dead"])
+                else:
+                    dh, ds = K.split_channels(blk.resnets[j].bwd(dh, rt), sk["c1"])
                 done(f"up_blocks.{i}.resnets.{j}")
-                c1 = rt.saved.pop()["c1"]
-                dh, ds = K.split_channels(dhc, c1)
-                skip_grads.append(ds)
+                rt.saved.pop()
+                if not sk["dead"]:
+                    skip_grads.append(ds)
         m = self.mid_block
         dh = m.resnets[1].bwd(dh, rt)
         done("mid_block.resnets.1")
```

Result: no change. 39.07 imgs/s (median of 6 runs) (+0.7%).
